# djeedai/bevy_hanabi

Hardware: AMD Instinct MI355X
Metric: particle-updates/sec (higher is better)
Workload: dtype f32

## Files before the change

### bevy_hanabi_amd/__init__.py

```python
from . import build

try:
    from ._hanabi_host import *
except ImportError:
    try:
        build.build_host(verbose=True)
        from ._hanabi_host import *
    except Exception as _e:
        raise ImportError("bevy_hanabi_amd._hanabi_host could not be built: run `python -m bevy_hanabi_amd.build`") from _e
from . import _hanabi_host as host

from .runtime import Comm, Context, Effect, EffectMetadata, HanabiError, Program, SimParams, jit_precompile, jit_precompile_set, jit_precompile_steps, validate_program
```

### bevy_hanabi_amd/build.py

```python
import os
import subprocess
import sys
import sysconfig

_DIR = os.path.dirname(os.path.abspath(__file__))
_CSRC = os.path.join(_DIR, "csrc")

HIP_FLAGS = ["--offload-arch=gfx950", "-O3", "-std=c++17", "-ffp-contract=off", "-fhip-fp32-correctly-rounded-divide-sqrt",
             "-fPIC", "-shared", "-Wno-unused-value"]
HOST_FLAGS = ["-std=c++17", "-O2", "-fPIC", "-shared", "-ffp-contract=off", "-fvisibility=hidden"]


def _newer(target, sources):
    if not os.path.exists(target):
        return True
    t = os.path.getmtime(target)
    return any(os.path.getmtime(s) > t for s in sources)


def runtime_lib_path():
    return os.path.join(_DIR, "libhanabi_amd.so")


def host_module_path():
# ... 74 lines not shown
    lines = [f"// generated by bevy_hanabi_amd/build.py from {unit}.hsaco -- do not edit",
             f"alignas(4096) static const unsigned char {array}[{len(code)}] = {{"]
    lines += ["    " + ",".join(str(b) for b in code[i:i + 64]) + "," for i in range(0, len(code), 64)]
    lines.append("};")
    new = "\n".join(lines) + "\n"
    if not os.path.exists(inc) or open(inc).read() != new:
        open(inc, "w").write(new)
    return out


def build_export_code(force=False, verbose=False):
    return _build_code_object("hnb_export", "kExportCode", [], force, verbose)


def build_export_sort_code(force=False, verbose=False):
    return _build_code_object("hnb_export_sort", "kExportSortCode", ["-ffp-contract=off"], force, verbose)


def build_export_filter_code(force=False, verbose=False):
    return _build_code_object("hnb_export_filter", "kExportFilterCode", ["-ffp-contract=off"], force, verbose)


def build_export_cull_code(force=False, verbose=False):
    return _build_code_object("hnb_export_cull", "kExportCullCode", ["-ffp-contract=off"], force, verbose)


def build_export_filter_prog_code(force=False, verbose=False):
    return _build_code_object("hnb_export_filter_prog", "kExportFilterProgCode", ["-ffp-contract=off"], force, verbose)


def build_export_cull_prog_code(force=False, verbose=False):
    return _build_code_object("hnb_export_cull_prog", "kExportCullProgCode", ["-ffp-contract=off"], force, verbose)


def build_export_bin_code(force=False, verbose=False):
    return _build_code_object("hnb_export_bin", "kExportBinCode", ["-ffp-contract=off"], force, verbose,
                              headers=("hnb_export_bin.h", "hnb_bin_cell.h", "hnb_export.h", "hnb_export_rows.hip.h", "hnb_sort_key.h", "hnb_export_sort.hip.h"))


EXPORT_CODE_OBJECTS = (build_export_code, build_export_sort_code, build_export_filter_code, build_export_cull_code, build_export_filter_prog_code,
                       build_export_cull_prog_code)
BINNED_CODE_OBJECTS = (build_export_bin_code,)


def build_bounds_code(force=False, verbose=False):
    return _build_code_object("hnb_bounds", "kBoundsCode", ["-ffp-contract=off"], force, verbose, headers=("hnb_bounds.h", "hnb_sort_key.h"))


QUERY_CODE_OBJECTS = (build_bounds_code,)


def build_runtime(force=False, verbose=False):
    srcs = [os.path.join(_CSRC, "hanabi_amd.hip")] + sorted(os.path.join(_CSRC, f) for f in os.listdir(_CSRC) if f.endswith(".h"))
    srcs += [os.path.join(_DIR, "..", "include", h) for h in ("hanabi_amd.h", "hanabi_amd_binned.h")]
    for build_code in EXPORT_CODE_OBJECTS + BINNED_CODE_OBJECTS + QUERY_CODE_OBJECTS:
        srcs.append(build_code(force, verbose))
    out = runtime_lib_path()
    if force or _newer(out, srcs):
        embed_headers()
        hipcc = os.environ.get("HIPCC", "/opt/rocm/bin/hipcc")
        cmd = [hipcc] + HIP_FLAGS + [srcs[0], "-o", out, "-lhiprtc", "-ldl"]
        if verbose:
            print(" ".join(cmd))
        subprocess.check_call(cmd, cwd=_CSRC)
    return out


def build_host(force=False, verbose=False):
    import pybind11

    hdir = os.path.join(_CSRC, "host")
    srcs = [os.path.join(hdir, f) for f in ("pybind.cpp", "hanabi.cpp", "lowering.cpp", "wgsl.cpp", "ron.cpp")]
    deps = srcs + [os.path.join(hdir, "hanabi.hpp"), os.path.join(_DIR, "..", "include", "hanabi_amd.h")]
    out = host_module_path()
    if force or _newer(out, deps):
        cmd = ["g++"] + HOST_FLAGS + ["-I" + pybind11.get_include(), "-I" + sysconfig.get_paths()["include"]] + srcs + ["-o", out]
        if verbose:
            print(" ".join(cmd))
        subprocess.check_call(cmd)
    return out


def host_lib_path():
    return os.path.join(_DIR, "libhanabi_host.so")


def build_host_lib(force=False, verbose=False):
    hdir = os.path.join(_CSRC, "host")
    srcs = [os.path.join(hdir, f) for f in ("capi.cpp", "hanabi.cpp", "lowering.cpp", "wgsl.cpp", "ron.cpp")]
    deps = srcs + [os.path.join(hdir, "hanabi.hpp"), os.path.join(_DIR, "..", "include", "hanabi_amd.h"), os.path.join(_DIR, "..", "include", "hanabi_amd_host.h")]
    out = host_lib_path()
    if force or _newer(out, deps):
        cmd = ["g++"] + [f for f in HOST_FLAGS if f != "-fvisibility=hidden"] + srcs + ["-o", out]
        if verbose:
            print(" ".join(cmd))
        subprocess.check_call(cmd)
    return out


def build_examples(force=False, verbose=False):
    root = os.path.join(_DIR, "..")
    src = os.path.join(root, "examples", "multi_gpu.c")
    out = os.path.join(root, "examples", "multi_gpu")
    if force or _newer(out, [src, os.path.join(root, "include", "hanabi_amd.h"), runtime_lib_path()]):
        cmd = ["gcc", "-std=c99", "-O2", "-Wall", "-pthread", "-I" + os.path.join(root, "include"), src, "-L" + _DIR, "-lhanabi_amd",
               "-Wl,-rpath," + os.path.abspath(_DIR), "-Wl,-rpath,$ORIGIN/../bevy_hanabi_amd", "-o", out]
        if verbose:
# ... 25 lines not shown
```

### bevy_hanabi_amd/csrc/hanabi_amd.hip

```cpp
#include <hip/hip_runtime.h>

#include <algorithm>
#include <atomic>
#include <chrono>
#include <cmath>
#include <condition_variable>
#include <cstdarg>
#include <cstdio>
#include <cstring>
#include <deque>
#include <memory>
#include <mutex>
#include <string>
#include <thread>
#include <vector>

#include "hnb_kernels.hip.h"
#include "hnb_jit.h"
#include "hnb_sort.hip.h"
#include "hnb_comm.h"
#include "hnb_plan.h"
#include "hnb_export.h"
#include "hnb_export_code.inc"
#include "hnb_export_sort_code.inc"
#include "hnb_filter_pred.h"
#include "hnb_export_filter_code.inc"
#include "hnb_export_cull_code.inc"
#include "hnb_export_filter_prog_code.inc"
#include "hnb_export_cull_prog_code.inc"
#include "hnb_export_bin.h"
#include "hnb_export_bin_code.inc"
#include "hnb_bounds.h"
#include "hnb_bounds_code.inc"

using namespace hnb;

namespace {

thread_local std::string g_last_error;

int fail(int code, const char* fmt, ...) {
    char buf[512];
    va_list ap;
    va_start(ap, fmt);
    vsnprintf(buf, sizeof buf, fmt, ap);
    va_end(ap);
    g_last_error = buf;
    return code;
}

#define HIP_TRY(expr)                                                                            \
    do {                                                                                         \
        hipError_t e_ = (expr);                                                                  \
        if (e_ != hipSuccess)                                                                    \
            return fail(e_ == hipErrorOutOfMemory ? HNB_ERR_OUT_OF_MEMORY : HNB_ERR_HIP, "%s failed: %s", #expr, \
                        hipGetErrorString(e_));                                                  \
    } while (0)

size_t align_up(size_t v, size_t a) { return (v + a - 1) / a * a; }


struct TimingPair { hipEvent_t a, b; const HnbProgram* prog; };
constexpr uint32_t kFrameRing = plan::kStageSlots;
constexpr uint32_t kSceneMaxChunks = 16;
constexpr uint32_t kSceneMaxInitBlocks = 64;
#ifndef HNB_GENERIC_SPLIT_MAX
#define HNB_GENERIC_SPLIT_MAX 128
#endif
constexpr uint32_t kGenericSplitMaxChunks = HNB_GENERIC_SPLIT_MAX;
#ifndef HNB_STREAM_QUARTERS
#define HNB_STREAM_QUARTERS 1
#endif
constexpr uint32_t kSceneMaxCodeLen = 64;

}

typedef void (*StreamLaunchFn)(uint32_t grid, hipStream_t stream, const SlotArgs& sa, const uint64_t* inst_base, const DevFrameInst* fi,
                               const uint32_t* ublocks, const CompactBufs& cb);
#ifndef HNB_STREAM_WAVES_COHORT
#define HNB_STREAM_WAVES_COHORT 4
#endif
template <class PROG, int WAVES>
void launch_stream(uint32_t grid, hipStream_t stream, const SlotArgs& sa, const uint64_t* inst_base, const DevFrameInst* fi,
                   const uint32_t* ublocks, const CompactBufs& cb) {
    if (sa.age_cohort) k_update_slots_stream<PROG, (WAVES > HNB_STREAM_WAVES_COHORT ? HNB_STREAM_WAVES_COHORT : WAVES), 0, true><<<grid, kBlock, 0, stream>>>(sa, inst_base, fi, ublocks, cb);
// ... 23 lines not shown
typedef ProgStatic<OP_(AGE_TICK), OP_(VEL_ADD), OP_(VEL_SCALE), OP_(EULER)> ProgAccelDrag;
typedef ProgStatic<OP_(AGE_TICK), OP_(VEL_ADD), OP_(KILL_AABB), OP_(EULER)> ProgAccelKillAabb;
typedef ProgStatic<OP_(AGE_TICK), OP_(RADIAL_ACCEL), OP_(EULER)> ProgRadial;
typedef ProgStatic<OP_(AGE_TICK), OP_(CONFORM_SPHERE), OP_(CONFORM_SPHERE), OP_(KILL_AABB), OP_(KILL_SPHERE), OP_(EULER)> ProgForceField;
#undef OP_
#ifndef HNB_STREAM_WAVES_INTERP
#define HNB_STREAM_WAVES_INTERP 5
#endif

void select_stream_kernel(const Ins* code, uint32_t n, StreamLaunchFn* fn, const char** name, StreamLaunchFn* fused) {
#define TRY_(PROG, WAVES) if (PROG::matches(code, n)) { *fn = &launch_stream<PROG, WAVES>; *fused = &launch_stream_fused<PROG, WAVES>; *name = #PROG; return; }
    *fused = nullptr;
    if (ProgNone::matches(code, n)) { *fn = &launch_stream<ProgNone, HNB_STREAM_WAVES>; *name = "ProgNone"; return; }
    if (ProgAge::matches(code, n)) { *fn = &launch_stream_age; *fused = &launch_stream_fused<ProgAge, 4>; *name = "ProgAge"; return; }
    TRY_(ProgAgeEuler, HNB_STREAM_WAVES)
    TRY_(ProgAccel, HNB_STREAM_WAVES)
    TRY_(ProgDrag, HNB_STREAM_WAVES)
    TRY_(ProgDragAccel, HNB_STREAM_WAVES)
    TRY_(ProgAccelDrag, HNB_STREAM_WAVES)
    TRY_(ProgAccelKillAabb, HNB_STREAM_WAVES)
    TRY_(ProgRadial, HNB_STREAM_WAVES)
    TRY_(ProgForceField, HNB_STREAM_WAVES_FULL)
#undef TRY_
    *fn = &launch_stream<ProgInterp, HNB_STREAM_WAVES_INTERP>;
    *name = "ProgInterp";
}

struct ProgramOptions {
    uint32_t age_cohort = HNB_AGE_COHORT_AUTO;
    bool cull_lifetime = true;
    bool horizon = true;
};

struct SetBuildJob {
    struct Member { std::vector<HnbAttrEntry> attrs; std::vector<Ins> init, update; bool streams = false, cohort = false; };
    std::vector<Member> members;
    jit::SetResult res;
    bool ok = false;
    std::atomic<bool> done{false};
    std::thread worker;
};

struct JitJob {
    uint64_t program_serial = 0;
    std::vector<uint8_t> blob;
    HnbProgramHeader hdr{};
    std::vector<HnbAttrEntry> attrs;
    bool streams = false, aot_static = false;
    ProgramOptions opt;
    bool steps = false;
    std::vector<Ins> steps_ops;
    int steps_waves = 0;
    bool steps_cohort = false;
    jit::Result res;
    bool ok = false;
};
struct JitWorker {
    std::thread thread;
    std::mutex mu;
    std::condition_variable cv, done_cv;
    std::deque<std::unique_ptr<JitJob>> queue, done;
    bool stop = false;
    uint32_t in_flight = 0;
};

struct HnbContext {
    int device = 0;
    hipStream_t stream = nullptr;
    hipStream_t own_stream = nullptr;
    hipStream_t upload_stream = nullptr;
    hipStream_t side_stream = nullptr;
    hipEvent_t ev_fork = nullptr, ev_join = nullptr;
    bool overlap_updates = true;
    bool stream_hints = true;
    bool break_proof = false;
    void* h_stage[kFrameRing] = {};
    void* d_stage[kFrameRing] = {};
    size_t stage_bytes = 0;
    bool large_bar = false;
    bool direct_upload = true;
    bool stage_direct = false;
    bool direct_failed = false;
    uint64_t direct_frames = 0, copied_frames = 0;
    uint64_t ring_waits = 0, ring_wait_ns = 0;
    hipEvent_t stage_done[plan::kStageGroups] = {};
    plan::StageRing stage_ring;
    uint32_t num_cus = 256;
    std::vector<HnbProgram*> programs;
    HnbSimParams sim{};
    uint32_t frame = 0;
    uint32_t list_order = HNB_LIST_ORDER_SPAWN;
    ProgramOptions popt;
    bool skip_lists = true;
    bool alternate = true;
    bool suffix_proof = true;
    uint32_t slot_init = 1;
    bool ring_lists = true;
    bool scene_merge = true;
    bool transpose = true;
    uint32_t timing = 0;
    uint32_t timing_tick = 0;
    std::vector<TimingPair> t_update, t_init, t_compact;
    std::vector<hipEvent_t> event_pool;
    uint32_t comm_refs = 0;
    uint32_t set_mode = HNB_SET_MODULE_CACHED;
    struct SetModule {
        hipModule_t module = nullptr;
        hipFunction_t init = nullptr, update = nullptr;
        jit::SetPlan plan;
        uint32_t gen = 0;
    } set;
    bool jit_async = false;
    std::unique_ptr<JitWorker> jit_worker;
    uint64_t next_program_serial = 1;
    std::shared_ptr<SetBuildJob> set_job;
    plan::SetLookupState set_lookup;
    uint32_t set_frames = 0;
    uint32_t set_failed_builds = 0;
    std::string set_log;
    bool fuse_steps = true;
    HnbStepStats step_stats{};
    hipModule_t export_module[kExportUnitCount] = {};
    hipFunction_t export_fn[kExpKernelCount] = {};
    hipModule_t export_bin_module = nullptr;
    hipFunction_t export_bin_fn[kExportBinKernelCount] = {};
    hipModule_t bounds_module = nullptr;
    hipFunction_t bounds_fn[kBoundsKernelCount] = {};
};

struct HnbProgram {
    HnbContext* ctx = nullptr;
    HnbProgramHeader hdr{};
    std::vector<HnbAttrEntry> attrs;
    std::vector<HnbPropEntry> props;
    DevProgram dev{};
    Ins* d_code = nullptr;
    size_t slab_bytes = 0;
    bool wide_file = false;
    uint32_t cull_dt_operand = 0;
    bool update_streams = false;
    uint32_t age_cohort_mode = HNB_AGE_COHORT_AUTO;
    bool auto_materialise = false;
    StreamLaunchFn stream_launch = nullptr;
    StreamLaunchFn stream_launch_fused = nullptr;
    uint32_t fuse_span = 1, fused_left = 0;
    uint32_t safe_launches = 0;
    std::vector<uint32_t> fuse_ublocks;
    uint32_t fused_frames = 0;
    const char* stream_kernel_name = "";
    hipModule_t jit_module = nullptr;
    hipFunction_t jit_init = nullptr, jit_update = nullptr, jit_init_slots = nullptr;
    bool slot_init_eligible = false;
    uint32_t slot_init_frames = 0;
    uint32_t sort_skipped_frames = 0;
    uint32_t sort_path_frames[3] = {0, 0, 0};
    bool tick_sign_seen = false;
    uint64_t serial = 0;
    bool jit_pending = false;
    std::string kernel_info, jit_log;
    enum class StepsState { NotRequested, Built, Pending, Failed };
    hipModule_t steps_module = nullptr;
    hipFunction_t steps_update = nullptr;
    StepsState steps_state = StepsState::NotRequested;
    bool steps_from_cache = false;
    std::string steps_why;
    std::vector<Ins> steps_ops;
    int steps_waves = 0;
    bool steps_cohort = false;
    std::vector<Ins> h_init, h_update;
    std::string set_sig;
    uint64_t set_sig_hash = 0;
    uint32_t set_gen = 0, set_case = kNoSetCase, set_frames = 0;
    std::vector<Ins> uniform_code;
    std::vector<HnbEffect*> effects;
    uint32_t table_cap = 0;
    uint64_t* d_inst_base = nullptr;
    DevMeta* d_meta[2] = {nullptr, nullptr};
    struct SlabBlock { char* base = nullptr; uint32_t n_slots = 0; };
    std::vector<SlabBlock> slab_blocks;
    std::vector<void*> free_slabs;
    size_t slab_stride = 0;
    bool slot_order = false;
    bool has_ribbons = false;
    SortArgs sort{};
    uint32_t* d_plane_by_attr = nullptr;
    std::vector<uint32_t> parent_attrs;
    uint32_t* d_ev_totals = nullptr;
    unsigned long long* h_ev_counts = nullptr;
    uint32_t level = 0;
    uint32_t* d_counts = nullptr;
    uint32_t* d_deaths = nullptr;
    plan::SkipFacts skip_facts;
    plan::SkipHistory skip_hist;
    plan::RibbonFacts ribbon_facts;
    plan::RibbonHistory ribbon_hist;
    plan::FramePlan plan;
    const char* d_frame_cur = nullptr;
    uint32_t ring = 0;
    size_t frame_bytes = 0;
    uint32_t parity = 0;
    uint32_t frames_run = 0;
    uint32_t merged_frames = 0;
    uint32_t unmerged_frames = 0;
    bool horizon_eligible = false;
    uint32_t hz_parity = 0;
    uint32_t hz_frames = 0;
    uint32_t* d_safe = nullptr;
    unsigned long long* h_safe = nullptr;
    uint32_t* d_fault = nullptr;
    uint32_t skipped_frames = 0;
    uint32_t sort_parity = 0;
    uint32_t suffix_frames = 0;
    uint32_t sort_rotated_frames = 0;
    bool ring_live = false;
    uint32_t ring_frames = 0;
    uint32_t* d_export = nullptr;
    uint32_t export_cap = 0;
    std::vector<uint32_t> export_slot_bases;
    void* d_export_sort = nullptr;
    uint32_t export_sort_inst = 0;
    void* d_export_filter = nullptr;
// ... 529 lines not shown

void install_program_jit(HnbProgram* p, const jit::Result& res) {
    const bool aot_static = p->update_streams && strcmp(p->stream_kernel_name, "ProgInterp") != 0;
    hipModule_t mod = nullptr;
    hipFunction_t fi = nullptr, fu = nullptr;
    hipError_t je = hipModuleLoadData(&mod, res.code.data());
    if (je == hipSuccess && !res.init_name.empty()) je = hipModuleGetFunction(&fi, mod, res.init_name.c_str());
    hipFunction_t fs = nullptr;
    if (je == hipSuccess && !res.init_slots_name.empty()) je = hipModuleGetFunction(&fs, mod, res.init_slots_name.c_str());
    if (je == hipSuccess && !res.update_name.empty()) je = hipModuleGetFunction(&fu, mod, res.update_name.c_str());
    if (je != hipSuccess) {
        p->jit_log = std::string("loading the specialised code object failed: ") + hipGetErrorString(je);
        if (mod) hipModuleUnload(mod);
        (void)hipGetLastError();
        return;
    }
    p->jit_module = mod; p->jit_init = fi; p->jit_update = fu; p->jit_init_slots = fs;
    p->kernel_info = std::string(p->wide_file ? "wide-file " : "") + "init=" + (p->jit_init ? "jit" : (p->hdr.init_len ? "interp" : "none")) + " update=" +
                     (p->jit_update ? (p->update_streams ? "jit-stream" : "jit-generic")
                                    : (p->update_streams ? (aot_static ? std::string("aot-stream:") + p->stream_kernel_name : std::string("interp-stream"))
                                                         : std::string("interp-generic")));
    if (res.from_cache) p->kernel_info += " (jit cache hit)";
}

jit::Request make_steps_request(const std::vector<Ins>& ops, int waves, bool cohort) {
    jit::Request rq;
    rq.update = ops.data(); rq.update_len = (uint32_t)ops.size();
    rq.want_update_stream = !ops.empty();
    rq.stream_waves = waves;
    rq.stream_cohort = cohort;
    return rq;
}
void steps_build_failed(HnbProgram* p, const std::string& log) {
    p->steps_state = HnbProgram::StepsState::Failed;
    p->steps_why = log.substr(0, log.find('\n'));
    if (p->steps_why.empty()) p->steps_why = "no log";
    p->jit_log = "steps kernel: " + log;
}
void install_program_steps(HnbProgram* p, const jit::Result& res) {
    hipModule_t mod = nullptr;
    hipFunction_t fu = nullptr;
    hipError_t je = hipModuleLoadData(&mod, res.code.data());
    if (je == hipSuccess) je = hipModuleGetFunction(&fu, mod, res.update_name.c_str());
    if (je != hipSuccess) {
        if (mod) hipModuleUnload(mod);
        (void)hipGetLastError();
        steps_build_failed(p, std::string("loading the code object failed: ") + hipGetErrorString(je));
        return;
    }
    p->steps_module = mod; p->steps_update = fu;
    p->steps_from_cache = res.from_cache;
    p->steps_state = HnbProgram::StepsState::Built;
}
const char* steps_never_reason(const HnbProgram* p) {
    if (!p->update_streams) return "never fuses: not a macro-op update";
    if (!p->skip_facts.eligible) return "never fuses: particles can die by more than their lifetime, or the program is linked to others";
    if (p->has_ribbons || p->hdr.n_event_channels != 0u) return "never fuses: ribbons or spawn events";
    if (p->stream_launch_fused) return "pre-built fused kernel";
    if (p->steps_ops.empty()) return "never fuses: the update is not specialised (HNB_JIT=0)";
    return nullptr;
}
void jit_worker_main(JitWorker* w);
void queue_jit_job(HnbContext* ctx, std::unique_ptr<JitJob> job) {
    if (!ctx->jit_worker) {
        ctx->jit_worker.reset(new JitWorker());
        ctx->jit_worker->thread = std::thread(jit_worker_main, ctx->jit_worker.get());
    }
    {
        std::lock_guard<std::mutex> lk(ctx->jit_worker->mu);
        ctx->jit_worker->queue.push_back(std::move(job));
        ctx->jit_worker->in_flight += 1;
    }
    ctx->jit_worker->cv.notify_one();
}
void request_steps_kernel(HnbContext* ctx, HnbProgram* p, bool wait) {
    if (p->steps_state != HnbProgram::StepsState::NotRequested || !p->jit_update || steps_never_reason(p)) return;
    const bool async = ctx->jit_async && !wait;
    jit::Result res;
    if (jit::build_steps(make_steps_request(p->steps_ops, p->steps_waves, p->steps_cohort), res, async)) {
        install_program_steps(p, res);
    } else if (async && res.log.empty()) {
        std::unique_ptr<JitJob> job(new JitJob());
        job->program_serial = p->serial;
        job->steps = true;
        job->steps_ops = p->steps_ops; job->steps_waves = p->steps_waves; job->steps_cohort = p->steps_cohort;
        queue_jit_job(ctx, std::move(job));
        p->steps_state = HnbProgram::StepsState::Pending;
    } else {
        steps_build_failed(p, res.log);
    }
}

void jit_worker_main(JitWorker* w) {
    for (;;) {
        std::unique_ptr<JitJob> job;
        {
            std::unique_lock<std::mutex> lk(w->mu);
            w->cv.wait(lk, [&] { return w->stop || !w->queue.empty(); });
            if (w->stop) return;
            job = std::move(w->queue.front());
            w->queue.pop_front();
        }
        if (job->steps) {
            job->ok = jit::build_steps(make_steps_request(job->steps_ops, job->steps_waves, job->steps_cohort), job->res);
        } else {
            const jit::Request rq = make_jit_request(job->blob.data(), job->hdr, job->attrs.data(), job->streams, job->aot_static, job->opt);
            job->ok = jit::build(rq, job->res);
        }
        {
            std::lock_guard<std::mutex> lk(w->mu);
            w->done.push_back(std::move(job));
        }
        w->done_cv.notify_all();
    }
}
void install_finished_jit(HnbContext* ctx) {
    if (!ctx->jit_worker) return;
    std::deque<std::unique_ptr<JitJob>> done;
    {
        std::lock_guard<std::mutex> lk(ctx->jit_worker->mu);
        done.swap(ctx->jit_worker->done);
        ctx->jit_worker->in_flight -= (uint32_t)done.size();
    }
    for (std::unique_ptr<JitJob>& j : done) {
        HnbProgram* p = nullptr;
        for (HnbProgram* q : ctx->programs)
            if (q->serial == j->program_serial) p = q;
        if (!p) continue;
        if (j->steps) {
            if (j->ok) install_program_steps(p, j->res);
            else steps_build_failed(p, j->res.log);
            continue;
        }
        p->jit_pending = false;
        if (j->ok) install_program_jit(p, j->res);
        else if (!j->res.log.empty()) p->jit_log = j->res.log;
    }
}

jit::Request make_set_request(const Ins* init, uint32_t init_len, const Ins* update, uint32_t update_len, const HnbAttrEntry* attrs, uint32_t n_attrs,
                              bool streams, bool cohort) {
    jit::Request rq;
    rq.attrs = attrs; rq.n_attrs = n_attrs;
    rq.init = init; rq.init_len = init_len; rq.update = update; rq.update_len = update_len;
    rq.want_init = true;
    rq.want_update_stream = streams;
    rq.want_update_generic = !streams;
    rq.stream_cohort = streams && cohort;
    rq.wide_file = false;
    return rq;
}

}

extern "C" {

const char* hnb_last_error(void) { return g_last_error.c_str(); }
const char* hnb_version(void) { return "bevy_hanabi_amd 0.2.0 (gfx950)"; }

int hnb_ctx_create(int device_id, HnbContext** out_ctx) {
    if (!out_ctx) return fail(HNB_ERR_INVALID_ARG, "out_ctx is NULL");
    int count = 0;
    if (hipGetDeviceCount(&count) != hipSuccess || count <= 0)
        return fail(HNB_ERR_NO_DEVICE, "no HIP device available (the hanabi hot path has no CPU fallback)");
    if (device_id < 0 || device_id >= count) return fail(HNB_ERR_INVALID_ARG, "device %d out of range [0,%d)", device_id, count);
    HIP_TRY(hipSetDevice(device_id));
    HnbContext* ctx = new HnbContext();
    ctx->device = device_id;
    hipError_t e = hipStreamCreateWithFlags(&ctx->stream, hipStreamNonBlocking);
    if (e != hipSuccess) { delete ctx; return fail(HNB_ERR_HIP, "hipStreamCreate failed: %s", hipGetErrorString(e)); }
    ctx->own_stream = ctx->stream;
    e = hipStreamCreateWithFlags(&ctx->upload_stream, hipStreamNonBlocking);
    if (e != hipSuccess) { hipStreamDestroy(ctx->stream); delete ctx; return fail(HNB_ERR_HIP, "hipStreamCreate failed: %s", hipGetErrorString(e)); }
    if (hipStreamCreateWithFlags(&ctx->side_stream, hipStreamNonBlocking) != hipSuccess || hipEventCreateWithFlags(&ctx->ev_fork, hipEventDisableTiming) != hipSuccess ||
        hipEventCreateWithFlags(&ctx->ev_join, hipEventDisableTiming) != hipSuccess) {
        (void)hipGetLastError();
        ctx->overlap_updates = false;
    }
    hipDeviceProp_t prop;
    if (hipGetDeviceProperties(&prop, device_id) == hipSuccess) {
        if (prop.multiProcessorCount > 0) ctx->num_cus = (uint32_t)prop.multiProcessorCount;
        ctx->large_bar = prop.isLargeBar != 0;
    }
    *out_ctx = ctx;
// ... 26 lines not shown
    if (ctx->ev_fork) hipEventDestroy(ctx->ev_fork);
    if (ctx->ev_join) hipEventDestroy(ctx->ev_join);
    for (uint32_t i = 0; i < kFrameRing; ++i) {
        hipFree(ctx->d_stage[i]);
        if (ctx->h_stage[i]) hipHostFree(ctx->h_stage[i]);
    }
    for (hipEvent_t e : ctx->stage_done)
        if (e) hipEventDestroy(e);
    delete ctx;
    return HNB_OK;
}

int hnb_ctx_set_stream(HnbContext* ctx, void* hip_stream) {
    if (!ctx) return fail(HNB_ERR_INVALID_ARG, "ctx is NULL");
    HIP_TRY(hipStreamSynchronize(ctx->stream));
    plan::stage_ring_drained(ctx->stage_ring);
    ctx->stream = hip_stream ? static_cast<hipStream_t>(hip_stream) : ctx->own_stream;
    return HNB_OK;
}

int hnb_ctx_set_option(HnbContext* ctx, uint32_t option, uint32_t value) {
    if (!ctx) return fail(HNB_ERR_INVALID_ARG, "ctx is NULL");
    switch (option) {
        case HNB_OPT_LIST_ORDER:
            if (value != HNB_LIST_ORDER_SPAWN && value != HNB_LIST_ORDER_SLOT) return fail(HNB_ERR_INVALID_ARG, "unknown list order %u", value);
            ctx->list_order = value;
            return HNB_OK;
        case HNB_OPT_ALTERNATE: ctx->alternate = value != 0u; return HNB_OK;
        case HNB_OPT_SKIP_LISTS: ctx->skip_lists = value != 0u; return HNB_OK;
        case HNB_OPT_AGE_COHORT:
            if (value > HNB_AGE_COHORT_AUTO) return fail(HNB_ERR_INVALID_ARG, "unknown age-cohort mode %u", value);
            ctx->popt.age_cohort = value;
            return HNB_OK;
        case HNB_OPT_CULL_LIFETIME: ctx->popt.cull_lifetime = value != 0u; return HNB_OK;
        case HNB_OPT_HORIZON: ctx->popt.horizon = value != 0u; return HNB_OK;
        case HNB_OPT_TEST_BREAK_PROOF: {
            const char* e = getenv("HNB_ENABLE_TEST_HOOKS");
            if (value != 0u && !(e && e[0] == '1')) return fail(HNB_ERR_INVALID_ARG, "HNB_OPT_TEST_BREAK_PROOF is a test hook: refused unless HNB_ENABLE_TEST_HOOKS=1 is set in the environment");
            ctx->break_proof = value != 0u;
            return HNB_OK;
        }
        case HNB_OPT_TRANSPOSE: ctx->transpose = value != 0u; return HNB_OK;
        case HNB_OPT_SCENE_MERGE: ctx->scene_merge = value != 0u; return HNB_OK;
        case HNB_OPT_SUFFIX_PROOF: ctx->suffix_proof = value != 0u; return HNB_OK;
        case HNB_OPT_RING_LISTS: ctx->ring_lists = value != 0u; return HNB_OK;
        case HNB_OPT_SLOT_INIT:
            if (value > 2u) return fail(HNB_ERR_INVALID_ARG, "unknown slot-init mode %u", value);
            ctx->slot_init = value;
            return HNB_OK;
        case HNB_OPT_STREAM_HINTS: ctx->stream_hints = value != 0u; return HNB_OK;
        case HNB_OPT_DIRECT_UPLOAD: ctx->direct_upload = value != 0u; return HNB_OK;
        case HNB_OPT_JIT_ASYNC: ctx->jit_async = value != 0u; return HNB_OK;
        case HNB_OPT_FUSE_STEPS: ctx->fuse_steps = value != 0u; return HNB_OK;
        case HNB_OPT_SET_MODULE:
            if (value > HNB_SET_MODULE_BACKGROUND) return fail(HNB_ERR_INVALID_ARG, "unknown set-module mode %u", value);
            ctx->set_mode = value;
            ctx->set_lookup = plan::SetLookupState();
            return HNB_OK;
        case HNB_OPT_OVERLAP_UPDATES: ctx->overlap_updates = value != 0u && ctx->side_stream && ctx->ev_fork && ctx->ev_join; return HNB_OK;
        default: return fail(HNB_ERR_INVALID_ARG, "unknown option %u", option);
    }
}

int hnb_ctx_synchronize(HnbContext* ctx) {
    if (!ctx) return fail(HNB_ERR_INVALID_ARG, "ctx is NULL");
    HIP_TRY(hipStreamSynchronize(ctx->stream));
    return HNB_OK;
}

int hnb_program_validate(const void* blob, size_t blob_size) { return validate_blob(blob, blob_size, nullptr); }

int hnb_program_create(HnbContext* ctx, const void* blob, size_t blob_size, HnbProgram** out_prog) {
    if (!ctx || !out_prog) return fail(HNB_ERR_INVALID_ARG, "NULL argument");
    HnbProgramHeader h;
    int rc = validate_blob(blob, blob_size, &h);
    if (rc != HNB_OK) return rc;
    HIP_TRY(hipSetDevice(ctx->device));
    const uint8_t* b = static_cast<const uint8_t*>(blob);
    HnbProgram* p = new HnbProgram();
    p->ctx = ctx;
    p->hdr = h;
    p->attrs.resize(h.n_attrs);
    memcpy(p->attrs.data(), b + h.attrs_off, h.n_attrs * sizeof(HnbAttrEntry));
    p->props.resize(h.n_props);
    if (h.n_props) memcpy(p->props.data(), b + h.props_off, h.n_props * sizeof(HnbPropEntry));

    DevProgram& d = p->dev;
    size_t slab_bytes = 0;
    p->update_streams = update_is_streamable(b, h, p->attrs.data());
    if (!layout_slab(h, p->attrs.data(), d, p->sort, &slab_bytes)) { delete p; return fail(HNB_ERR_BAD_PROGRAM, "effect slab exceeds 1 TiB (capacity %u)", h.capacity); }
    p->slot_order = ctx->list_order == HNB_LIST_ORDER_SLOT && !(h.flags & HNB_PROG_HAS_RIBBONS);
    p->has_ribbons = (h.flags & HNB_PROG_HAS_RIBBONS) != 0;
    p->slab_bytes = slab_bytes;
    p->parent_attrs.resize(h.parent_n_attrs);
    if (h.parent_n_attrs) memcpy(p->parent_attrs.data(), b + h.parent_attrs_off, (size_t)h.parent_n_attrs * 4);
    {
        uint32_t planes[HNB_ATTR_COUNT];
        for (uint32_t i = 0; i < HNB_ATTR_COUNT; ++i) planes[i] = kNoPlane;
        for (uint32_t i = 0; i < h.n_attrs; ++i) planes[p->attrs[i].attr] = d.attrs[i].plane_off.v;
        hipError_t pe = hipMalloc(&p->d_plane_by_attr, sizeof planes);
        if (pe != hipSuccess) { delete p; return fail(HNB_ERR_OUT_OF_MEMORY, "hipMalloc failed: %s", hipGetErrorString(pe)); }
        hipMemcpy(p->d_plane_by_attr, planes, sizeof planes, hipMemcpyHostToDevice);
    }
    p->uniform_code.resize(h.uniform_len);
    if (h.uniform_len) memcpy(p->uniform_code.data(), b + h.uniform_off, (size_t)h.uniform_len * 8);
    p->wide_file = std::max(h.init_regs, h.update_regs) > HNB_VM_MAX_REGS;
    p->slot_init_eligible = slot_init_eligible(b, h);
    if (cull_eligible(b, h, p->attrs.data(), p->update_streams, ctx->popt, &p->cull_dt_operand)) {
        d.cull_lifetime = 1u;
        d.age_cohort = age_cohort_eligible(b, h, p->attrs.data(), p->update_streams, ctx->popt) ? 1u : 0u;
    }
    p->age_cohort_mode = ctx->popt.age_cohort;
    p->auto_materialise = ctx->popt.age_cohort == HNB_AGE_COHORT_AUTO && d.age_cohort != 0u && (h.render_reads_lo >> HNB_ATTR_AGE & 1u) != 0u;
    if (p->update_streams) select_stream_kernel(reinterpret_cast<const Ins*>(b + h.update_off), h.update_len, &p->stream_launch, &p->stream_kernel_name, &p->stream_launch_fused);
    if (!p->wide_file && jit::enabled()) {
        p->h_init.assign(reinterpret_cast<const Ins*>(b + h.init_off), reinterpret_cast<const Ins*>(b + h.init_off) + h.init_len);
        p->h_update.assign(reinterpret_cast<const Ins*>(b + h.update_off), reinterpret_cast<const Ins*>(b + h.update_off) + h.update_len);
        p->set_sig = jit::set_signature(make_set_request(p->h_init.data(), h.init_len, p->h_update.data(), h.update_len, p->attrs.data(), h.n_attrs, p->update_streams, d.age_cohort != 0u));
        p->set_sig_hash = jit::fnv1a(p->set_sig);
    }
    const bool aot_static = p->update_streams && strcmp(p->stream_kernel_name, "ProgInterp") != 0;
    p->kernel_info = std::string(p->wide_file ? "wide-file " : "") + "init=" + (h.init_len ? "interp" : "none") + " update=" +
                     (p->update_streams ? (aot_static ? std::string("aot-stream:") + p->stream_kernel_name : std::string("interp-stream")) : std::string("interp-generic"));
    p->serial = ctx->next_program_serial++;
    if (jit::enabled()) {
        const jit::Request rq = make_jit_request(b, h, p->attrs.data(), p->update_streams, aot_static, ctx->popt);
        if (rq.want_update_stream) {
            p->steps_ops.assign(rq.update, rq.update + rq.update_len);
            p->steps_waves = rq.stream_waves; p->steps_cohort = rq.stream_cohort;
        }
        jit::Result res;
        if (jit::build(rq, res, ctx->jit_async)) {
            install_program_jit(p, res);
        } else if (ctx->jit_async && res.log.empty() && (rq.want_init || rq.want_update_generic || rq.want_update_stream)) {
            std::unique_ptr<JitJob> job(new JitJob());
            job->program_serial = p->serial;
            job->blob.assign(b, b + blob_size);
            job->hdr = h; job->attrs = p->attrs; job->streams = p->update_streams; job->aot_static = aot_static; job->opt = ctx->popt;
            queue_jit_job(ctx, std::move(job));
            p->jit_pending = true;
        } else if (!res.log.empty()) {
            p->jit_log = res.log;
        }
    }
    if (p->has_ribbons && p->update_streams) {
        bool ok = true;
        uint32_t ticks = 0;
        const Ins* uc = reinterpret_cast<const Ins*>(b + h.update_off);
        for (uint32_t i = 0; i < h.update_len && ok; ++i) {
            const uint32_t op = uc[i].x & 0xffu, dst = (uc[i].x >> 8) & 0xffu;
            if (op == HNB_OP_M_AGE_TICK) { ticks += 1; p->ribbon_facts.tick_operand = HNB_OPERAND_DECODE((uc[i].x >> 16) & 0xffu, uc[i].y >> 13); ok = (p->ribbon_facts.tick_operand & HNB_OPERAND_DECODED_U) != 0; }
            if (op == HNB_OP_M_PIN_SET && dst == HNB_REG_AGE) ok = false;
        }
        ok = ok && ticks == 1;
        for (uint32_t a = 0; a < h.n_attrs; ++a)
            if (p->attrs[a].attr == HNB_ATTR_RIBBON_ID && (p->attrs[a].update_flags & HNB_ATTR_UPD_STORE)) ok = false;
        const Ins* ic = reinterpret_cast<const Ins*>(b + h.init_off);
        for (uint32_t i = 0; i < h.init_len && ok; ++i) {
            const uint32_t op = ic[i].x & 0xffu, dst = (ic[i].x >> 8) & 0xffu, wd = ((ic[i].y >> 8) & 3u) + 1u;
            if (op == HNB_OP_M_PIN_SET && dst == HNB_REG_AGE) {
                p->ribbon_facts.age_init_operand = HNB_OPERAND_DECODE((ic[i].x >> 16) & 0xffu, ic[i].y >> 13);
                p->ribbon_facts.age_init_set = true;
                ok = (p->ribbon_facts.age_init_operand & HNB_OPERAND_DECODED_U) != 0;
            } else if (op != HNB_OP_STA && op != HNB_OP_ALIVE_SET && op != HNB_OP_ALIVE_AND && op != HNB_OP_KILL_IF && !(op >= HNB_OP_M_AGE_TICK) &&
                       dst <= HNB_REG_AGE && dst + wd > HNB_REG_AGE) {
                ok = false;
            }
        }
        p->ribbon_facts.provable = ok;
        int rid_index = -1;
        for (uint32_t a = 0; a < h.n_attrs; ++a) if (p->attrs[a].attr == HNB_ATTR_RIBBON_ID) rid_index = (int)a;
        uint32_t rid_stores = 0;
        bool front = ok && rid_index >= 0;
        for (uint32_t i = 0; i < h.init_len && front; ++i) {
            const uint32_t op = ic[i].x & 0xffu;
            if (op == HNB_OP_STA && (ic[i].y >> 16) == (uint32_t)rid_index) {
                rid_stores += 1;
                p->ribbon_facts.rid_operand = HNB_OPERAND_DECODE((ic[i].x >> 16) & 0xffu, ic[i].y >> 13);
                front = (p->ribbon_facts.rid_operand & HNB_OPERAND_DECODED_U) != 0;
            }
        }
        p->ribbon_facts.rid_set = rid_stores == 1;
        uint32_t life_sets = 0;
        for (uint32_t i = 0; i < h.init_len && front; ++i) {
            const uint32_t op = ic[i].x & 0xffu, dst = (ic[i].x >> 8) & 0xffu, wd = ((ic[i].y >> 8) & 3u) + 1u;
            if (op == HNB_OP_M_PIN_SET && dst == HNB_REG_LIFETIME) {
                life_sets += 1;
                p->ribbon_facts.life_operand = HNB_OPERAND_DECODE((ic[i].x >> 16) & 0xffu, ic[i].y >> 13);
                front = (p->ribbon_facts.life_operand & HNB_OPERAND_DECODED_U) != 0;
            } else if (op != HNB_OP_STA && op != HNB_OP_ALIVE_SET && op != HNB_OP_ALIVE_AND && op != HNB_OP_KILL_IF && !(op >= HNB_OP_M_AGE_TICK) &&
                       dst <= HNB_REG_LIFETIME && dst + wd > HNB_REG_LIFETIME) {
                front = false;
            }
        }
        for (uint32_t i = 0; i < h.update_len && front; ++i) {
            const uint32_t op = uc[i].x & 0xffu, dst = (uc[i].x >> 8) & 0xffu;
            if (op == HNB_OP_M_KILL_SPHERE || op == HNB_OP_M_KILL_AABB || op == HNB_OP_KILL_IF || op == HNB_OP_ALIVE_SET || op == HNB_OP_ALIVE_AND) front = false;
            if (op == HNB_OP_M_PIN_SET && dst == HNB_REG_LIFETIME) front = false;
        }
        p->ribbon_facts.front_static = front && rid_stores <= 1 && life_sets == 1;
    }
    {
        bool kills = false;
        const Ins* uc = reinterpret_cast<const Ins*>(b + h.update_off);
        for (uint32_t i = 0; i < h.update_len; ++i) {
            const uint32_t op = uc[i].x & 0xffu;
            kills = kills || op == HNB_OP_M_KILL_SPHERE || op == HNB_OP_M_KILL_AABB;
        }
        p->skip_facts.eligible = p->update_streams && d.cull_lifetime && !kills && h.n_event_channels == 0 && !(h.flags & HNB_PROG_READS_PARENT);
        p->skip_facts.dt_operand = p->cull_dt_operand;
        p->horizon_eligible = p->update_streams && d.cull_lifetime && !kills && !p->has_ribbons && !p->slot_order && ctx->popt.horizon;
        if (hipMalloc(&p->d_fault, 4) != hipSuccess ||
            hipHostMalloc(reinterpret_cast<void**>(&p->h_safe), 8, hipHostMallocDefault) != hipSuccess) {
            if (p->jit_module) hipModuleUnload(p->jit_module);
            hipFree(p->d_fault); hipFree(p->d_plane_by_attr);
            delete p;
            return fail(HNB_ERR_OUT_OF_MEMORY, "allocating the program's bookkeeping words failed");
        }
        hipMemset(p->d_fault, 0, 4);
        *p->h_safe = 0xffffffffull;
        p->dev.horizon = p->horizon_eligible ? 1u : 0u;
    }
    const size_t code_bytes = ((size_t)h.init_len + h.update_len) * 8;
    hipError_t e = hipMalloc(&p->d_code, std::max<size_t>(code_bytes, 8));
    if (e != hipSuccess) {
        if (p->jit_module) hipModuleUnload(p->jit_module);
        hipFree(p->d_plane_by_attr); hipFree(p->d_fault); hipHostFree(p->h_safe);
        delete p;
        return fail(HNB_ERR_OUT_OF_MEMORY, "hipMalloc(code) failed: %s", hipGetErrorString(e));
    }
    if (h.init_len) hipMemcpy(p->d_code, b + h.init_off, (size_t)h.init_len * 8, hipMemcpyHostToDevice);
    if (h.update_len) hipMemcpy(p->d_code + h.init_len, b + h.update_off, (size_t)h.update_len * 8, hipMemcpyHostToDevice);
    d.init_code = p->d_code;
    d.update_code = p->d_code + h.init_len;
    ctx->programs.push_back(p);
    *out_prog = p;
    return HNB_OK;
}

int hnb_program_destroy(HnbProgram* p) {
    if (!p) return HNB_OK;
    HnbContext* ctx = p->ctx;
    hipSetDevice(ctx->device);
    hipStreamSynchronize(ctx->stream);
    while (!p->effects.empty()) hnb_effect_destroy(p->effects.back());
    free_tables(p);
    if (p->jit_module) hipModuleUnload(p->jit_module);
    if (p->steps_module) hipModuleUnload(p->steps_module);
    for (auto& blk : p->slab_blocks) hipFree(blk.base);
    hipFree(p->d_plane_by_attr);
    hipFree(p->d_code);
    hipFree(p->d_fault);
    hipFree(p->d_export);
    hipFree(p->d_export_sort);
    hipFree(p->d_export_filter);
    hipFree(p->d_bounds);
    hipFree(p->d_export_cull);
    if (p->h_export_filter_rows) hipHostFree(p->h_export_filter_rows);
    if (p->export_filter_staged) hipEventDestroy(p->export_filter_staged);
    if (p->h_safe) hipHostFree(p->h_safe);
    ctx->programs.erase(std::remove(ctx->programs.begin(), ctx->programs.end(), p), ctx->programs.end());
    delete p;
    return HNB_OK;
}

constexpr size_t kPlacementMinBytes = (size_t)256 << 20;
constexpr size_t kPlacementMaxTransient = (size_t)32 << 30;
hipError_t alloc_slab_block(HnbProgram* p, size_t bytes, char** out) {
    int want = 24;
    if (const char* e = getenv("HNB_SLAB_CANDIDATES")) want = std::max(1, std::min(32, atoi(e)));
    want = (int)std::min<size_t>((size_t)want, std::max<size_t>(1, kPlacementMaxTransient / std::max<size_t>(bytes, 1)));
    if (bytes < kPlacementMinBytes || bytes != p->slab_stride) want = 1;
    const bool debug = getenv("HNB_DEBUG_ALLOC") != nullptr;
    if (want == 1) return hipMalloc(reinterpret_cast<void**>(out), bytes);
    ProbeArgs pa{};
    pa.n_quads = (p->dev.capacity + 3u) / 4u;
    for (uint32_t a = 0; a < p->dev.n_attrs && pa.n_planes < 8; ++a) {
        const DevAttr& at = p->dev.attrs[a];
        if (at.reg == HNB_REG_NONE) continue;
        pa.off[pa.n_planes] = at.plane_off;
        pa.stride16[pa.n_planes] = at.ncomp;
        if (at.reg != HNB_REG_LIFETIME) pa.write_mask |= 1u << pa.n_planes;
        pa.n_planes += 1;
    }
    hipStream_t st = p->ctx->stream;
    hipEvent_t ev0 = nullptr, ev1 = nullptr;
    if (hipEventCreate(&ev0) != hipSuccess || hipEventCreate(&ev1) != hipSuccess) {
        if (ev0) hipEventDestroy(ev0);
        (void)hipGetLastError();
        return hipMalloc(reinterpret_cast<void**>(out), bytes);
    }
    char* best = nullptr;
    float best_ms = 0.0f;
    std::vector<float> times;
    std::vector<char*> rejected;
    hipError_t first_error = hipSuccess;
    for (int c = 0; c < want; ++c) {
        char* cand = nullptr;
        const hipError_t e = hipMalloc(reinterpret_cast<void**>(&cand), bytes);
        if (e != hipSuccess) { if (!best) first_error = e; (void)hipGetLastError(); break; }
        hipMemsetAsync(cand, 0, bytes, st);
// ... 743 lines not shown
    } else {
        p->sort_path_frames[2] += 1;
        for (uint32_t pass = 0; pass < 8; ++pass) {
            k_sort_hist<<<tiles, kBlock, 0, st>>>(so, p->d_inst_base, mo, pass);
            k_sort_scatter<<<tiles, kBlock, 0, st>>>(so, p->d_inst_base, mo, pass);
        }
    }
    k_sort_merge<<<tiles, kBlock, 0, st>>>(so, p->d_inst_base, mo);
    p->ribbon_hist.dirty = false;
}

static bool reads_particles_of(const HnbProgram* child, const HnbProgram* parent) {
    for (const HnbEffect* fx : child->effects)
        if (fx->parent && fx->parent->prog == parent) return true;
    return false;
}
static int enqueue_init_passes(HnbContext* ctx, const std::vector<HnbProgram*>& order, FrameJobs& fj, bool timed) {
    const uint32_t np = (uint32_t)order.size();
    std::vector<uint8_t> on_side(np, 0);
    if (fj.heavy) {
        std::vector<uint8_t> reads((size_t)np * np, 0);
        int heavy = -1;
        for (uint32_t c = 0; c < np; ++c) {
            if (order[c] == fj.heavy) heavy = (int)c;
            for (uint32_t p = 0; p < np; ++p) reads[(size_t)c * np + p] = reads_particles_of(order[c], order[p]) ? 1u : 0u;
        }
        plan::partition_init_passes(reads.data(), np, heavy, on_side.data());
    }
    for (int pass = 0; pass < (fj.heavy ? 2 : 1); ++pass) {
    hipStream_t st = ctx->stream;
    if (pass == 1) {
        st = ctx->side_stream;
        HIP_TRY(hipEventRecord(ctx->ev_fork, ctx->stream));
        HIP_TRY(hipStreamWaitEvent(st, ctx->ev_fork, 0));
        fj.forked = true;
    }
    for (size_t pi = 0; pi < order.size(); ++pi) {
        HnbProgram* p = order[pi];
        if ((int)on_side[pi] != pass) continue;
        const uint32_t n = (uint32_t)p->effects.size();
        const uint32_t par = p->parity;
        const uint32_t blocks = p->plan.init_blocks;
        const char* d = p->d_frame_cur;
        const DevFrameInst* dfi = reinterpret_cast<const DevFrameInst*>(d);
        const uint32_t* dub = reinterpret_cast<const uint32_t*>(d + (size_t)n * sizeof(DevFrameInst));
        if (blocks && p->plan.merge.init_family < 0) {
            TimingPair ti{};
            ti.prog = p;
            if (timed) { ti.a = take_event(ctx); ti.b = take_event(ctx); hipEventRecord(ti.a, st); }
            if (p->plan.slot_init.use) {
                const uint32_t grid = n * p->dev.chunks_per_inst * (kChunk / kSlotInitWg);
                const DevMeta* mi = p->d_meta[par];
                if (p->plan.slot_init.marks) k_spawn_mark<<<grid, kBlock, 0, st>>>(p->dev, p->d_inst_base, mi, dfi);
                if (p->jit_init_slots) {
                    void* ka[] = {&p->dev, &p->d_inst_base, &mi, &dfi, &dub};
                    HIP_TRY(hipModuleLaunchKernel(p->jit_init_slots, grid, 1, 1, kBlock, 1, 1, 0, st, ka, nullptr));
                } else if (p->wide_file) k_init_slots<InterpCodeWide><<<grid, kBlock, 0, st>>>(p->dev, p->d_inst_base, mi, dfi, dub);
                else k_init_slots<InterpCode><<<grid, kBlock, 0, st>>>(p->dev, p->d_inst_base, mi, dfi, dub);
                p->slot_init_frames += 1;
            } else if (p->jit_init) {
                const DevMeta* mi = p->d_meta[par];
                void* ka[] = {&p->dev, &p->d_inst_base, &mi, &dfi, &dub};
                HIP_TRY(hipModuleLaunchKernel(p->jit_init, blocks, 1, 1, kInitBlock, 1, 1, 0, st, ka, nullptr));
            } else {
                if (p->wide_file) k_init<InterpCodeWide><<<blocks, kInitBlock, 0, st>>>(p->dev, p->d_inst_base, p->d_meta[par], dfi, dub);
                else k_init<InterpCode><<<blocks, kInitBlock, 0, st>>>(p->dev, p->d_inst_base, p->d_meta[par], dfi, dub);
            }
            if (timed) { hipEventRecord(ti.b, st); ctx->t_init.push_back(ti); }
        }
    }
    }

    hipStream_t ms = fj.forked ? ctx->side_stream : ctx->stream;
    if (fj.init_set) {
        const void* jobs = fj.init[0].d_jobs;
        uint32_t n_jobs = fj.init[0].n;
        void* ka[] = {&jobs, &n_jobs};
        HIP_TRY(hipModuleLaunchKernel(ctx->set.init, fj.init[0].wgs, 1, 1, kInitBlock, 1, 1, 0, ms, ka, nullptr));
    } else if (fj.init[0].n) k_init_jobs<InterpCode><<<fj.init[0].wgs, kInitBlock, 0, ms>>>(static_cast<const ProgJob*>(fj.init[0].d_jobs), fj.init[0].n);
    if (fj.init[1].n) k_init_jobs<InterpCodeWide><<<fj.init[1].wgs, kInitBlock, 0, ms>>>(static_cast<const ProgJob*>(fj.init[1].d_jobs), fj.init[1].n);
    return HNB_OK;
}

static int enqueue_program_update(HnbContext* ctx, HnbProgram* p, hipStream_t st, bool timed) {
    const uint32_t n = (uint32_t)p->effects.size();
    const uint32_t par = p->parity;
    const char* d = p->d_frame_cur;
    const DevFrameInst* dfi = reinterpret_cast<const DevFrameInst*>(d);
    const uint32_t* dub = reinterpret_cast<const uint32_t*>(d + (size_t)n * sizeof(DevFrameInst));
    const uint32_t total_chunks = n * p->dev.chunks_per_inst;
    CompactBufs cb = compact_bufs_of(ctx, p, n);
    TimingPair tu{}, tc{};
    tu.prog = tc.prog = p;
    if (timed) { tu.a = take_event(ctx); tu.b = take_event(ctx); tc.b = take_event(ctx); hipEventRecord(tu.a, st); }
    const uint32_t write_died = (p->plan.lists && !p->slot_order) ? 1u : 0u;
    if (p->plan.merge.update_family >= 0) {
    } else if (p->update_streams) {
        SlotArgs sa = slot_args_of(ctx, p, n, write_died);
        ctx->step_stats.update_launches += 1;
        if (p->fuse_span >= 2u) {
            sa.fuse_steps = p->fuse_span;
            if (p->steps_update) {
                void* ka[] = {&sa, &p->d_inst_base, &dfi, &dub, &cb};
                HIP_TRY(hipModuleLaunchKernel(p->steps_update, total_chunks, 1, 1, kBlock, 1, 1, 0, st, ka, nullptr));
            } else p->stream_launch_fused(total_chunks, st, sa, p->d_inst_base, dfi, dub, cb);
            ctx->step_stats.fused_launches += 1;
            ctx->step_stats.fused_frames += p->fuse_span;
            p->fused_frames += p->fuse_span;
        } else if (p->jit_update) {
            void* ka[] = {&sa, &p->d_inst_base, &dfi, &dub, &cb};
            HIP_TRY(hipModuleLaunchKernel(p->jit_update, total_chunks, 1, 1, kBlock, 1, 1, 0, st, ka, nullptr));
        } else {
            p->stream_launch(total_chunks, st, sa, p->d_inst_base, dfi, dub, cb);
        }
    } else {
        uint32_t split = total_chunks <= kGenericSplitMaxChunks ? 1u : 0u;
        const uint32_t grid = split ? total_chunks * (kChunk / kBlock) : total_chunks;
        ctx->step_stats.update_launches += 1;
        if (p->jit_update) {
            uint32_t dm = write_died;
            void* ka[] = {&p->dev, &p->d_inst_base, &dfi, &dub, &cb, &dm, &split};
            HIP_TRY(hipModuleLaunchKernel(p->jit_update, grid, 1, 1, kBlock, 1, 1, 0, st, ka, nullptr));
        } else if (p->wide_file) k_update_slots_generic<InterpCodeWide><<<grid, kBlock, 0, st>>>(p->dev, p->d_inst_base, dfi, dub, cb, write_died, split);
        else k_update_slots_generic<InterpCode><<<grid, kBlock, 0, st>>>(p->dev, p->d_inst_base, dfi, dub, cb, write_died, split);
    }
    if (timed) { hipEventRecord(tu.b, st); ctx->t_update.push_back(tu); }
    const CompactArgs ca = compact_args_of(p);
    const bool lists = p->plan.lists;
    if (!lists) p->skipped_frames += p->fuse_span;
    else if (ca.suffix_dead) p->suffix_frames += 1;
    if (lists && p->dev.n_event_channels) {
        k_emit_count<<<total_chunks, kBlock, 0, st>>>(p->dev, p->d_inst_base, p->d_meta[par], dfi, cb);
        uint32_t max_ev = 0;
        for (const HnbEffect* fx : p->effects)
            for (const EventChannel& ch : fx->channels) max_ev = std::max(max_ev, ch.capacity);
        const uint32_t splits = plan::size_event_grid(max_ev, total_chunks);
        k_emit_events<<<dim3(total_chunks, splits), kBlock, 0, st>>>(p->dev, p->d_inst_base, p->d_meta[par], dfi, cb, p->h_ev_counts, ctx->frame);
    }
    if (!p->plan.lists_merged) {
        if (lists) ctx->step_stats.list_launches += ((!p->slot_order && !ca.suffix_dead) ? 2u : 1u) + (p->slot_order ? 2u : 0u);
        if (lists && !p->slot_order && !ca.suffix_dead) k_count_rows<<<total_chunks, kBlock, 0, st>>>(ca, p->d_inst_base, p->d_meta[par], dfi, cb);
        if (lists) k_compact<<<total_chunks, kBlock, 0, st>>>(ca, p->d_inst_base, p->d_meta[par], p->d_meta[par ^ 1], dfi, cb);
        if (lists && p->slot_order) {
            k_order_count<<<total_chunks, kBlock, 0, st>>>(ca, p->d_inst_base, p->d_meta[par], dfi, cb);
            k_order_write<<<total_chunks, kBlock, 0, st>>>(ca, p->d_inst_base, p->d_meta[par], p->d_meta[par ^ 1], dfi, cb);
        }
        if (timed) { tc.a = tu.b; hipEventRecord(tc.b, st); ctx->t_compact.push_back(tc); }
        if (p->has_ribbons) enqueue_ribbon_sort(ctx, p, st);
    }
    HIP_TRY(hipGetLastError());
    return HNB_OK;
}

static int enqueue_update_passes(HnbContext* ctx, const std::vector<HnbProgram*>& order, const FrameJobs& fj, bool timed) {
    hipStream_t light = ctx->stream;
    if (fj.heavy) {
        light = ctx->side_stream;
        if (!fj.forked) {
            HIP_TRY(hipEventRecord(ctx->ev_fork, ctx->stream));
            HIP_TRY(hipStreamWaitEvent(light, ctx->ev_fork, 0));
        }
// ... 5 lines not shown
        const void *sj0 = fj.stream[0].d_jobs, *sj1 = fj.stream[1].d_jobs, *pj = fj.generic[0].d_jobs;
        uint32_t n0 = fj.stream[0].n, n1 = fj.stream[1].n, np = fj.generic[0].n, b0 = fj.stream[0].wgs, b1 = fj.stream[0].wgs + fj.stream[1].wgs;
        void* ka[] = {&sj0, &n0, &sj1, &n1, &pj, &np, &b0, &b1};
        HIP_TRY(hipModuleLaunchKernel(ctx->set.update, fj.stream[0].wgs + fj.stream[1].wgs + fj.generic[0].wgs, 1, 1, kBlock, 1, 1, 0, light, ka, nullptr));
    } else if (fj.stream[0].wgs + fj.stream[1].wgs + fj.generic[0].wgs)
        k_update_jobs<<<fj.stream[0].wgs + fj.stream[1].wgs + fj.generic[0].wgs, kBlock, 0, light>>>(
            static_cast<const StreamJob*>(fj.stream[0].d_jobs), fj.stream[0].n, static_cast<const StreamJob*>(fj.stream[1].d_jobs), fj.stream[1].n,
            static_cast<const ProgJob*>(fj.generic[0].d_jobs), fj.generic[0].n, fj.stream[0].wgs, fj.stream[0].wgs + fj.stream[1].wgs);
    if (fj.generic[1].wgs) k_update_generic_wide_jobs<<<fj.generic[1].wgs, kBlock, 0, light>>>(static_cast<const ProgJob*>(fj.generic[1].d_jobs), fj.generic[1].n);
    for (HnbProgram* p : order) {
        if (p == fj.heavy) continue;
        const int rc = enqueue_program_update(ctx, p, light, timed);
        if (rc != HNB_OK) return rc;
    }
    if (fj.n_lists) {
        k_count_rows_multi<<<fj.lists_wgs, kBlock, 0, light>>>(fj.d_lists, fj.n_lists);
        k_compact_multi<<<fj.lists_wgs, kBlock, 0, light>>>(fj.d_lists, fj.n_lists);
        for (HnbProgram* p : order)
            if (p->plan.lists_merged && p->has_ribbons) enqueue_ribbon_sort(ctx, p, light);
        HIP_TRY(hipGetLastError());
    }
    if (fj.heavy) {
        const int rc = enqueue_program_update(ctx, const_cast<HnbProgram*>(fj.heavy), ctx->stream, timed);
        if (rc != HNB_OK) return rc;
        HIP_TRY(hipEventRecord(ctx->ev_join, light));
        HIP_TRY(hipStreamWaitEvent(ctx->stream, ctx->ev_join, 0));
    }
    return HNB_OK;
}

static int simulate_frame(HnbContext* ctx) {
    HIP_TRY(hipSetDevice(ctx->device));
    install_finished_jit(ctx);
    std::vector<HnbProgram*> order, covered;
    for (HnbProgram* p : ctx->programs)
        if (!p->effects.empty()) (p->fused_left ? covered : order).push_back(p);
    std::stable_sort(order.begin(), order.end(), [](const HnbProgram* x, const HnbProgram* y) { return x->level < y->level; });
    const bool timed = ctx->timing && (ctx->timing_tick % ctx->timing) == 0;
    for (HnbProgram* p : order)
        if (!p->parent_attrs.empty())
            for (size_t i = 0; i < p->effects.size(); ++i)
                if (!p->effects[i]->parent)
                    return fail(HNB_ERR_INVALID_ARG, "effect #%zu reads its parent particle (InheritAttributeModifier / parent_attr) but has no parent: call hnb_effect_set_parent", i);
    uint32_t slot = 0;
    int rc = ensure_stage(ctx, order, &slot);
    if (rc != HNB_OK) return rc;
    size_t stage_off = 0;
    std::vector<plan::InstanceFrame> inst_frames;
    for (HnbProgram* p : order) stage_program_frame(ctx, p, slot, stage_off, inst_frames);
    FrameJobs fj;
    fj.heavy = pick_heavy_program(ctx, order, timed);
    fill_lists_jobs(ctx, order, slot, stage_off, timed, fj);
    fill_merge_jobs(ctx, order, slot, stage_off, timed, fj);
    if (stage_off) {
        if (ctx->stage_direct) {
            direct_write(ctx->d_stage[slot], ctx->h_stage[slot], stage_off);
            ctx->direct_frames += 1;
        } else {
            hipError_t ce = hipMemcpyAsync(ctx->d_stage[slot], ctx->h_stage[slot], stage_off, hipMemcpyHostToDevice, ctx->upload_stream);
            if (ce == hipSuccess) ce = hipStreamSynchronize(ctx->upload_stream);
            if (ce != hipSuccess) {
                plan::stage_ring_end(ctx->stage_ring, !order.empty(), true, false);
                HIP_TRY(ce);
            }
            ctx->copied_frames += 1;
        }
    }
    rc = enqueue_init_passes(ctx, order, fj, timed);
    if (rc == HNB_OK) rc = enqueue_update_passes(ctx, order, fj, timed);
    if (rc != HNB_OK) {
        if (ctx->side_stream && (fj.forked || fj.heavy)) hipStreamSynchronize(ctx->side_stream);
        plan::stage_ring_end(ctx->stage_ring, !order.empty(), true, false);
        return rc;
    }
    for (HnbProgram* p : covered) p->fused_left -= 1;
    for (HnbProgram* p : order) {
        const uint32_t span = p->fuse_span;
        p->fused_left = span - 1u;
        p->fuse_span = 1u;
        p->safe_launches += 1;
        p->ring += span;
        p->parity ^= span & 1u;
        p->frames_run += span;
        if (p->horizon_eligible && p->plan.lists) p->hz_parity ^= 1u;
        if (p->plan.ribbon.ring) { p->ring_live = true; p->ring_frames += 1; }
        else if (p->plan.lists) p->ring_live = false;
    }
    const int stage_event = plan::stage_ring_end(ctx->stage_ring, !order.empty(), true, true);
    if (stage_event != plan::kStageWaitNone) {
        const hipError_t re = hipEventRecord(ctx->stage_done[stage_event], ctx->stream);
        if (re != hipSuccess) ctx->stage_ring.torn = true;
        HIP_TRY(re);
    }
    for (HnbProgram* p : ctx->programs)
        for (HnbEffect* fx : p->effects) fx->spawn_count = 0;
    ctx->frame += 1;
    ctx->step_stats.frames += 1;
    if (ctx->timing) ctx->timing_tick += 1;
    return HNB_OK;
}

static void drop_ahead_inputs(HnbContext* ctx) {
    for (HnbProgram* p : ctx->programs)
        for (HnbEffect* fx : p->effects) { fx->ahead_n = 0; fx->ahead_spawn.clear(); fx->ahead_seed.clear(); fx->ahead_xf.clear(); }
}

// ... 53 lines not shown
        p->fuse_ublocks.resize((size_t)n * span * nu);
        for (uint32_t i = 0; i < n; ++i)
            for (uint32_t t = 0; t < span; ++t)
                if (nu) memcpy(p->fuse_ublocks.data() + ((size_t)i * span + t) * nu, blocks.data() + ((size_t)t * n + i) * nu, (size_t)nu * 4);
    }
}

int hnb_simulate_steps(HnbContext* ctx, uint32_t n_steps, const HnbSimParams* params) {
    if (!ctx) return fail(HNB_ERR_INVALID_ARG, "ctx is NULL");
    if (n_steps == 0u) return HNB_OK;
    if (!params) return fail(HNB_ERR_INVALID_ARG, "params is NULL");
    for (HnbProgram* p : ctx->programs)
        if (!p->parent_attrs.empty())
            for (size_t i = 0; i < p->effects.size(); ++i)
                if (!p->effects[i]->parent)
                    return fail(HNB_ERR_INVALID_ARG, "effect #%zu reads its parent particle (InheritAttributeModifier / parent_attr) but has no parent: call hnb_effect_set_parent", i);
    if (n_steps >= 2u) {
        HIP_TRY(hipSetDevice(ctx->device));
        install_finished_jit(ctx);
        for (HnbProgram* p : ctx->programs) {
            if (p->steps_state != HnbProgram::StepsState::NotRequested || !p->jit_update || !ctx->fuse_steps) continue;
            bool parent = false;
            for (const HnbEffect* fx : p->effects) parent = parent || fx->parent != nullptr;
            if (!parent && (uint64_t)p->effects.size() * p->dev.chunks_per_inst > kSceneMaxChunks) request_steps_kernel(ctx, p, false);
        }
    }
    int rc = HNB_OK;
    for (uint32_t s = 0; s < n_steps && rc == HNB_OK; ++s) {
        ctx->sim = params[s];
        for (HnbProgram* p : ctx->programs)
            for (HnbEffect* fx : p->effects) {
                if (s >= fx->ahead_n) continue;
                fx->spawn_count = fx->ahead_spawn[s];
                fx->seed = fx->ahead_seed[s];
                if (!fx->ahead_xf.empty()) memcpy(fx->xf, &fx->ahead_xf[(size_t)s * 12], sizeof fx->xf);
            }
        if (n_steps - s >= 2u) plan_fused_spans(ctx, params + s, n_steps - s, s);
        rc = simulate_frame(ctx);
    }
    for (HnbProgram* p : ctx->programs) {
        if (rc != HNB_OK) {
            if (p->fuse_span >= 2u) p->skip_hist.dirty = true;
            p->fused_left = 0u;
        }
        p->fuse_span = 1u;
    }
    drop_ahead_inputs(ctx);
    return rc;
}

int hnb_ctx_step_stats(HnbContext* ctx, HnbStepStats* out) {
    if (!ctx || !out) return fail(HNB_ERR_INVALID_ARG, "NULL argument");
    *out = ctx->step_stats;
    return HNB_OK;
}

int hnb_effect_metadata(HnbEffect* fx, HnbEffectMetadata* out) {
    if (!fx || !out) return fail(HNB_ERR_INVALID_ARG, "NULL argument");
    DevMeta m;
    int rc = read_meta(fx, &m);
    if (rc != HNB_OK) return rc;
    const uint32_t cap = fx->prog->dev.capacity;
    out->capacity = cap;
    out->alive_count = m.alive_count;
    out->max_update = m.max_update;
    out->max_spawn = cap - m.alive_count;
    out->indirect_write_index = m.ref_write_index;
    out->particle_counter = m.particle_counter;
    out->instance_count = m.instance_count;
    out->dispatch_x = (m.alive_count + 63u) >> 6;
    out->dead_count = m.dead_count;
    out->spawned = m.spawned;
    out->fault = 0;
    if (fx->prog->d_fault) HIP_TRY(hipMemcpy(&out->fault, fx->prog->d_fault, 4, hipMemcpyDeviceToHost));
    out->reserved = 0;
    return HNB_OK;
}

int hnb_effect_alive_count(HnbEffect* fx, uint32_t* out) {
    if (!fx || !out) return fail(HNB_ERR_INVALID_ARG, "NULL argument");
    DevMeta m;
    int rc = read_meta(fx, &m);
    if (rc != HNB_OK) return rc;
    *out = m.alive_count;
    return HNB_OK;
}

int hnb_effect_read_attr(HnbEffect* fx, uint32_t attr, void* dst, size_t dst_size) {
    if (!fx || !dst) return fail(HNB_ERR_INVALID_ARG, "NULL argument");
    HnbProgram* p = fx->prog;
    const int ai = find_attr(p, attr);
    if (ai < 0) return fail(HNB_ERR_NOT_FOUND, "attribute %u is not part of the particle layout", attr);
    const size_t bytes = (size_t)p->dev.capacity * p->attrs[ai].ncomp * 4;
    if (dst_size < bytes) return fail(HNB_ERR_INVALID_ARG, "destination too small (%zu < %zu)", dst_size, bytes);
    HIP_TRY(hipSetDevice(p->ctx->device));
    if (p->dev.age_cohort && attr == HNB_ATTR_AGE)
        k_materialise_age<<<p->dev.chunks_per_inst, kBlock, 0, p->ctx->stream>>>(p->d_inst_base + fx->index, p->dev.capacity, p->dev.chunks_per_inst, p->dev.lmin_off,
                                                                                  p->dev.attrs[ai].plane_off, p->dev.alive_flag_off);
    HIP_TRY(hipStreamSynchronize(p->ctx->stream));
    HIP_TRY(hipMemcpy(dst, static_cast<char*>(fx->slab) + p->dev.attrs[ai].plane_off, bytes, hipMemcpyDeviceToHost));
    return HNB_OK;
}

int hnb_effect_write_attr(HnbEffect* fx, uint32_t attr, const void* src, size_t src_size) {
    if (!fx || !src) return fail(HNB_ERR_INVALID_ARG, "NULL argument");
    HnbProgram* p = fx->prog;
// ... 808 lines not shown
        cmp(0, sa + pa->dev.alive_off[list_column(ma.write_index)], sb + pb->dev.alive_off[list_column(mb.write_index)], ma.alive_count, list_head(ma.write_index), list_head(mb.write_index), cap);
        cmp(1, sa + pa->dev.dead_off + (size_t)ma.alive_count * 4, sb + pb->dev.dead_off + (size_t)mb.alive_count * 4, cap - ma.alive_count);
    }
    for (size_t i = 0; i < pa->attrs.size(); ++i) cmp(2 + i, sa + pa->dev.attrs[i].plane_off, sb + pb->dev.attrs[i].plane_off, (uint64_t)cap * pa->attrs[i].ncomp);
    std::vector<unsigned long long> res(n_sections * 2);
    e = hipGetLastError();
    if (e == hipSuccess) e = hipDeviceSynchronize();
    if (e == hipSuccess) e = hipMemcpy(res.data(), d_out, n_sections * 16, hipMemcpyDeviceToHost);
    hipFree(d_out);
    if (e != hipSuccess) return fail(HNB_ERR_HIP, "hnb_effect_compare: %s", hipGetErrorString(e));
    out->alive_list_diffs = res[0]; out->dead_list_diffs = res[2];
    for (size_t i = 0; i < pa->attrs.size(); ++i) out->attr_diffs += res[2 * (2 + i)];
    for (size_t i = 0; i < n_sections && out->first_section < 0; ++i)
        if (res[2 * i]) { out->first_section = i < 2 ? (int32_t)i : (int32_t)(2 + pa->attrs[i - 2].attr); out->first_index = res[2 * i + 1]; }
    out->equal = out->counter_diffs == 0u && out->alive_list_diffs == 0ull && out->dead_list_diffs == 0ull && out->attr_diffs == 0ull;
    return HNB_OK;
}

int hnb_effect_sort_ribbons(HnbEffect* fx) {
    if (!fx) return fail(HNB_ERR_INVALID_ARG, "fx is NULL");
    if (!fx->prog->has_ribbons) return fail(HNB_ERR_INVALID_ARG, "the particle layout has no RIBBON_ID attribute: nothing to sort");
    return HNB_OK;
}

int hnb_program_kernel_info(HnbProgram* prog, char* buf, size_t buf_size) {
    if (!prog || !buf || !buf_size) return fail(HNB_ERR_INVALID_ARG, "NULL argument");
    std::string s = prog->kernel_info;
    if (prog->jit_pending) s += " (specialisation pending: HNB_OPT_JIT_ASYNC)";
    if (!prog->jit_log.empty()) s += "\njit log: " + prog->jit_log;
    {
        const char* never = steps_never_reason(prog);
        s += "\nsteps kernel: ";
        switch (prog->steps_state) {
        case HnbProgram::StepsState::NotRequested: s += std::string("not requested") + (never ? std::string(" (") + never + ")" : std::string()); break;
        case HnbProgram::StepsState::Built: s += std::string("built") + (prog->steps_from_cache ? " (jit cache hit)" : ""); break;
        case HnbProgram::StepsState::Pending: s += "pending (HNB_OPT_JIT_ASYNC)"; break;
        case HnbProgram::StepsState::Failed: s += "failed: " + prog->steps_why; break;
        }
    }
    if (!prog->dev.age_cohort && prog->dev.cull_lifetime && prog->age_cohort_mode == HNB_AGE_COHORT_AUTO && (prog->hdr.render_reads_lo >> HNB_ATTR_AGE & 1u))
        s += "\nage cohorts: off (HNB_AGE_COHORT_AUTO: the asset's render modifiers read AGE after every frame)";
    if (prog->dev.age_cohort) {
        hipStreamSynchronize(prog->ctx->stream);
        std::vector<uint32_t> st(prog->dev.chunks_per_inst);
        size_t in_cohort = 0;
        for (const HnbEffect* fx : prog->effects) {
            if (hipMemcpy(st.data(), static_cast<const char*>(fx->slab) + prog->dev.lmin_off + (size_t)prog->dev.chunks_per_inst * 8, st.size() * 4, hipMemcpyDeviceToHost) != hipSuccess) break;
            for (uint32_t v : st) in_cohort += v == 1u ? 1u : 0u;
        }
        s += "\nage cohorts: " + std::to_string(in_cohort) + " of " + std::to_string(prog->effects.size() * (size_t)prog->dev.chunks_per_inst) + " chunks";
        if (prog->auto_materialise) s += " (HNB_AGE_COHORT_AUTO: the asset's render modifiers read AGE, the update keeps the plane current)";
    }
    if (prog->slot_init_frames) s += "\nslot-major init (large spawns): " + std::to_string(prog->slot_init_frames) + " frames";
    if (prog->has_ribbons && prog->suffix_frames) s += "\ncasualties proven to be the list's last rows (no k_count_rows): " + std::to_string(prog->suffix_frames) + " frames";
    if (prog->has_ribbons && prog->ring_frames) s += "\nlist kept as a ring (no row rewritten): " + std::to_string(prog->ring_frames) + " frames";
    if (prog->has_ribbons && prog->sort_skipped_frames) s += "\nribbon sorts skipped in list-free frames: " + std::to_string(prog->sort_skipped_frames) + " frames";
    if (prog->has_ribbons) s += "\nribbon sorts by rotation: " + std::to_string(prog->sort_rotated_frames) + " of " + std::to_string(prog->frames_run) + " frames" + (prog->ribbon_facts.front_static ? "" : " (not eligible)");
    if (prog->has_ribbons) s += "\nribbon sorts by path: one-tile " + std::to_string(prog->sort_path_frames[0]) + ", one-workgroup " + std::to_string(prog->sort_path_frames[1]) +
                                ", multi-launch " + std::to_string(prog->sort_path_frames[2]) + " frames";
    if (prog->merged_frames) s += "\nupdate served by a merged launch (small programs of the context share one): " + std::to_string(prog->merged_frames) + " frames";
    if (prog->unmerged_frames) s += "\nkept out of the shared launches (the loaded set module does not know this program; its own specialised kernels): " + std::to_string(prog->unmerged_frames) + " frames";
    if (prog->set_frames) s += "\n... by the context's set module (the program's specialised code behind the shared launch): " + std::to_string(prog->set_frames) + " frames";
    if (!prog->ctx->set_log.empty() && !prog->set_sig.empty()) s += "\nset module: " + prog->ctx->set_log;
    if (prog->ctx->set_failed_builds && !prog->set_sig.empty()) s += "\nset module builds that failed: " + std::to_string(prog->ctx->set_failed_builds);
    if (prog->horizon_eligible) s += "\ndeath horizons in use: " + std::to_string(prog->hz_frames) + " frames";
    s += "\nlists skipped: " + std::to_string(prog->skipped_frames) + " of " + std::to_string(prog->frames_run) + " frames" + (prog->skip_facts.eligible ? "" : " (not eligible)");
    s += "\nframe parameters (context): written by the host into device memory in " + std::to_string(prog->ctx->direct_frames) + " frames, copied in " + std::to_string(prog->ctx->copied_frames) +
         (prog->ctx->large_bar ? "" : " (the device memory is not host-visible: no large BAR)") + (prog->ctx->direct_failed ? " (host-visible slots failed their check)" : "");
    s += "\nhnb_simulate waited for the device (the frame " + std::to_string(kFrameRing - plan::kStageGroup + 1u) + " before still running) in " + std::to_string(prog->ctx->ring_waits) + " of " + std::to_string(prog->ctx->frame) +
         " frames, " + std::to_string(prog->ctx->ring_wait_ns / 1000) + " us in all";
    snprintf(buf, buf_size, "%s", s.c_str());
    return HNB_OK;
}

int hnb_jit_precompile(const void* blob, size_t blob_size) {
    HnbProgramHeader h;
    int rc = validate_blob(blob, blob_size, &h);
    if (rc != HNB_OK) return rc;
    const uint8_t* b = static_cast<const uint8_t*>(blob);
    std::vector<HnbAttrEntry> attrs(h.n_attrs);
    memcpy(attrs.data(), b + h.attrs_off, h.n_attrs * sizeof(HnbAttrEntry));
    const bool streams = update_is_streamable(b, h, attrs.data());
    bool aot_static = false;
    if (streams) {
        StreamLaunchFn fn = nullptr;
        const char* name = "";
        StreamLaunchFn fused = nullptr;
        select_stream_kernel(reinterpret_cast<const Ins*>(b + h.update_off), h.update_len, &fn, &name, &fused);
        aot_static = strcmp(name, "ProgInterp") != 0;
    }
    const jit::Request rq = make_jit_request(b, h, attrs.data(), streams, aot_static, ProgramOptions());
    if (!rq.want_init && !rq.want_update_generic && !rq.want_update_stream) return HNB_OK;
    jit::Result res;
    if (!jit::build(rq, res)) return fail(HNB_ERR_BAD_PROGRAM, "kernel specialisation failed: %s", res.log.c_str());
    return HNB_OK;
}

int hnb_jit_precompile_steps(const void* blob, size_t blob_size) {
    HnbProgramHeader h;
    int rc = validate_blob(blob, blob_size, &h);
    if (rc != HNB_OK) return rc;
    const uint8_t* b = static_cast<const uint8_t*>(blob);
    std::vector<HnbAttrEntry> attrs(h.n_attrs);
    memcpy(attrs.data(), b + h.attrs_off, h.n_attrs * sizeof(HnbAttrEntry));
    if (!update_is_streamable(b, h, attrs.data())) return HNB_OK;
    StreamLaunchFn fn = nullptr, fused = nullptr;
    const char* name = "";
    select_stream_kernel(reinterpret_cast<const Ins*>(b + h.update_off), h.update_len, &fn, &name, &fused);
    const jit::Request rq = make_jit_request(b, h, attrs.data(), true, strcmp(name, "ProgInterp") != 0, ProgramOptions());
    if (!rq.want_update_stream) return HNB_OK;
    jit::Result res;
    if (!jit::build_steps(rq, res)) return fail(HNB_ERR_BAD_PROGRAM, "steps kernel: specialisation failed: %s", res.log.c_str());
    return HNB_OK;
}

int hnb_program_prepare_steps(HnbProgram* prog) {
    if (!prog) return fail(HNB_ERR_INVALID_ARG, "prog is NULL");
    HnbContext* ctx = prog->ctx;
    if (steps_never_reason(prog)) return HNB_OK;
    HIP_TRY(hipSetDevice(ctx->device));
    for (;;) {
        install_finished_jit(ctx);
        if (!prog->jit_pending && prog->steps_state != HnbProgram::StepsState::Pending) break;
        std::unique_lock<std::mutex> lk(ctx->jit_worker->mu);
        ctx->jit_worker->done_cv.wait(lk, [&] { return !ctx->jit_worker->done.empty(); });
    }
    request_steps_kernel(ctx, prog, true);
    if (prog->steps_state == HnbProgram::StepsState::Failed) return fail(HNB_ERR_BAD_PROGRAM, "steps kernel: %s", prog->steps_why.c_str());
    return HNB_OK;
}

int hnb_jit_precompile_set(const void* const* blobs, const size_t* blob_sizes, uint32_t n_blobs) {
    if (!blobs || !blob_sizes || n_blobs == 0u) return fail(HNB_ERR_INVALID_ARG, "NULL argument");
    struct Member { std::vector<HnbAttrEntry> attrs; std::vector<Ins> init, update; bool streams = false, cohort = false; };
    std::vector<Member> mem;
    mem.reserve(n_blobs);
    for (uint32_t i = 0; i < n_blobs; ++i) {
        HnbProgramHeader h;
        const int rc = validate_blob(blobs[i], blob_sizes[i], &h);
        if (rc != HNB_OK) return rc;
        if (std::max(h.init_regs, h.update_regs) > HNB_VM_MAX_REGS) continue;
        if ((uint64_t)h.capacity > (uint64_t)kSceneMaxChunks * kChunk || h.n_event_channels != 0u || (h.flags & HNB_PROG_READS_PARENT)) continue;
        const uint8_t* b = static_cast<const uint8_t*>(blobs[i]);
        Member m;
        m.attrs.resize(h.n_attrs);
        memcpy(m.attrs.data(), b + h.attrs_off, h.n_attrs * sizeof(HnbAttrEntry));
        m.init.assign(reinterpret_cast<const Ins*>(b + h.init_off), reinterpret_cast<const Ins*>(b + h.init_off) + h.init_len);
        m.update.assign(reinterpret_cast<const Ins*>(b + h.update_off), reinterpret_cast<const Ins*>(b + h.update_off) + h.update_len);
        m.streams = update_is_streamable(b, h, m.attrs.data());
        uint32_t dt_operand = 0;
        const ProgramOptions opt;
        m.cohort = cull_eligible(b, h, m.attrs.data(), m.streams, opt, &dt_operand) && age_cohort_eligible(b, h, m.attrs.data(), m.streams, opt);
        mem.push_back(std::move(m));
    }
    std::vector<jit::Request> members;
    for (const Member& m : mem)
        members.push_back(make_set_request(m.init.data(), (uint32_t)m.init.size(), m.update.data(), (uint32_t)m.update.size(), m.attrs.data(), (uint32_t)m.attrs.size(), m.streams, m.cohort));
    if (members.size() < 2u) return HNB_OK;
    jit::SetResult res;
    if (!jit::build_set(members, res, false)) return fail(HNB_ERR_BAD_PROGRAM, "set module: kernel specialisation failed: %s", res.log.c_str());
    return HNB_OK;
}

int hnb_comm_unique_id(void* out_id) {
    if (!out_id) return fail(HNB_ERR_INVALID_ARG, "out_id is NULL");
// ... 191 lines not shown
```

### bevy_hanabi_amd/csrc/hnb_jit.h

```cpp
#pragma once
#include <dlfcn.h>
#include <hip/hip_runtime.h>
#include <hip/hiprtc.h>
#include <sys/stat.h>
#include <unistd.h>
#include <cstdio>
#include <cstdlib>
#include <cstring>
#include <fstream>
#include <algorithm>
#include <atomic>
#include <sstream>
#include <string>
#include <vector>
#include "hnb_dev.h"
#include "hnb_embedded_headers.inc"

namespace hnb {
namespace jit {

inline bool enabled() {
    const char* e = getenv("HNB_JIT");
    return !(e && e[0] == '0');
}

inline uint64_t fnv1a(const std::string& s, uint64_t h = 1469598103934665603ull) {
    for (unsigned char c : s) { h ^= c; h *= 1099511628211ull; }
    return h;
}

inline std::string cache_dir() {
    if (const char* e = getenv("HNB_JIT_CACHE")) return e;
    Dl_info info;
    if (dladdr(reinterpret_cast<const void*>(&fnv1a), &info) && info.dli_fname) {
        std::string p = info.dli_fname;
        const size_t k = p.rfind('/');
        if (k != std::string::npos) return p.substr(0, k) + "/jit_cache";
    }
    return "/tmp/hanabi_amd_jit_cache";
}

struct Request {
    const HnbAttrEntry* attrs = nullptr;
    uint32_t n_attrs = 0;
    const Ins* init = nullptr;
    uint32_t init_len = 0;
    const Ins* update = nullptr;
    uint32_t update_len = 0;
    bool want_init = false;
    bool want_init_slots = false;
    bool want_update_generic = false;
    bool want_update_stream = false;
    int stream_waves = 6;
    bool stream_cohort = false;
    bool wide_file = false;
};

struct Result {
    std::vector<char> code;
    std::string init_name, init_slots_name, update_name;
    std::string log;
    bool from_cache = false;
};

inline void emit_ins(std::ostringstream& o, const Ins* code, uint32_t n) {
    char buf[160];
    for (uint32_t i = 0; i < n; ++i) {
        snprintf(buf, sizeof buf, "        vm_exec<true, false>(Ins{0x%08xu, 0x%08xu}, S, U, nullptr, nullptr, io);\n", code[i].x, code[i].y);
        o << buf;
    }
}

inline void emit_code_struct(std::ostringstream& o, const Request& rq, const std::string& name) {
    o << "struct " << name << " {\n";
    o << "    using file_t = " << (rq.wide_file ? "vreg_file_wide_t" : "vreg_file_t") << ";\n";
    o << "    template <class ST> static __device__ __forceinline__ void run_init(const DevProgram& p, ST& S, const VmUniforms& U, const VmAttrIO& io) {\n";
    if (rq.want_init) emit_ins(o, rq.init, rq.init_len);
    o << "    }\n";
    o << "    template <class ST> static __device__ __forceinline__ void run_update(const DevProgram& p, ST& S, const VmUniforms& U, const VmAttrIO& io) {\n";
    if (rq.want_update_generic) emit_ins(o, rq.update, rq.update_len);
    o << "    }\n";
    o << "    static __device__ __forceinline__ void zero_unassigned(const DevProgram& p, const VmAttrIO& io) {\n";
    for (uint32_t a = 0; a < rq.n_attrs; ++a) {
        if (rq.attrs[a].reg != HNB_REG_NONE) continue;
        o << "        { uint32_t* q = vm_attr_ptr(io, " << a << "u);";
        for (uint32_t c = 0; c < rq.attrs[a].ncomp; ++c) o << " q[" << c << "] = 0u;";
        o << " }\n";
    }
    o << "    }\n";
    o << "    template <class ST> static __device__ __forceinline__ void store_init(const DevProgram& p, const ST& S, char* base, uint32_t slot) {\n";
    for (uint32_t a = 0; a < rq.n_attrs; ++a)
        if (rq.attrs[a].reg != HNB_REG_NONE)
            o << "        vfile_store_attr(S.r, " << (unsigned)rq.attrs[a].ncomp << "u, " << (unsigned)rq.attrs[a].reg << "u, base + p.attrs[" << a
              << "].plane_off, slot);\n";
    o << "    }\n";
    o << "    template <class ST> static __device__ __forceinline__ void load_update(const DevProgram& p, ST& S, const char* base, uint32_t slot, bool valid) {\n";
    for (uint32_t a = 0; a < rq.n_attrs; ++a) {
        const HnbAttrEntry& at = rq.attrs[a];
        if (!(at.update_flags & HNB_ATTR_UPD_LOAD) || at.reg == HNB_REG_NONE) continue;
        o << "        { Out4 o = Out4{0u, 0u, 0u, 0u}; if (valid) o = vfile_load_attr(" << (unsigned)at.ncomp << "u, base + p.attrs[" << a << "].plane_off, slot);";
        for (uint32_t c = 0; c < at.ncomp; ++c) o << " S.r[" << (unsigned)(at.reg + c) << "] = o.v" << c << ";";
        o << " }\n";
    }
    o << "    }\n";
    o << "    template <class ST> static __device__ __forceinline__ void store_update(const DevProgram& p, const ST& S, char* base, uint32_t slot) {\n";
    for (uint32_t a = 0; a < rq.n_attrs; ++a) {
        const HnbAttrEntry& at = rq.attrs[a];
        if ((at.update_flags & HNB_ATTR_UPD_STORE) && at.reg != HNB_REG_NONE)
            o << "        vfile_store_attr(S.r, " << (unsigned)at.ncomp << "u, " << (unsigned)at.reg << "u, base + p.attrs[" << a << "].plane_off, slot);\n";
    }
    o << "    }\n};\n";
}
inline std::string stream_prog_type(const Request& rq) {
    std::ostringstream e;
    e << "hnb::ProgStatic<";
    for (uint32_t i = 0; i < rq.update_len; ++i) e << (i ? ", " : "") << (rq.update[i].x & 0xffu) << "u";
    e << ">";
    return e.str();
}

inline std::string make_source(const Request& rq, std::vector<std::string>& name_exprs) {
    std::ostringstream o;
    o << "#define HNB_JIT_TU 1\n#include \"hnb_kernels.hip.h\"\nnamespace hnb {\n";
    if (rq.want_init || rq.want_update_generic) emit_code_struct(o, rq, "JitCode");
    o << "}  // namespace hnb\n";
    name_exprs.clear();
    if (rq.want_init) name_exprs.push_back("hnb::k_init<hnb::JitCode>");
    if (rq.want_init && rq.want_init_slots) name_exprs.push_back("hnb::k_init_slots<hnb::JitCode>");
    if (rq.want_update_generic) name_exprs.push_back("hnb::k_update_slots_generic<hnb::JitCode>");
    if (rq.want_update_stream) {
        std::ostringstream e;
        e << "hnb::k_update_slots_stream<" << stream_prog_type(rq) << ", " << rq.stream_waves << ", 0, " << (rq.stream_cohort ? "true" : "false") << ">";
        name_exprs.push_back(e.str());
    }
    return o.str();
}

inline std::string make_steps_source(const Request& rq, std::vector<std::string>& name_exprs) {
    name_exprs.clear();
    if (!rq.want_update_stream) return std::string();
    std::ostringstream e;
    e << "hnb::k_update_slots_stream<" << stream_prog_type(rq) << ", " << rq.stream_waves << ", 0, " << (rq.stream_cohort ? "true" : "false") << ", true>";
    name_exprs.push_back(e.str());
    return "#define HNB_JIT_TU 1\n#include \"hnb_kernels.hip.h\"\n// steps module\n";
}

inline std::string set_signature(const Request& rq) {
    std::ostringstream o;
    if (rq.want_init || rq.want_update_generic) emit_code_struct(o, rq, "C");
    if (rq.want_update_stream) o << "//stream " << stream_prog_type(rq) << (rq.stream_cohort ? " cohort" : " plain") << "\n";
    return o.str();
}
struct SetPlan {
    std::vector<std::string> signatures;
    uint32_t case_of(const std::string& sig) const {
        const auto it = std::lower_bound(signatures.begin(), signatures.end(), sig);
        return (it != signatures.end() && *it == sig) ? (uint32_t)(it - signatures.begin()) : 0xffffffffu;
    }
};
inline std::string make_set_source(const std::vector<Request>& members, SetPlan& plan) {
    std::vector<std::pair<std::string, const Request*>> sorted;
    for (const Request& rq : members) sorted.emplace_back(set_signature(rq), &rq);
    std::sort(sorted.begin(), sorted.end(), [](const auto& a, const auto& b) { return a.first < b.first; });
    sorted.erase(std::unique(sorted.begin(), sorted.end(), [](const auto& a, const auto& b) { return a.first == b.first; }), sorted.end());
    plan.signatures.clear();
    std::ostringstream o, ki, ks0, ks1, kg;
    o << "#define HNB_JIT_TU 1\n#include \"hnb_kernels.hip.h\"\nnamespace hnb {\n";
    for (size_t i = 0; i < sorted.size(); ++i) {
        const Request& rq = *sorted[i].second;
        plan.signatures.push_back(sorted[i].first);
        const std::string name = "SetCode" + std::to_string(i);
        if (rq.want_init || rq.want_update_generic) emit_code_struct(o, rq, name);
        if (rq.want_init)
            ki << "    case " << i << "u: init_workgroup<" << name << ">(jb.prog, jb.inst_base, jb.meta_in, jb.fi, jb.ublocks, blockIdx.x - jb.first_wg, jb.n_wg); break;\n";
        if (rq.want_update_stream)
            (rq.stream_cohort ? ks1 : ks0) << "        case " << i << "u: update_stream_chunk<" << stream_prog_type(rq) << ", 0, " << (rq.stream_cohort ? "true" : "false")
                                           << ">(jb.args, jb.inst_base, jb.fi, jb.ublocks, jb.cb, blockIdx.x - jb.first_wg, jb.n_wg); break;\n";
        if (rq.want_update_generic)
            kg << "        case " << i << "u: update_generic_chunk<" << name
               << ">(jb.prog, jb.inst_base, jb.fi, jb.ublocks, jb.cb, jb.write_died, w / kGenericSubs, jb.n_wg / kGenericSubs, sub, sub + 1u); break;\n";
    }
    o << "extern \"C\" __global__ void __launch_bounds__(kInitBlock) hnb_set_init(const ProgJob* __restrict__ jobs, uint32_t n_jobs) {\n"
         "    const ProgJob& jb = job_of_workgroup_t(jobs, n_jobs);\n    switch (jb.set_case) {\n" << ki.str() << "    default: break;\n    }\n}\n";
    o << "extern \"C\" __global__ void __launch_bounds__(kBlock) hnb_set_update(const StreamJob* __restrict__ sj0, uint32_t n0, const StreamJob* __restrict__ sj1, uint32_t n1,\n"
         "                                                                    const ProgJob* __restrict__ pj, uint32_t np, uint32_t b0, uint32_t b1) {\n"
         "    if (blockIdx.x < b0) {\n        const StreamJob& jb = job_of_workgroup_t(sj0, n0);\n        switch (jb.set_case) {\n" << ks0.str() << "        default: break;\n        }\n"
         "    } else if (blockIdx.x < b1) {\n        const StreamJob& jb = job_of_workgroup_t(sj1, n1);\n        switch (jb.set_case) {\n" << ks1.str() << "        default: break;\n        }\n"
         "    } else {\n        const ProgJob& jb = job_of_workgroup_t(pj, np);\n        const uint32_t w = blockIdx.x - jb.first_wg, sub = w % kGenericSubs;\n        switch (jb.set_case) {\n"
      << kg.str() << "        default: break;\n        }\n    }\n}\n";
    o << "}  // namespace hnb\n";
    return o.str();
}

inline bool read_file(const std::string& p, std::vector<char>& out) {
    std::ifstream f(p, std::ios::binary);
    if (!f) return false;
    out.assign(std::istreambuf_iterator<char>(f), std::istreambuf_iterator<char>());
// ... 86 lines not shown
    }
    for (const std::string& e : exprs) {
        const char* ln = nullptr;
        if (hiprtcGetLoweredName(prog, e.c_str(), &ln) != HIPRTC_SUCCESS || !ln) { log = "no lowered name for " + e; hiprtcDestroyProgram(&prog); return false; }
        lowered.push_back(ln);
    }
    size_t cs = 0;
    hiprtcGetCodeSize(prog, &cs);
    code_out.resize(cs);
    hiprtcGetCode(prog, code_out.data());
    hiprtcDestroyProgram(&prog);
    mkdir(dir.c_str(), 0700);
    std::string names;
    for (const std::string& l : lowered) names += l + "\n";
    CacheHeader h = want;
    h.code_size = code_out.size(); h.code_hash = hash_bytes(code_out.data(), code_out.size());
    h.n_names = (uint32_t)lowered.size(); h.names_bytes = (uint32_t)names.size();
    static std::atomic<unsigned> tmp_serial{0};
    const std::string tmp = entry_path + ".tmp" + std::to_string((long)getpid()) + "." + std::to_string(tmp_serial.fetch_add(1u));
    bool ok = false;
    {
        std::ofstream f(tmp, std::ios::binary);
        f.write(reinterpret_cast<const char*>(&h), sizeof h);
        f.write(names.data(), (std::streamsize)names.size());
        f.write(code_out.data(), (std::streamsize)code_out.size());
        f.flush();
        ok = f.good();
    }
    if (!ok || rename(tmp.c_str(), entry_path.c_str()) != 0) unlink(tmp.c_str());
    return true;
}

inline bool build(const Request& rq, Result& out, bool cache_only = false) {
    std::vector<std::string> exprs, lowered;
    const std::string src = make_source(rq, exprs);
    if (exprs.empty()) return false;
    if (!compile_cached(src, exprs, out.code, lowered, out.log, out.from_cache, cache_only)) return false;
    size_t k = 0;
    if (rq.want_init) out.init_name = lowered[k++];
    if (rq.want_init && rq.want_init_slots) out.init_slots_name = lowered[k++];
    if (rq.want_update_generic || rq.want_update_stream) out.update_name = lowered[k++];
    return true;
}

inline bool build_steps(const Request& rq, Result& out, bool cache_only = false) {
    std::vector<std::string> exprs, lowered;
    const std::string src = make_steps_source(rq, exprs);
    if (exprs.empty()) return false;
    if (!compile_cached(src, exprs, out.code, lowered, out.log, out.from_cache, cache_only)) return false;
    out.update_name = lowered[0];
    return true;
}

struct SetResult {
    std::vector<char> code;
    SetPlan plan;
    std::string log;
    bool from_cache = false;
};
inline bool build_set(const std::vector<Request>& members, SetResult& out, bool cache_only) {
    if (members.empty()) return false;
    const std::string src = make_set_source(members, out.plan);
    std::vector<std::string> lowered;
    return compile_cached(src, {}, out.code, lowered, out.log, out.from_cache, cache_only);
}

}
}
```

### bevy_hanabi_amd/csrc/hnb_kernels.hip.h

```cpp
#pragma once
#ifndef __HIPCC_RTC__
#include <hip/hip_runtime.h>
#endif
#include "hnb_dev.h"

namespace hnb {

template <class T>
__device__ __forceinline__ T* global_ptr(uint64_t addr) {
    typedef __attribute__((address_space(1))) T global_t;
    return (T*)(global_t*)addr;
}

struct u2_t { uint32_t x, y; };
struct u3_t { uint32_t x, y, z; };
typedef uint32_t u4v __attribute__((ext_vector_type(4)));
#if defined(HNB_NONTEMPORAL) || defined(HNB_NONTEMPORAL_LOADS)
#define HNB_NT_LOAD(p) __builtin_nontemporal_load(p)
#else
#define HNB_NT_LOAD(p) (*(p))
#endif
#if defined(HNB_NONTEMPORAL) || defined(HNB_NONTEMPORAL_STORES)
#define HNB_NT_STORE(v, p) __builtin_nontemporal_store(v, p)
#else
// ... 261 lines not shown
                atomicMin(&hz.D(prog.hz_parity)[rc], d2u(clock_now + (double)u2f(m)));
                atomicMin(&hz.BF(prog.hz_parity)[rc], prog.frame_no);
            }
        }
        pass_no += 1u;
    }
    }
}
template <class CODE>
__global__ void __launch_bounds__(kInitBlock)
k_init(const DevProgram prog, const uint64_t* __restrict__ inst_base, const DevMeta* __restrict__ meta_in,
       const DevFrameInst* __restrict__ fi, const uint32_t* __restrict__ ublocks) {
    init_workgroup<CODE>(prog, inst_base, meta_in, fi, ublocks, blockIdx.x, gridDim.x);
}
constexpr uint32_t kSlotInitWg = 1024u;
struct SlotInitCtx {
    uint32_t k, w;
    uint32_t alive0, n_spawn;
    bool full;
    char* base;
};
__device__ __forceinline__ void slot_init_setup(SlotInitCtx& c, const DevProgram& prog, const uint64_t* __restrict__ inst_base, const DevMeta* __restrict__ meta_in,
                                                const DevFrameInst* __restrict__ fi, const uint32_t wg) {
    const uint32_t per_inst = prog.chunks_per_inst * (kChunk / kSlotInitWg);
    c.k = wg / per_inst;
    c.w = wg - c.k * per_inst;
    const uint64_t slab = inst_base[c.k];
    c.alive0 = meta_in[c.k].alive_count;
    const uint32_t max_spawn = prog.capacity - c.alive0;
    const uint32_t spawn = requested_spawn(fi[c.k]);
    c.n_spawn = spawn < max_spawn ? spawn : max_spawn;
    c.full = c.n_spawn == max_spawn;
    c.base = global_ptr<char>(slab);
}
#ifndef HNB_JIT_TU
__global__ void __launch_bounds__(kBlock)
k_spawn_mark(const DevProgram prog, const uint64_t* __restrict__ inst_base, const DevMeta* __restrict__ meta_in, const DevFrameInst* __restrict__ fi) {
    SlotInitCtx c;
    slot_init_setup(c, prog, inst_base, meta_in, fi, blockIdx.x);
    if (c.full || c.w * kSlotInitWg >= c.n_spawn) return;
    const uint32_t* dead = reinterpret_cast<const uint32_t*>(c.base + prog.dead_off);
    uint8_t* flags = reinterpret_cast<uint8_t*>(c.base + prog.alive_flag_off);
    uint32_t slot[kSlotInitWg / kBlock];
#pragma unroll
    for (uint32_t q = 0; q < kSlotInitWg / kBlock; ++q) {
        const uint32_t r = c.w * kSlotInitWg + q * kBlock + threadIdx.x;
        slot[q] = r < c.n_spawn ? dead[c.alive0 + r] : 0xffffffffu;
    }
#pragma unroll
    for (uint32_t q = 0; q < kSlotInitWg / kBlock; ++q)
        if (slot[q] != 0xffffffffu) flags[slot[q]] = 2u;
}
#endif
template <class CODE>
__device__ __forceinline__ void init_slots_workgroup(const DevProgram& prog, const uint64_t* __restrict__ inst_base, const DevMeta* __restrict__ meta_in,
                                                     const DevFrameInst* __restrict__ fi, const uint32_t* __restrict__ ublocks, const uint32_t wg) {
    SlotInitCtx c;
    slot_init_setup(c, prog, inst_base, meta_in, fi, wg);
    if (c.n_spawn == 0u) return;
    const uint32_t tid = threadIdx.x, k = c.k;
    char* base = c.base;
    constexpr uint32_t kSubs = kSlotInitWg / kBlock;
    const uint32_t* dead = reinterpret_cast<const uint32_t*>(base + prog.dead_off);
    uint32_t* alive = reinterpret_cast<uint32_t*>(base + prog.alive_off[list_column(meta_in[k].write_index)]);
    const uint32_t list_first = ring_row(list_head(meta_in[k].write_index), c.alive0, prog.capacity);
    const bool nt = prog.stream_hint != 0u;
    uint32_t row_slot[kSubs];
#pragma unroll
    for (uint32_t q = 0; q < kSubs; ++q) {
        const uint32_t r = c.w * kSlotInitWg + q * kBlock + tid;
        row_slot[q] = r < c.n_spawn ? ld_hint(dead + (c.alive0 + r), nt) : 0xffffffffu;
    }
    uint8_t* flags = reinterpret_cast<uint8_t*>(base + prog.alive_flag_off);
    const uint32_t slot0 = c.w * kSlotInitWg, j = slot0 / kChunk;
    uint32_t byte[kSubs];
#pragma unroll
    for (uint32_t q = 0; q < kSubs; ++q) {
        const uint32_t slot = slot0 + q * kBlock + tid;
        byte[q] = slot < prog.capacity ? (uint32_t)flags[slot] : 1u;
    }
    uint8_t alive_byte = 1u;
    uint32_t* astate = reinterpret_cast<uint32_t*>(base + prog.lmin_off) + 2u * prog.chunks_per_inst;
    uint32_t st = 0u;
    if (prog.age_cohort) {
        st = slot0 < prog.capacity ? astate[j] : 0u;
        if (st == 1u || st == 2u) alive_byte = 3u;
    }
    VmUniforms U;
    U.u = ublocks + (size_t)k * prog.n_uregs;
    U.xf = fi[k].xf;
    const uint32_t want = c.full ? 0u : 2u;
    bool any_spawn = false;
#pragma unroll 1
    for (uint32_t q = 0; q < kSubs; ++q) {
        const uint32_t b = q == 0u ? byte[0] : q == 1u ? byte[1] : q == 2u ? byte[2] : byte[3];
        const bool here = b == want;
        if (!__any(here)) continue;
        any_spawn = true;
        if (here) {
            const uint32_t slot = slot0 + q * kBlock + tid;
            VmState<typename CODE::file_t> S;
            S.r = typename CODE::file_t{};
            S.pindex = slot + fi[k].slot_base;
            S.seed = pcg_hash(S.pindex ^ fi[k].seed);
            S.pcounter = 0u;
            S.alive = true;
            VmAttrIO io;
            io.slab = base; io.attrs = prog.attrs; io.slot = slot;
            CODE::zero_unassigned(prog, io);
            CODE::run_init(prog, S, U, io);
            flags[slot] = alive_byte;
            CODE::store_init(prog, S, base, slot);
        }
    }
    static_assert(kSubs == 4u, "the byte select above is written for four steps");
    if (any_spawn && (tid & 63u) == 0u) {
        if (prog.cull_lifetime) reinterpret_cast<float*>(base + prog.lmin_off)[j] = 0.0f;
        if (alive_byte == 3u && st != 2u) astate[j] = 2u;
    }
#pragma unroll
    for (uint32_t q = 0; q < kSubs; ++q) {
        const uint32_t r = c.w * kSlotInitWg + q * kBlock + tid;
        if (row_slot[q] != 0xffffffffu) st_hint(row_slot[q], alive + ring_row(list_first, r, prog.capacity), nt);
    }
    if (prog.horizon && tid < 2u && c.w * kSlotInitWg < c.n_spawn) {
        const HorizonView hz = horizon_view(base, prog.horizon_off, prog.chunks_per_inst);
        const uint32_t r_first = c.alive0 + c.w * kSlotInitWg;
        const uint32_t r_last = c.alive0 + ((c.w + 1u) * kSlotInitWg < c.n_spawn ? (c.w + 1u) * kSlotInitWg : c.n_spawn) - 1u;
        const uint32_t rc = tid == 0u ? r_first / kChunk : r_last / kChunk;
        if ((tid == 0u || rc != r_first / kChunk) && rc < prog.chunks_per_inst) {
            atomicMin(&hz.D(prog.hz_parity)[rc], d2u(*hz.clock));
            atomicMin(&hz.BF(prog.hz_parity)[rc], prog.frame_no);
        }
    }
}
template <class CODE>
__global__ void __launch_bounds__(kBlock)
k_init_slots(const DevProgram prog, const uint64_t* __restrict__ inst_base, const DevMeta* __restrict__ meta_in,
             const DevFrameInst* __restrict__ fi, const uint32_t* __restrict__ ublocks) {
    init_slots_workgroup<CODE>(prog, inst_base, meta_in, fi, ublocks, blockIdx.x);
}

template <int P>
__device__ __forceinline__ void pin_load3(V3 (&dst)[P], const char* plane, const uint32_t (&slot)[P], const bool (&valid)[P], bool dense) {
    if constexpr (P == 4) {
        if (dense) {
            const u4v* src = reinterpret_cast<const u4v*>(plane) + (size_t)(slot[0] >> 2) * 3;
            const u4v q0 = HNB_NT_LOAD(src), q1 = HNB_NT_LOAD(src + 1), q2 = HNB_NT_LOAD(src + 2);
            dst[0] = V3{u2f(q0.x), u2f(q0.y), u2f(q0.z)};
            dst[1] = V3{u2f(q0.w), u2f(q1.x), u2f(q1.y)};
            dst[2] = V3{u2f(q1.z), u2f(q1.w), u2f(q2.x)};
            dst[3] = V3{u2f(q2.y), u2f(q2.z), u2f(q2.w)};
            return;
        }
    }
#pragma unroll
    for (int p = 0; p < P; ++p) {
        dst[p] = V3{0.0f, 0.0f, 0.0f};
        if (valid[p]) {
            const u3_t t = reinterpret_cast<const u3_t*>(plane)[slot[p]];
            dst[p] = V3{u2f(t.x), u2f(t.y), u2f(t.z)};
        }
    }
}
template <int P>
__device__ __forceinline__ void pin_store3(const V3 (&src)[P], char* plane, const uint32_t (&slot)[P], const bool (&valid)[P], bool dense) {
    if constexpr (P == 4) {
        if (dense) {
            u4v* dst = reinterpret_cast<u4v*>(plane) + (size_t)(slot[0] >> 2) * 3;
            HNB_NT_STORE((u4v{f2u(src[0].x), f2u(src[0].y), f2u(src[0].z), f2u(src[1].x)}), dst);
            HNB_NT_STORE((u4v{f2u(src[1].y), f2u(src[1].z), f2u(src[2].x), f2u(src[2].y)}), dst + 1);
            HNB_NT_STORE((u4v{f2u(src[2].z), f2u(src[3].x), f2u(src[3].y), f2u(src[3].z)}), dst + 2);
            return;
        }
    }
    if constexpr (P == 4) {
        u4v* dst = reinterpret_cast<u4v*>(plane) + (size_t)(slot[0] >> 2) * 3;
        u4v q0 = dst[0], q1 = dst[1], q2 = dst[2];
        if (valid[0]) { q0.x = f2u(src[0].x); q0.y = f2u(src[0].y); q0.z = f2u(src[0].z); }
        if (valid[1]) { q0.w = f2u(src[1].x); q1.x = f2u(src[1].y); q1.y = f2u(src[1].z); }
        if (valid[2]) { q1.z = f2u(src[2].x); q1.w = f2u(src[2].y); q2.x = f2u(src[2].z); }
        if (valid[3]) { q2.y = f2u(src[3].x); q2.z = f2u(src[3].y); q2.w = f2u(src[3].z); }
        dst[0] = q0; dst[1] = q1; dst[2] = q2;
        return;
    }
#pragma unroll
    for (int p = 0; p < P; ++p)
        if (valid[p]) reinterpret_cast<u3_t*>(plane)[slot[p]] = u3_t{f2u(src[p].x), f2u(src[p].y), f2u(src[p].z)};
}
template <int P>
__device__ __forceinline__ void pin_load1(float (&dst)[P], const char* plane, const uint32_t (&slot)[P], const bool (&valid)[P], bool dense) {
    if constexpr (P == 4) {
        if (dense) {
// ... 525 lines not shown
    soff_t alive_flag_off;
    uint32_t update_len;
    soff_t plane_off[4];
    uint32_t flags;
    soff_t died_bits_off;
    uint32_t write_died;
    uint32_t cull_lifetime;
    soff_t lmin_off;
    uint32_t dt_operand;
    uint32_t age_cohort;
    soff_t horizon_off;
    uint32_t horizon;
    uint32_t frame_phase;
    const Ins* update_code;
    uint32_t* safe_words;
    unsigned long long* safe_host;
    uint32_t safe_parity, publish_tag, safe_stride;
    uint32_t skip_lists;
    const DevMeta* meta_in;
    DevMeta* meta_out;
    uint32_t* fault;
    uint32_t transpose;
    uint32_t stream_hint;
    uint32_t store_hint;
    uint32_t quarters;
    uint32_t age_current;
    uint32_t fuse_steps;
};




__device__ __forceinline__ void store_died_bits(uint32_t* __restrict__ bits, uint32_t step_first, uint32_t nib, uint32_t lane) {
    int v = (int)(nib << (4u * (lane & 7u)));
    v |= __builtin_amdgcn_update_dpp(0, v, 0xB1, 0xf, 0xf, true);
    v |= __builtin_amdgcn_update_dpp(0, v, 0x4E, 0xf, 0xf, true);
    v |= __builtin_amdgcn_update_dpp(0, v, 0x141, 0xf, 0xf, true);
    if ((lane & 7u) == 0u) bits[(step_first >> 5) + (lane >> 3)] = (uint32_t)v;
}

struct StreamLds {
    uint32_t died[kBlock / 64];
    float lmin[kBlock / 64];
    uint32_t alive[kBlock / 64];
    float rem[kBlock / 64];
    uint32_t amin[kBlock / 64], amax[kBlock / 64];
    u4v xp[2][kBlock / 64][kStepRows * 3u / 4u];
};
__device__ __forceinline__ StreamLds& stream_lds() {
    __shared__ StreamLds s;
    return s;
}

template <class PROG, int PROBE, bool COHORT, bool FUSED = false>
__device__ __forceinline__ void update_stream_chunk(const SlotArgs& args, const uint64_t* __restrict__ inst_base, const DevFrameInst* __restrict__ fi,
                                                    const uint32_t* __restrict__ ublocks, const CompactBufs& cb,
                                                    const uint32_t wg, const uint32_t wg_total) {
    StreamLds& lds = stream_lds();
    uint32_t (&s_died)[kBlock / 64] = lds.died;
    float (&s_lmin)[kBlock / 64] = lds.lmin;
    uint32_t (&s_alive)[kBlock / 64] = lds.alive;
    float (&s_rem)[kBlock / 64] = lds.rem;
    uint32_t (&s_amin)[kBlock / 64] = lds.amin;
    uint32_t (&s_amax)[kBlock / 64] = lds.amax;
    u4v (&s_xp)[2][kBlock / 64][kStepRows * 3u / 4u] = lds.xp;
    const uint32_t tid = threadIdx.x, lane = tid & 63u, wave = tid >> 6;
    const bool split = !FUSED && !COHORT && args.quarters == 4u;
    const uint32_t S = FUSED ? args.fuse_steps : 1u;
    const uint32_t chunk = split ? chunk_of_workgroup(cb.xcd_remap, wg >> 2, wg_total >> 2) : chunk_of_workgroup(cb.xcd_remap, wg, wg_total);
    const uint32_t quarter = split ? (wg & 3u) : 0u;
    const uint32_t k = chunk / args.chunks_per_inst, j = chunk - k * args.chunks_per_inst;
    const uint32_t wave0 = j * kChunk + (split ? (quarter * (kBlock / 64u) + wave) * kStepRows : wave * kWaveRows);
    const uint32_t n_steps = split ? 1u : kWaveRows / kStepRows;
    const uint32_t n_words = split ? wg_total >> 2 : wg_total;
    const uint32_t frozen = fi[k].skip;
    const uint64_t slab = inst_base[k];
    const bool store_nt = args.store_hint != 0u;
#ifndef HNB_PUBLISH_FIRST_WG
#define HNB_PUBLISH_FIRST_WG 1
#endif
    if (args.safe_words && (HNB_PUBLISH_FIRST_WG ? wg == 0u : chunk == 0u)) {
        uint32_t* prev = args.safe_words + (size_t)(args.safe_parity ^ 1u) * args.safe_stride;
        uint32_t m = 0x7f800000u;
        for (uint32_t i = tid; i < n_words; i += kBlock) { const uint32_t v = prev[i]; prev[i] = 0x7f800000u; m = v < m ? v : m; }
        m = wave_min_u32(m);
        if (lane == 0) s_alive[wave] = m;
        __syncthreads();
        if (tid == 0u) {
            for (uint32_t w = 1; w < kBlock / 64; ++w) m = s_alive[w] < m ? s_alive[w] : m;
            *reinterpret_cast<volatile unsigned long long*>(args.safe_host) = ((unsigned long long)m << 32) | (unsigned long long)args.publish_tag;
        }
        __syncthreads();
    }
    if (args.skip_lists && j == 0u && quarter == 0u && tid == 0u) {
        DevMeta o = args.meta_in[k];
        if constexpr (FUSED) {
            DevMeta before = o;
            if (!frozen) {
                o.max_update = o.alive_count; o.dead_count = 0u; o.spawned = 0u; o.instance_count = o.alive_count;
                before = o;
                o.ref_write_index ^= S & 1u;
                before.ref_write_index ^= (S - 1u) & 1u;
            }
            DevMeta* row_in = const_cast<DevMeta*>(args.meta_in);
            ((S & 1u) ? args.meta_out : row_in)[k] = o;
            ((S & 1u) ? row_in : args.meta_out)[k] = before;
            cb.deaths[(size_t)(cb.parity ^ 1u) * cb.table_cap + k] = 0u;
        } else {
        if (!frozen) {
            o.ref_write_index ^= 1u;
            o.max_update = o.alive_count; o.dead_count = 0u; o.spawned = 0u; o.instance_count = o.alive_count;
        }
        args.meta_out[k] = o;
        cb.deaths[(size_t)(cb.parity ^ 1u) * cb.table_cap + k] = 0u;
        }
    }
    if (frozen) return;
    char* base = global_ptr<char>(slab);
    VmUniforms U;
    U.u = ublocks + (size_t)k * args.n_uregs * S;
    auto uniforms_of = [&](const uint32_t s) { VmUniforms Us = U; Us.u = U.u + (size_t)s * args.n_uregs; return Us; };
    U.xf = fi[k].xf;
    float rem_min = __builtin_inff();
    char* p_pos = base + args.plane_off[0];
    char* p_vel = base + args.plane_off[1];
    char* p_age = base + args.plane_off[2];
    char* p_life = base + args.plane_off[3];
    uint32_t* flags4 = reinterpret_cast<uint32_t*>(base + args.alive_flag_off);
    const uint32_t fl = args.flags;
    uint32_t died_total = 0;
    uint32_t* cfull = reinterpret_cast<uint32_t*>(base + args.lmin_off) + args.chunks_per_inst;
    const bool chunk_full = cfull[j] == 1u;
    uint32_t* astate = cfull + args.chunks_per_inst;
    uint32_t* aval = astate + args.chunks_per_inst;
    const uint32_t ast_raw = COHORT ? astate[j] : 0u;
    bool check_due = ((args.frame_phase + j) & 15u) == 0u;
    if constexpr (FUSED) {
        for (uint32_t s = 1; s < S; ++s) check_due = check_due || ((args.frame_phase + s + j) & 15u) == 0u;
    }
    const bool mixed = COHORT && ast_raw == 4u && !check_due;
    const uint32_t ast = ast_raw == 4u ? 0u : ast_raw;
    const float A = COHORT ? u2f(aval[j]) : 0.0f;
    uint32_t amin = 0xffffffffu, amax = 0u;
    uint32_t lane_alive = 0;
    const bool cull = args.cull_lifetime != 0u;
    float* lmin = reinterpret_cast<float*>(base + args.lmin_off);
    const float Lm = cull ? lmin[j] : 0.0f;
    const float dt_tick = cull ? uf(U, args.dt_operand) : 0.0f;
    auto age_after = [&](float a) {
        if constexpr (FUSED) {
            for (uint32_t s = 0; s < S; ++s) a = a + uf(uniforms_of(s), args.dt_operand);
            return a;
        } else return a + dt_tick;
    };
    if (args.horizon && j == 0u && quarter == 0u && tid == 0u) {
        double* clk = horizon_view(base, args.horizon_off, args.chunks_per_inst).clock;
        if constexpr (FUSED) {
            double c = *clk;
            for (uint32_t s = 0; s < S; ++s) { const float t = cull ? uf(uniforms_of(s), args.dt_operand) : 0.0f; c = c + (double)(t > 0.0f ? t : 0.0f) * (1.0 + 0x1p-16); }
            *clk = c;
        } else
        *clk = *clk + (double)(dt_tick > 0.0f ? dt_tick : 0.0f) * (1.0 + 0x1p-16);
    }
    float wave_min = __builtin_inff();
    bool loaded_all = true;
    bool flat = false;
    if constexpr (PROG::kFlat && COHORT && PROBE == 0) {
        flat = chunk_full && ast == 1u && cull && Lm > 0.0f && (age_after(A) < Lm) && (fl & 3u) == 3u && !(fl & 128u);
    }
    if (flat) {
        if constexpr (PROG::kFlat && COHORT && PROBE == 0) {
            const float A2 = age_after(A);
            u4v* pw = reinterpret_cast<u4v*>(p_pos + (size_t)j * (kChunk * 12u)) + wave * (kWaveRows * 3u / 4u);
            u4v* vw = reinterpret_cast<u4v*>(p_vel + (size_t)j * (kChunk * 12u)) + wave * (kWaveRows * 3u / 4u);
            const uint32_t rot = lane % 3u;
            if (args.age_current && (fl & 64u)) {
                u4v* aw = reinterpret_cast<u4v*>(p_age + (size_t)j * (kChunk * 4u)) + wave * (kWaveRows / 4u);
                const uint32_t a2 = f2u(A2);
#pragma unroll
                for (uint32_t step = 0; step < kWaveRows / kStepRows; ++step) aw[step * 64u + lane] = u4v{a2, a2, a2, a2};
            }
#pragma unroll 2
            for (uint32_t step = 0; step < kWaveRows / kStepRows; ++step) {
                float P[3][4], V[3][4];
#pragma unroll
                for (uint32_t w = 0; w < 3; ++w) {
                    const u4v a = pw[(step * 3u + w) * 64u + lane], b = vw[(step * 3u + w) * 64u + lane];
                    P[w][0] = u2f(a.x); P[w][1] = u2f(a.y); P[w][2] = u2f(a.z); P[w][3] = u2f(a.w);
                    V[w][0] = u2f(b.x); V[w][1] = u2f(b.y); V[w][2] = u2f(b.z); V[w][3] = u2f(b.w);
                }
                if constexpr (FUSED) {
                    for (uint32_t s = 0; s < S; ++s) PROG::run_flat(args.update_code, P, V, rot, uniforms_of(s));
                } else
                PROG::run_flat(args.update_code, P, V, rot, U);
#pragma unroll
                for (uint32_t w = 0; w < 3; ++w) {
                    if (fl & 16u) pw[(step * 3u + w) * 64u + lane] = u4v{f2u(P[w][0]), f2u(P[w][1]), f2u(P[w][2]), f2u(P[w][3])};
                    if (fl & 32u) vw[(step * 3u + w) * 64u + lane] = u4v{f2u(V[w][0]), f2u(V[w][1]), f2u(V[w][2]), f2u(V[w][3])};
                }
            }
            if (args.write_died && lane < kWaveRows / 32u)
                reinterpret_cast<uint32_t*>(base + args.died_bits_off)[((j * kChunk + wave * kWaveRows) >> 5) + lane] = 0u;
            amin = amax = f2u(A2);
            loaded_all = false;
            if (args.safe_words) rem_min = (f2u(A2) >> 31) ? 0.0f : (Lm - A2) - 1.0e-5f * Lm;
        }
    }
    auto step_body = [&](auto coh_tag, const uint32_t step, const uint32_t f4, const u4v* pre_age = nullptr) {
        constexpr bool COH = decltype(coh_tag)::value;
        const uint32_t s0 = wave0 + step * kStepRows + lane * 4u;
        bool was[4], fresh[4];
#pragma unroll
        for (int p = 0; p < 4; ++p) {
            const uint32_t byte = (f4 >> (8 * p)) & 0xffu;
            fresh[p] = COH && byte == 3u;
            was[p] = byte == 1u || fresh[p];
            lane_alive += was[p] ? 1u : 0u;
        }
        const bool any = was[0] || was[1] || was[2] || was[3];
        if (!__any(any)) {
            if (args.write_died) store_died_bits(reinterpret_cast<uint32_t*>(base + args.died_bits_off), s0 - lane * 4u, 0u, lane);
            return;
        }
        const bool full = was[0] && was[1] && was[2] && was[3];
        uint32_t slot[4];
#pragma unroll
        for (int p = 0; p < 4; ++p) slot[p] = s0 + p;
        bool lanes_on[4] = {any, any, any, any};
        Pinned<4> X;
#pragma unroll
        for (int p = 0; p < 4; ++p) { X.pos[p] = V3{0, 0, 0}; X.vel[p] = V3{0, 0, 0}; X.age[p] = 0.0f; X.lifetime[p] = 0.0f; X.alive[p] = true; }
        bool need_life = true;
        float age_was[4] = {0.0f, 0.0f, 0.0f, 0.0f};
        const uint32_t step_first = s0 - lane * 4u;
        const bool xp = args.transpose != 0u && PROBE == 0 && step_first + kStepRows <= args.capacity && __popcll(__ballot(any)) >= 32;
        if (xp) {
            if (fl & 1u) xpose_load3(X.pos, p_pos, step_first, s_xp[0][wave], lane);
            if (fl & 2u) xpose_load3(X.vel, p_vel, step_first, s_xp[1][wave], lane);
        }
        if (any) {
            if (!xp) {
                if (fl & 1u) pin_load3<4>(X.pos, p_pos, slot, lanes_on, true);
                if (fl & 2u) pin_load3<4>(X.vel, p_vel, slot, lanes_on, true);
            }
            if (fl & 4u) {
                if (!COH || ast != 1u) {
                    if (pre_age) { X.age[0] = u2f(pre_age->x); X.age[1] = u2f(pre_age->y); X.age[2] = u2f(pre_age->z); X.age[3] = u2f(pre_age->w); }
                    else pin_load1<4>(X.age, p_age, slot, lanes_on, true);
                    for (int p = 0; p < 4; ++p) age_was[p] = X.age[p];
                }
                if (COH && ast != 0u) {
#pragma unroll
                    for (int p = 0; p < 4; ++p) X.age[p] = fresh[p] ? X.age[p] : A;
                }
            }
        }
        if (cull && Lm > 0.0f && (COH || !mixed)) {
            bool may_die = false;
#pragma unroll
            for (int p = 0; p < 4; ++p) may_die = may_die || (was[p] && !(age_after(X.age[p]) < Lm));
            need_life = __any(may_die);
        }
        if (any && (fl & 8u)) {
            if (need_life) {
                if (args.stream_hint) {
                    const u4v ql = __builtin_nontemporal_load(reinterpret_cast<const u4v*>(p_life) + (slot[0] >> 2));
                    X.lifetime[0] = u2f(ql.x); X.lifetime[1] = u2f(ql.y); X.lifetime[2] = u2f(ql.z); X.lifetime[3] = u2f(ql.w);
                } else pin_load1<4>(X.lifetime, p_life, slot, lanes_on, true);
            }
            else {
#pragma unroll
                for (int p = 0; p < 4; ++p) X.lifetime[p] = Lm;
            }
        }
        if (!need_life) loaded_all = false;
        if constexpr (FUSED) {
            bool gone[4] = {false, false, false, false};
            for (uint32_t s = 0; s < S; ++s) {
                PROG::template run<4>(args.update_code, args.update_len, X, uniforms_of(s));
#pragma unroll
                for (int p = 0; p < 4; ++p) gone[p] = gone[p] || !X.alive[p];
            }
#pragma unroll
            for (int p = 0; p < 4; ++p) X.alive[p] = !gone[p];
        } else
        if constexpr (!(PROBE & 8)) PROG::template run<4>(args.update_code, args.update_len, X, U);
        if constexpr (!(PROBE & 4)) {
            const bool xp_pos = xp && (fl & 17u) == 17u, xp_vel = xp && (fl & 34u) == 34u;
            if (xp_pos) xpose_store3(X.pos, p_pos, step_first, s_xp[0][wave], lane, was, full, store_nt);
            if (xp_vel) xpose_store3(X.vel, p_vel, step_first, s_xp[1][wave], lane, was, full, store_nt);
            if (any) {
                if ((fl & 16u) && !xp_pos) pin_store3<4>(X.pos, p_pos, slot, was, full);
                if ((fl & 32u) && !xp_vel) pin_store3<4>(X.vel, p_vel, slot, was, full);
                if (fl & 64u) {
                    const bool plane_loaded = !COH || ast != 1u;
                    if (plane_loaded || args.age_current) {
                        if (plane_loaded && (fl & 4u) && !full) {
                            float q[4];
#pragma unroll
                            for (int p = 0; p < 4; ++p) q[p] = was[p] ? X.age[p] : age_was[p];
                            pin_store1<4>(q, p_age, slot, was, true, store_nt);
                        } else pin_store1<4>(X.age, p_age, slot, was, full, store_nt);
                    }
                }
                if (fl & 128u) pin_store1<4>(X.lifetime, p_life, slot, was, full);
            }
        } else {
            float acc = 0.0f;
#pragma unroll
            for (int p = 0; p < 4; ++p) acc += X.pos[p].x + X.pos[p].y + X.pos[p].z + X.vel[p].x + X.vel[p].y + X.vel[p].z + X.age[p] + X.lifetime[p];
            if (acc == 123.456f) X.alive[0] = false;
        }
        if (cull && need_life) {
#pragma unroll
            for (int p = 0; p < 4; ++p)
                if (was[p] && X.alive[p]) wave_min = fminf(wave_min, X.lifetime[p]);
        }
        if (args.safe_words) {
#pragma unroll
            for (int p = 0; p < 4; ++p)
                if (was[p] && X.alive[p]) rem_min = fminf(rem_min, (f2u(X.age[p]) >> 31) ? 0.0f : (X.lifetime[p] - X.age[p]) - 1.0e-5f * X.lifetime[p]);
        }
        if constexpr (COH) {
#pragma unroll
            for (int p = 0; p < 4; ++p) {
                const bool stays = was[p] && X.alive[p];
                const uint32_t b = f2u(X.age[p]);
                amin = (stays && b < amin) ? b : amin;
                amax = (stays && b > amax) ? b : amax;
            }
            if constexpr (!(PROBE & 4)) {
                const bool dies = (was[0] && !X.alive[0]) || (was[1] && !X.alive[1]) || (was[2] && !X.alive[2]) || (was[3] && !X.alive[3]);
                if (ast == 1u && (fl & 64u) && !args.age_current && __any(dies)) {
#pragma unroll
                    for (int p = 0; p < 4; ++p)
                        if (was[p] && !X.alive[p]) reinterpret_cast<float*>(p_age)[slot[p]] = X.age[p];
                }
            }
        }
        uint32_t nf = f4, nib = 0u;
        uint32_t died_here = 0;
#pragma unroll
        for (int p = 0; p < 4; ++p) {
            const bool died = was[p] && !X.alive[p];
            if (died) { nf &= ~(0xffu << (8 * p)); nib |= 1u << p; }
            else if (COH && fresh[p]) nf = (nf & ~(0xffu << (8 * p))) | (1u << (8 * p));
            died_here += (uint32_t)__popcll(__ballot(died));
        }
        if (nf != f4) flags4[s0 >> 2] = nf;
        if (args.write_died) store_died_bits(reinterpret_cast<uint32_t*>(base + args.died_bits_off), step_first, nib, lane);
        died_total += died_here;
    };
    if (!flat) {
        auto f4_of = [&](const uint32_t step) {
            const uint32_t s0 = wave0 + step * kStepRows + lane * 4u;
            return chunk_full ? 0x01010101u : (s0 < args.capacity ? ld_hint(flags4 + (s0 >> 2), args.stream_hint != 0u) : 0u);
        };
        if constexpr (COHORT || PROG::kFlat) {
            uint32_t f4s[kWaveRows / kStepRows];
#pragma unroll
            for (uint32_t step = 0; step < kWaveRows / kStepRows; ++step) f4s[step] = step < n_steps ? f4_of(step) : 0u;
            if constexpr (PROG::kAgeOnly && !COHORT) {
                if ((fl & 4u) && !(fl & 3u)) {
                    u4v ages[kWaveRows / kStepRows];
#pragma unroll
                    for (uint32_t step = 0; step < kWaveRows / kStepRows; ++step) {
                        const uint32_t s0 = wave0 + step * kStepRows + lane * 4u;
                        ages[step] = (step < n_steps && s0 < args.capacity) ? reinterpret_cast<const u4v*>(p_age)[s0 >> 2] : u4v{0u, 0u, 0u, 0u};
                    }
#pragma unroll
                    for (uint32_t step = 0; step < kWaveRows / kStepRows; ++step) if (step < n_steps) step_body(BoolTag<false>{}, step, f4s[step], &ages[step]);
                    goto steps_done;
                }
            }
            if (mixed) {
#pragma unroll
                for (uint32_t step = 0; step < kWaveRows / kStepRows; ++step) if (step < n_steps) step_body(BoolTag<false>{}, step, f4s[step]);
            } else {
#pragma unroll
                for (uint32_t step = 0; step < kWaveRows / kStepRows; ++step) if (step < n_steps) step_body(BoolTag<COHORT>{}, step, f4s[step]);
            }
        } else {
#pragma unroll
            for (uint32_t step = 0; step < kWaveRows / kStepRows; ++step) if (step < n_steps) step_body(BoolTag<false>{}, step, f4_of(step));
        }
    }
steps_done:
    if (cull) wave_min = wave_min_f32(wave_min);
    if (!chunk_full) lane_alive = wave_sum_u32(lane_alive);
    if (lane == 0) s_alive[wave] = lane_alive;
    if (args.safe_words) {
        rem_min = wave_min_f32(rem_min);
        if (lane == 0) s_rem[wave] = rem_min;
    }
    if constexpr (COHORT) {
        amin = wave_min_u32(amin); amax = wave_max_u32(amax);
        if (lane == 0) { s_amin[wave] = amin; s_amax[wave] = amax; }
    }
    if (lane == 0) { s_died[wave] = died_total; s_lmin[wave] = loaded_all ? wave_min : -1.0f; }
    lds_barrier();
    if (tid == 0) {
        if (COHORT && !mixed) {
            uint32_t lo = 0xffffffffu, hi = 0u;
#pragma unroll
            for (uint32_t w = 0; w < kBlock / 64; ++w) { lo = s_amin[w] < lo ? s_amin[w] : lo; hi = s_amax[w] > hi ? s_amax[w] : hi; }
            const uint32_t next = (lo == hi) ? 1u : (lo > hi ? 0u : 4u);
            if (next == 1u) aval[j] = lo;
            if (next != ast_raw) astate[j] = next;
        }
        uint32_t d = 0;
#pragma unroll
        for (uint32_t w = 0; w < kBlock / 64; ++w) d += s_died[w];
        if (d) atomicAdd(&cb.deaths[(size_t)cb.parity * cb.table_cap + k], d);
        if (d && args.skip_lists) *args.fault = 1u;
        if (args.safe_words) {
            float r = fminf(fminf(s_rem[0], s_rem[1]), fminf(s_rem[2], s_rem[3]));
            r = r > 0.0f ? r : 0.0f;
            uint32_t* word = args.safe_words + (size_t)args.safe_parity * args.safe_stride + chunk;
            if (split) atomicMin(word, f2u(r));
            else *word = f2u(r);
        }
        if (chunk_full) { if (d) cfull[j] = 0u; }
        else if (!split && d == 0u && s_alive[0] + s_alive[1] + s_alive[2] + s_alive[3] == kChunk) cfull[j] = 1u;
        if (cull && !split) {
            float m = __builtin_inff();
            bool all = true;
#pragma unroll
            for (uint32_t w = 0; w < kBlock / 64; ++w) { all = all && !(s_lmin[w] < 0.0f); m = fminf(m, s_lmin[w]); }
            if (all) lmin[j] = m < 3.0e38f ? m : 3.0e38f;
        }
    }
}

template <class PROG, int WAVES, int PROBE = 0, bool COHORT = false, bool FUSED = false>
__global__ void __launch_bounds__(kBlock, WAVES)
k_update_slots_stream(const SlotArgs args, const uint64_t* __restrict__ inst_base, const DevFrameInst* __restrict__ fi,
                      const uint32_t* __restrict__ ublocks, const CompactBufs cb) {
    update_stream_chunk<PROG, PROBE, COHORT, FUSED>(args, inst_base, fi, ublocks, cb, blockIdx.x, gridDim.x);
}
#ifndef HNB_JIT_TU
#ifndef HNB_AGEK_CUT
#define HNB_AGEK_CUT 0
#endif
__global__ void __launch_bounds__(kBlock)
k_update_slots_stream_age(const SlotArgs args, const uint64_t* __restrict__ inst_base, const DevFrameInst* __restrict__ fi,
                          const uint32_t* __restrict__ ublocks, const CompactBufs cb) {
    __shared__ uint32_t s_died[kBlock / 64], s_alive[kBlock / 64];
    __shared__ float s_lmin[kBlock / 64], s_rem[kBlock / 64];
    constexpr uint32_t kSteps = kWaveRows / kStepRows;
    const uint32_t tid = threadIdx.x, lane = tid & 63u, wave = tid >> 6;
    const uint32_t wg = blockIdx.x, wg_total = gridDim.x;
    const uint32_t chunk = chunk_of_workgroup(cb.xcd_remap, wg, wg_total);
    const uint32_t k = chunk / args.chunks_per_inst, j = chunk - k * args.chunks_per_inst;
    const uint32_t frozen = fi[k].skip;
    char* base = global_ptr<char>(inst_base[k]);
    const float dt_tick = u2f(ublocks[(size_t)k * args.n_uregs + (args.dt_operand & 0xffu)]);
    char* p_age = base + args.plane_off[2];
    const char* p_life = base + args.plane_off[3];
    uint32_t* flags4 = reinterpret_cast<uint32_t*>(base + args.alive_flag_off);
    float* lmin = reinterpret_cast<float*>(base + args.lmin_off);
    uint32_t* cfull = reinterpret_cast<uint32_t*>(lmin) + args.chunks_per_inst;
    const uint32_t wave0 = j * kChunk + wave * kWaveRows;
    uint32_t f4s[kSteps];
    u4v ages[kSteps];
#pragma unroll
    for (uint32_t step = 0; step < kSteps; ++step) {
        const uint32_t s0 = wave0 + step * kStepRows + lane * 4u;
        const bool in = s0 < args.capacity;
        f4s[step] = in ? ld_hint(flags4 + (s0 >> 2), args.stream_hint != 0u) : 0u;
        ages[step] = in ? reinterpret_cast<const u4v*>(p_age)[s0 >> 2] : u4v{0u, 0u, 0u, 0u};
    }
    const uint32_t cf = cfull[j];
    const float Lm = lmin[j];
    if (!(HNB_AGEK_CUT & 1) && args.safe_words && wg == 0u) {
        uint32_t* prev = args.safe_words + (size_t)(args.safe_parity ^ 1u) * args.safe_stride;
        uint32_t m = 0x7f800000u;
        for (uint32_t i = tid; i < wg_total; i += kBlock) { const uint32_t v = prev[i]; prev[i] = 0x7f800000u; m = v < m ? v : m; }
        m = wave_min_u32(m);
        if (lane == 0) s_alive[wave] = m;
        __syncthreads();
        if (tid == 0u) {
            for (uint32_t w = 1; w < kBlock / 64; ++w) m = s_alive[w] < m ? s_alive[w] : m;
            *reinterpret_cast<volatile unsigned long long*>(args.safe_host) = ((unsigned long long)m << 32) | (unsigned long long)args.publish_tag;
        }
        __syncthreads();
    }
    if (args.skip_lists && j == 0u && tid == 0u) {
        DevMeta o = args.meta_in[k];
        if (!frozen) {
            o.ref_write_index ^= 1u;
            o.max_update = o.alive_count; o.dead_count = 0u; o.spawned = 0u; o.instance_count = o.alive_count;
// ... 402 lines not shown
```

### bevy_hanabi_amd/csrc/hnb_plan.h

```cpp
#pragma once
#include <cstdint>
#include <cstring>

namespace hnb {
namespace plan {

struct InstanceFrame {
    bool simulated = true;
    bool has_parent = false;
    uint32_t spawn_count = 0;
    uint32_t event_capacity = 0;
    const uint32_t* ublock = nullptr;
};
inline uint32_t uword(const InstanceFrame& f, uint32_t decoded_operand) { return f.ublock[decoded_operand & 0xffu]; }
inline float as_float(uint32_t bits) { float f; std::memcpy(&f, &bits, 4); return f; }
inline bool nonneg_not_nan(uint32_t float_bits) { return float_bits <= 0x7f800000u; }

struct SkipFacts {
    bool eligible = false;
    uint32_t dt_operand = 0;
};
struct SkipHistory {
    double cum_tick[128] = {};
    uint32_t last_dirty = 0;
// ... 124 lines not shown
    d.ring = option_ring && d.suffix && (d.rotate || d.max_spawn == 0u);
    return d;
}

inline bool horizon_usable(bool eligible, uint32_t dt_operand, const InstanceFrame* inst, uint32_t n) {
    if (!eligible) return false;
    for (uint32_t i = 0; i < n; ++i)
        if (inst[i].simulated && (uword(inst[i], dt_operand) & 0x7f800000u) == 0x7f800000u) return false;
    return true;
}

struct InitGridInputs {
    bool simulated = true, has_parent = false;
    uint32_t spawn_count = 0, event_capacity = 0;
    bool events_known = false;
    uint32_t known_events = 0;
};
inline uint32_t size_init_grid(const InitGridInputs& in, uint32_t capacity, uint32_t init_block, uint32_t rounds_if_big, bool big_burst, uint32_t num_cus) {
    uint32_t request = in.simulated ? in.spawn_count : 0u;
    if (in.has_parent && in.simulated) {
        request = in.event_capacity;
        if (in.events_known) request = in.known_events < in.event_capacity ? in.known_events : in.event_capacity;
    }
    const uint32_t capped = request < capacity ? request : capacity;
    uint32_t blocks = (uint32_t)(((uint64_t)capped + init_block - 1u) / init_block);
    if (big_burst) blocks = (blocks + rounds_if_big - 1u) / rounds_if_big;
    if (in.has_parent) blocks = blocks < num_cus * 8u ? blocks : num_cus * 8u;
    return blocks;
}
inline uint32_t size_event_grid(uint32_t max_event_capacity, uint32_t total_chunks) {
    const uint32_t per_chunk = max_event_capacity / (total_chunks ? total_chunks : 1u);
    const uint32_t splits = (per_chunk + 16383u) / 16384u;
    return splits < 1u ? 1u : (splits > 64u ? 64u : splits);
}

struct SlotInitDecision { bool use = false, marks = false; };
constexpr uint32_t kSlotInitMinChunks = 17;
inline SlotInitDecision plan_slot_init(bool eligible, uint32_t option, uint32_t capacity, uint32_t chunks_per_inst, const InstanceFrame* inst, uint32_t n) {
    SlotInitDecision d;
    if (!eligible || option == 0u || n == 0u || (option == 1u && (uint64_t)n * chunks_per_inst < kSlotInitMinChunks)) return d;
    uint64_t spawns = 0;
    bool partial = false;
    for (uint32_t i = 0; i < n; ++i) {
        if (inst[i].has_parent) return d;
        if (!inst[i].simulated || inst[i].spawn_count == 0u) continue;
        spawns += inst[i].spawn_count < capacity ? inst[i].spawn_count : capacity;
        partial = partial || inst[i].spawn_count < capacity;
    }
    d.use = spawns != 0u && (option >= 2u || spawns * 8u >= (uint64_t)n * capacity);
    d.marks = d.use && partial;
    return d;
}

struct MergeFacts {
    bool independent = false;
    uint32_t total_chunks = 0;
    uint32_t init_blocks = 0;
    uint32_t init_len = 0, update_len = 0;
    bool wide_file = false, update_streams = false, age_cohort = false;
};
enum UpdateFamily : int8_t { kNotMerged = -1, kStream = 0, kStreamCohort = 1, kGeneric = 2, kGenericWide = 3 };
struct MergeDecision { int8_t init_family = -1;  int8_t update_family = kNotMerged; };
struct MergeLimits { uint32_t max_chunks = 16, max_init_blocks = 64, max_code_len = 64; };

inline void plan_merged_launches(const MergeFacts* progs, MergeDecision* out, uint32_t n, bool option_enabled, bool timed_frame, MergeLimits lim = MergeLimits()) {
    for (uint32_t i = 0; i < n; ++i) out[i] = MergeDecision();
    if (!option_enabled || timed_frame || n < 2u) return;
    auto small = [&](const MergeFacts& p) { return p.independent && p.total_chunks <= lim.max_chunks; };
    auto init_family = [&](const MergeFacts& p) -> int { return small(p) && p.init_blocks != 0u && p.init_blocks <= lim.max_init_blocks && p.init_len <= lim.max_code_len ? (p.wide_file ? 1 : 0) : -1; };
    auto update_family = [&](const MergeFacts& p) -> int {
        if (!small(p) || p.update_len > lim.max_code_len) return kNotMerged;
        if (p.update_streams) return p.age_cohort ? kStreamCohort : kStream;
        return p.wide_file ? kGenericWide : kGeneric;
    };
    uint32_t n_init[2] = {0, 0}, n_upd[4] = {0, 0, 0, 0};
    for (uint32_t i = 0; i < n; ++i) {
        const int fi = init_family(progs[i]), fu = update_family(progs[i]);
        if (fi >= 0) n_init[fi] += 1;
        if (fu >= 0) n_upd[fu] += 1;
    }
    const bool shared_update = n_upd[kStream] + n_upd[kStreamCohort] + n_upd[kGeneric] >= 2u;
    for (uint32_t i = 0; i < n; ++i) {
        const int fi = init_family(progs[i]), fu = update_family(progs[i]);
        if (fi >= 0 && n_init[fi] >= 2u) out[i].init_family = (int8_t)fi;
        if (fu == kGenericWide ? n_upd[kGenericWide] >= 2u : (fu >= 0 && shared_update)) out[i].update_family = (int8_t)fu;
    }
}

inline void split_uncovered(const MergeDecision* dec, const uint8_t* has_case, const uint8_t* has_own_kernels, uint32_t n, bool module_loaded, uint8_t* out) {
    for (uint32_t i = 0; i < n; ++i) out[i] = 0u;
    if (!module_loaded) return;
    auto in_set_launch = [&](uint32_t i) { return dec[i].init_family == 0 || (dec[i].update_family >= 0 && dec[i].update_family != kGenericWide); };
    uint32_t covered = 0, uncovered = 0;
    for (uint32_t i = 0; i < n; ++i) {
        if (!in_set_launch(i)) continue;
        if (has_case[i]) covered += 1; else uncovered += 1;
    }
    if (uncovered == 0u || covered < 2u || covered < 4u * uncovered) return;
    for (uint32_t i = 0; i < n; ++i)
        if (in_set_launch(i) && !has_case[i] && has_own_kernels[i]) out[i] = 1u;
}

inline void partition_init_passes(const uint8_t* reads, uint32_t n, int heavy, uint8_t* side) {
    for (uint32_t i = 0; i < n; ++i) side[i] = heavy >= 0 ? 1u : 0u;
    if (heavy < 0) return;
    side[heavy] = 0u;
// ... 15 lines not shown
    if (population != st.seen) { st.seen = population; return false; }
    st.tried = population;
    return true;
}

constexpr uint64_t kStreamHintBytes = 256ull << 20;
inline bool use_streaming_hints(uint64_t total_slots, uint32_t update_bytes_per_slot) {
    return total_slots * (uint64_t)(update_bytes_per_slot + 8u) > kStreamHintBytes;
}

constexpr uint64_t kStoreHintBytes = 384ull << 20;
inline bool use_store_hints(uint64_t total_slots, uint32_t stored_bytes_per_slot) { return total_slots * (uint64_t)stored_bytes_per_slot > kStoreHintBytes; }

constexpr uint32_t kStageSlots = 16, kStageGroup = 4, kStageGroups = kStageSlots / kStageGroup;
constexpr int kStageWaitNone = -1, kStageWaitStream = -2;
struct StageRing {
    uint32_t staged = 0;
    uint32_t recorded = 0;
    bool torn = false;
};
struct StageStep { uint32_t slot = 0; int wait = kStageWaitNone; };
inline StageStep stage_ring_begin(const StageRing& r, bool stages) {
    StageStep st;
    if (!stages) return st;
    st.slot = r.staged % kStageSlots;
    const uint32_t g = st.slot / kStageGroup;
    if (r.torn) st.wait = kStageWaitStream;
    else if (st.slot % kStageGroup == 0u && (r.recorded >> g & 1u)) st.wait = (int)g;
    return st;
}
inline void stage_ring_drained(StageRing& r) { r.recorded = 0u; r.torn = false; }
inline int stage_ring_end(StageRing& r, bool stages, bool written, bool ok) {
    if (!stages) return kStageWaitNone;
    if (!ok) { r.torn = r.torn || written; return kStageWaitNone; }
    const uint32_t slot = r.staged % kStageSlots, g = slot / kStageGroup;
    r.staged += 1u;
    if (slot % kStageGroup != kStageGroup - 1u) return kStageWaitNone;
    r.recorded |= 1u << g;
    return (int)g;
}

struct FramePlan {
    bool skip_lists = false;
    bool lists = true;
    bool lists_merged = false;
    bool hz_use = false;
    bool stream_hint = false;
    bool store_hint = false;
    RibbonDecision ribbon;
    bool independent = false;
    MergeDecision merge;
    uint32_t init_blocks = 0;
    SlotInitDecision slot_init;
};

}
}
```

### bevy_hanabi_amd/runtime.py

```python
import ctypes as C
import os

import numpy as np

from . import build as _build

HNB_OK = 0
HNB_ERR_NO_DEVICE = -4
HNB_ERR_NOT_FOUND = -6

ATTR_COMPONENTS = [1, 1, 3, 3, 1, 1, 1, 4, 1, 1, 2, 3, 1, 1, 3, 3, 3, 1, 1, 1, 1, 1, 2, 2, 2, 2, 3, 3, 3, 3, 4, 4, 4, 4, 1, 1, 1, 1, 1]
ATTR_IS_FLOAT = [0, 0, 1, 1, 1, 1, 0, 1, 1, 1, 1, 1, 0, 0, 1, 1, 1, 0] + [1] * 16 + [0] * 5

ABI_SYMBOLS = [
    "hnb_last_error", "hnb_version", "hnb_ctx_create", "hnb_ctx_destroy", "hnb_ctx_set_stream", "hnb_ctx_synchronize",
    "hnb_program_create", "hnb_program_destroy", "hnb_program_validate", "hnb_effect_create", "hnb_effect_destroy",
    "hnb_effect_set_parent", "hnb_frame_begin", "hnb_effect_set_frame", "hnb_effect_set_property", "hnb_simulate",
    "hnb_effect_metadata", "hnb_effect_alive_count", "hnb_effect_read_attr", "hnb_effect_read_alive_list",
    "hnb_effect_read_dead_list", "hnb_effect_write_attr", "hnb_effect_sort_ribbons", "hnb_ctx_enable_kernel_timing",
    "hnb_ctx_kernel_timing", "hnb_program_kernel_info", "hnb_jit_precompile", "hnb_effect_set_simulated", "hnb_ctx_set_option", "hnb_program_set_frames", "hnb_effect_index",
    "hnb_ctx_profile_marker", "hnb_program_kernel_timing",
    "hnb_comm_create_local", "hnb_comm_unique_id", "hnb_comm_create_rank", "hnb_comm_allreduce_alive", "hnb_comm_destroy", "hnb_comm_set_library",
    "hnb_effect_device_view", "hnb_effect_materialise", "hnb_jit_precompile_set", "hnb_effect_check", "hnb_effect_compare", "hnb_comm_describe", "hnb_program_device_view",
    "hnb_simulate_steps", "hnb_effect_set_frames_ahead", "hnb_program_set_frames_ahead", "hnb_ctx_step_stats",
    "hnb_program_prepare_steps", "hnb_jit_precompile_steps",
    "hnb_effect_export", "hnb_program_export", "hnb_effect_export_sorted", "hnb_program_export_sorted",
    "hnb_effect_export_filtered", "hnb_effect_export_filtered_sorted", "hnb_program_export_filtered",
    "hnb_effect_bounds", "hnb_program_bounds",
]
ABI_BINNED_SYMBOLS = ["hnb_effect_export_binned"]

OPTIONS = {"list_order": 1, "alternate": 2, "skip_lists": 3, "age_cohort": 4, "cull_lifetime": 5, "horizon": 6, "transpose": 7, "scene_merge": 8,
           "suffix_proof": 9, "overlap_updates": 10, "stream_hints": 11, "set_module": 12, "jit_async": 13, "test_break_proof": 15, "ring_lists": 16, "slot_init": 17, "direct_upload": 18, "fuse_steps": 19}
MAX_FUSED_STEPS = 8
SET_MODULE_OFF, SET_MODULE_CACHED, SET_MODULE_COMPILE, SET_MODULE_BACKGROUND = 0, 1, 2, 3


class HanabiError(RuntimeError):
    def __init__(self, code, message):
        super().__init__(f"[{code}] {message}")
        self.code = code


class SimParams(C.Structure):
    _fields_ = [("delta_time", C.c_float), ("time", C.c_float), ("virtual_delta_time", C.c_float), ("virtual_time", C.c_float),
                ("real_delta_time", C.c_float), ("real_time", C.c_float)]


class EffectMetadata(C.Structure):
    _fields_ = [(n, C.c_uint32) for n in ("capacity", "alive_count", "max_update", "max_spawn", "indirect_write_index",
                                          "particle_counter", "instance_count", "dispatch_x", "dead_count", "spawned", "fault",
                                          "reserved")]

    def as_dict(self):
        return {n: int(getattr(self, n)) for n, _ in self._fields_ if n != "reserved"}


class StepStats(C.Structure):
    _fields_ = [(n, C.c_uint64) for n in ("frames", "fused_frames", "fused_launches", "update_launches", "list_launches")]

    def as_dict(self):
        return {n: int(getattr(self, n)) for n, _ in self._fields_}


class DeviceMeta(C.Structure):
    _fields_ = [(n, C.c_uint32) for n in ("alive_count", "particle_counter", "list_column", "max_update", "dead_count", "spawned",
                                          "indirect_write_index", "instance_count")]


class EffectCheck(C.Structure):
    _fields_ = [(n, C.c_uint32) for n in ("ok", "capacity", "alive_count", "bad_slots", "duplicate_slots", "alive_byte_mismatches", "alive_past_lifetime", "fault")]

    def as_dict(self):
        return {n: int(getattr(self, n)) for n, _ in self._fields_}


class EffectDiff(C.Structure):
    _fields_ = [("equal", C.c_uint32), ("counter_diffs", C.c_uint32), ("alive_list_diffs", C.c_uint64), ("dead_list_diffs", C.c_uint64), ("attr_diffs", C.c_uint64),
                ("first_section", C.c_int32), ("reserved", C.c_uint32), ("first_index", C.c_uint64)]

    def as_dict(self):
        return {n: int(getattr(self, n)) for n, _ in self._fields_ if n != "reserved"}


class DeviceAttr(C.Structure):
    _fields_ = [("attr", C.c_uint16), ("ncomp", C.c_uint8), ("scalar_type", C.c_uint8), ("stride_bytes", C.c_uint16), ("reserved", C.c_uint16),
                ("plane", C.c_void_p)]


class DeviceView(C.Structure):
    _fields_ = [("struct_size", C.c_uint32), ("device", C.c_int32), ("stream", C.c_void_p),
                ("capacity", C.c_uint32), ("slot_base", C.c_uint32), ("n_attrs", C.c_uint32), ("reserved", C.c_uint32),
                ("stale_attr_mask", C.c_uint64), ("alive_list", C.c_void_p * 2), ("dead_list", C.c_void_p),
                ("meta", C.c_void_p), ("meta_next", C.c_void_p), ("attrs", DeviceAttr * 40)]

    def plane(self, attr_id):
        for i in range(self.n_attrs):
            if self.attrs[i].attr == int(attr_id):
                return self.attrs[i]
        raise KeyError(attr_id)


class ProgramAttr(C.Structure):
    _fields_ = [("attr", C.c_uint16), ("ncomp", C.c_uint8), ("scalar_type", C.c_uint8), ("stride_bytes", C.c_uint16), ("reserved", C.c_uint16),
                ("plane_off", C.c_uint64)]


class ProgramView(C.Structure):
    _fields_ = [("struct_size", C.c_uint32), ("device", C.c_int32), ("stream", C.c_void_p),
                ("capacity", C.c_uint32), ("n_instances", C.c_uint32), ("n_attrs", C.c_uint32), ("reserved", C.c_uint32),
                ("stale_attr_mask", C.c_uint64), ("slabs", C.c_void_p), ("meta", C.c_void_p), ("meta_next", C.c_void_p),
                ("alive_list_off", C.c_uint64 * 2), ("dead_list_off", C.c_uint64), ("attrs", ProgramAttr * 40)]
# ... 138 lines not shown
        if not os.path.exists(path):
            raise HanabiError(-1, f"{path} not found: run `python -m bevy_hanabi_amd.build` (needs hipcc)")
        lib = C.CDLL(path)
        lib.hnb_last_error.restype = C.c_char_p
        lib.hnb_version.restype = C.c_char_p
        lib.hnb_ctx_create.argtypes = [C.c_int, C.POINTER(C.c_void_p)]
        lib.hnb_ctx_destroy.argtypes = [C.c_void_p]
        lib.hnb_ctx_set_stream.argtypes = [C.c_void_p, C.c_void_p]
        lib.hnb_ctx_synchronize.argtypes = [C.c_void_p]
        lib.hnb_program_create.argtypes = [C.c_void_p, C.c_char_p, C.c_size_t, C.POINTER(C.c_void_p)]
        lib.hnb_program_destroy.argtypes = [C.c_void_p]
        lib.hnb_program_validate.argtypes = [C.c_char_p, C.c_size_t]
        lib.hnb_effect_create.argtypes = [C.c_void_p, C.c_uint32, C.POINTER(C.c_void_p)]
        lib.hnb_effect_destroy.argtypes = [C.c_void_p]
        lib.hnb_effect_set_parent.argtypes = [C.c_void_p, C.c_void_p, C.c_uint32, C.c_uint32]
        lib.hnb_frame_begin.argtypes = [C.c_void_p, C.POINTER(SimParams)]
        lib.hnb_effect_set_frame.argtypes = [C.c_void_p, C.c_uint32, C.c_uint32, C.c_void_p]
        lib.hnb_effect_set_property.argtypes = [C.c_void_p, C.c_char_p, C.c_void_p, C.c_uint32]
        lib.hnb_simulate.argtypes = [C.c_void_p]
        lib.hnb_effect_metadata.argtypes = [C.c_void_p, C.POINTER(EffectMetadata)]
        lib.hnb_effect_alive_count.argtypes = [C.c_void_p, C.POINTER(C.c_uint32)]
        lib.hnb_effect_read_attr.argtypes = [C.c_void_p, C.c_uint32, C.c_void_p, C.c_size_t]
        lib.hnb_effect_write_attr.argtypes = [C.c_void_p, C.c_uint32, C.c_void_p, C.c_size_t]
        lib.hnb_effect_read_alive_list.argtypes = [C.c_void_p, C.c_void_p, C.c_size_t]
        lib.hnb_effect_read_dead_list.argtypes = [C.c_void_p, C.c_void_p, C.c_size_t]
        lib.hnb_effect_sort_ribbons.argtypes = [C.c_void_p]
        lib.hnb_ctx_enable_kernel_timing.argtypes = [C.c_void_p, C.c_int]
        lib.hnb_ctx_kernel_timing.argtypes = [C.c_void_p, C.POINTER(C.c_double), C.POINTER(C.c_double), C.POINTER(C.c_double), C.POINTER(C.c_uint32)]
        lib.hnb_effect_set_simulated.argtypes = [C.c_void_p, C.c_int]
        lib.hnb_ctx_set_option.argtypes = [C.c_void_p, C.c_uint32, C.c_uint32]
        lib.hnb_program_set_frames.argtypes = [C.c_void_p, C.c_uint32, C.c_uint32, C.c_void_p, C.c_void_p, C.c_void_p]
        lib.hnb_effect_index.argtypes = [C.c_void_p, C.POINTER(C.c_uint32)]
        lib.hnb_ctx_profile_marker.argtypes = [C.c_void_p, C.c_uint32]
        lib.hnb_program_kernel_timing.argtypes = [C.c_void_p, C.POINTER(C.c_double), C.POINTER(C.c_double), C.POINTER(C.c_double), C.POINTER(C.c_uint32)]
        lib.hnb_comm_create_local.argtypes = [C.POINTER(C.c_void_p), C.c_uint32, C.POINTER(C.c_void_p)]
        lib.hnb_comm_unique_id.argtypes = [C.c_void_p]
        lib.hnb_comm_create_rank.argtypes = [C.c_void_p, C.c_void_p, C.c_uint32, C.c_uint32, C.POINTER(C.c_void_p)]
        lib.hnb_comm_allreduce_alive.argtypes = [C.c_void_p, C.POINTER(C.c_void_p), C.c_uint32, C.POINTER(C.c_uint64)]
        lib.hnb_comm_destroy.argtypes = [C.c_void_p]
        lib.hnb_comm_set_library.argtypes = [C.c_char_p, C.c_uint32]
        lib.hnb_program_device_view.argtypes = [C.c_void_p, C.POINTER(ProgramView)]
        lib.hnb_comm_describe.argtypes = [C.c_void_p, C.c_char_p, C.c_size_t]
        lib.hnb_effect_check.argtypes = [C.c_void_p, C.POINTER(EffectCheck)]
        lib.hnb_effect_compare.argtypes = [C.c_void_p, C.c_void_p, C.POINTER(EffectDiff)]
        lib.hnb_effect_device_view.argtypes = [C.c_void_p, C.POINTER(DeviceView)]
        lib.hnb_effect_materialise.argtypes = [C.c_void_p, C.c_uint64]
        lib.hnb_program_kernel_info.argtypes = [C.c_void_p, C.c_char_p, C.c_size_t]
        lib.hnb_jit_precompile.argtypes = [C.c_char_p, C.c_size_t]
        lib.hnb_jit_precompile_set.argtypes = [C.POINTER(C.c_char_p), C.POINTER(C.c_size_t), C.c_uint32]
        lib.hnb_simulate_steps.argtypes = [C.c_void_p, C.c_uint32, C.POINTER(SimParams)]
        lib.hnb_effect_set_frames_ahead.argtypes = [C.c_void_p, C.c_uint32, C.c_void_p, C.c_void_p, C.c_void_p]
        lib.hnb_program_set_frames_ahead.argtypes = [C.c_void_p, C.c_uint32, C.c_uint32, C.c_uint32, C.c_void_p, C.c_void_p, C.c_void_p]
        lib.hnb_ctx_step_stats.argtypes = [C.c_void_p, C.POINTER(StepStats)]
        lib.hnb_program_prepare_steps.argtypes = [C.c_void_p]
        lib.hnb_jit_precompile_steps.argtypes = [C.c_char_p, C.c_size_t]
        lib.hnb_effect_export.argtypes = [C.c_void_p, C.POINTER(ExportDesc)]
        lib.hnb_program_export.argtypes = [C.c_void_p, C.POINTER(ExportDesc), C.c_void_p]
        lib.hnb_effect_export_sorted.argtypes = [C.c_void_p, C.POINTER(ExportDesc), C.POINTER(ExportSort)]
        lib.hnb_program_export_sorted.argtypes = [C.c_void_p, C.POINTER(ExportDesc), C.POINTER(ExportSort), C.c_uint32, C.c_void_p]
        lib.hnb_effect_export_filtered.argtypes = [C.c_void_p, C.POINTER(ExportDesc), C.POINTER(ExportFilter)]
        lib.hnb_effect_export_filtered_sorted.argtypes = [C.c_void_p, C.POINTER(ExportDesc), C.POINTER(ExportFilter), C.POINTER(ExportSort)]
        lib.hnb_program_export_filtered.argtypes = [C.c_void_p, C.POINTER(ExportDesc), C.POINTER(ExportFilter), C.c_uint32, C.c_void_p]
        lib.hnb_effect_bounds.argtypes = [C.c_void_p, C.POINTER(BoundsDesc)]
        lib.hnb_program_bounds.argtypes = [C.c_void_p, C.POINTER(BoundsDesc)]
        lib.hnb_effect_export_binned.argtypes = [C.c_void_p, C.POINTER(ExportDesc), C.POINTER(ExportBins)]
        _lib = lib
    return _lib


def _check(rc):
    if rc != HNB_OK:
        raise HanabiError(rc, load_library().hnb_last_error().decode())


def validate_program(blob: bytes):
    _check(load_library().hnb_program_validate(blob, len(blob)))


def jit_precompile(blob: bytes):
    _check(load_library().hnb_jit_precompile(blob, len(blob)))


def jit_precompile_steps(blob: bytes):
    _check(load_library().hnb_jit_precompile_steps(blob, len(blob)))


def jit_precompile_set(blobs):
    blobs = list(blobs)
    arr = (C.c_char_p * len(blobs))(*blobs)
    sizes = (C.c_size_t * len(blobs))(*[len(b) for b in blobs])
    _check(load_library().hnb_jit_precompile_set(arr, sizes, len(blobs)))


class Context:

    def __init__(self, device_id=0):
        self._lib = load_library()
        self._h = C.c_void_p()
        _check(self._lib.hnb_ctx_create(device_id, C.byref(self._h)))
        self._programs = []
        for kv in filter(None, os.environ.get("HNB_CTX_OPTIONS", "").split(",")):
            k, v = kv.split("=")
            self.set_option(k.strip(), int(v))

    def close(self):
        if self._h:
            for p in list(self._programs):
                p._h = None
                for e in p._effects:
                    e._h = None
            self._lib.hnb_ctx_destroy(self._h)
            self._h = None

    def __del__(self):
        try:
            self.close()
        except Exception:
            pass

    def set_stream(self, hip_stream):
        _check(self._lib.hnb_ctx_set_stream(self._h, C.c_void_p(hip_stream)))

    def synchronize(self):
        _check(self._lib.hnb_ctx_synchronize(self._h))

    def set_list_order(self, order):
        _check(self._lib.hnb_ctx_set_option(self._h, 1, {"spawn": 0, "slot": 1}[order]))

    def set_option(self, option, value):
        _check(self._lib.hnb_ctx_set_option(self._h, OPTIONS[option] if isinstance(option, str) else int(option), int(value)))

    def create_program(self, blob: bytes):
        return Program(self, blob)

    def frame_begin(self, dt, time=0.0, virtual_dt=None, virtual_time=None, real_dt=None, real_time=None):
        sp = SimParams(dt, time, dt if virtual_dt is None else virtual_dt, time if virtual_time is None else virtual_time,
                       dt if real_dt is None else real_dt, time if real_time is None else real_time)
        _check(self._lib.hnb_frame_begin(self._h, C.byref(sp)))

    def simulate(self):
        _check(self._lib.hnb_simulate(self._h))

    def simulate_steps(self, params_list):
        steps = []
        for e in params_list:
            if isinstance(e, SimParams):
                steps.append(e)
                continue
            a = tuple(e) if isinstance(e, (tuple, list)) else (e,)
            dt, time = a[0], (a[1] if len(a) > 1 else 0.0)
            rest = list(a[2:]) + [None] * (6 - len(a))
            steps.append(SimParams(dt, time, dt if rest[0] is None else rest[0], time if rest[1] is None else rest[1],
                                   dt if rest[2] is None else rest[2], time if rest[3] is None else rest[3]))
        arr = (SimParams * max(len(steps), 1))(*steps)
        _check(self._lib.hnb_simulate_steps(self._h, len(steps), arr))

    def step_stats(self):
        s = StepStats()
        _check(self._lib.hnb_ctx_step_stats(self._h, C.byref(s)))
        return s.as_dict()

    def enable_kernel_timing(self, every_n_frames=1):
        _check(self._lib.hnb_ctx_enable_kernel_timing(self._h, int(every_n_frames)))

    def profile_marker(self, tag):
        _check(self._lib.hnb_ctx_profile_marker(self._h, int(tag)))

    def kernel_timing(self):
        u, c, i, n = C.c_double(), C.c_double(), C.c_double(), C.c_uint32()
        _check(self._lib.hnb_ctx_kernel_timing(self._h, C.byref(u), C.byref(c), C.byref(i), C.byref(n)))
        return {"update_ms_avg": u.value, "compact_ms_avg": c.value, "init_ms_avg": i.value, "frames": n.value}


def comm_set_library(path, duplicate_devices=False, single_rank=False):
    _check(load_library().hnb_comm_set_library(None if path is None else os.fsencode(path), (1 if duplicate_devices else 0) | (2 if single_rank else 0)))


class Comm:

    def __init__(self, handle, contexts):
        self._lib = load_library()
        self._h = handle
        self._contexts = list(contexts)

    @classmethod
    def local(cls, contexts):
        lib = load_library()
        arr = (C.c_void_p * len(contexts))(*[c._h for c in contexts])
        h = C.c_void_p()
        _check(lib.hnb_comm_create_local(arr, len(contexts), C.byref(h)))
        return cls(h, contexts)

    @staticmethod
    def unique_id():
        buf = C.create_string_buffer(128)
        _check(load_library().hnb_comm_unique_id(buf))
        return buf.raw

    @classmethod
    def rank(cls, ctx, unique_id, rank, n_ranks):
        lib = load_library()
        h = C.c_void_p()
        _check(lib.hnb_comm_create_rank(ctx._h, C.c_char_p(unique_id), int(rank), int(n_ranks), C.byref(h)))
        return cls(h, [ctx])

    def allreduce_alive(self, effects_per_context):
        n = len(effects_per_context[0])
        assert len(effects_per_context) == len(self._contexts) and all(len(e) == n for e in effects_per_context)
        flat = [None if fx is None else fx._h for row in effects_per_context for fx in row]
        arr = (C.c_void_p * len(flat))(*flat)
        out = (C.c_uint64 * n)()
        _check(self._lib.hnb_comm_allreduce_alive(self._h, arr, n, out))
        return [int(v) for v in out]

# ... 229 lines not shown
```

### include/hanabi_amd.h

```cpp
#ifndef HANABI_AMD_H
#define HANABI_AMD_H

#ifndef __HIPCC_RTC__
#include <stddef.h>
#include <stdint.h>
#endif

#ifdef __cplusplus
extern "C" {
#endif

typedef enum HnbStatus {
    HNB_OK = 0,
    HNB_ERR_INVALID_ARG = -1,
    HNB_ERR_BAD_PROGRAM = -2,
    HNB_ERR_HIP = -3,
    HNB_ERR_NO_DEVICE = -4,
    HNB_ERR_OUT_OF_MEMORY = -5,
    HNB_ERR_NOT_FOUND = -6,
    HNB_ERR_DEVICE_FAULT = -7
} HnbStatus;

typedef enum HnbAttr {
    HNB_ATTR_ID = 0, HNB_ATTR_PARTICLE_COUNTER = 1,
// ... 135 lines not shown
    uint32_t capacity;
    uint32_t alive_count;
    uint32_t max_update;
    uint32_t max_spawn;
    uint32_t indirect_write_index;
    uint32_t particle_counter;
    uint32_t instance_count;
    uint32_t dispatch_x;
    uint32_t dead_count;
    uint32_t spawned;
    uint32_t fault;
    uint32_t reserved;
} HnbEffectMetadata;

typedef struct HnbContext HnbContext;
typedef struct HnbProgram HnbProgram;
typedef struct HnbEffect HnbEffect;

const char* hnb_last_error(void);
const char* hnb_version(void);

int hnb_ctx_create(int device_id, HnbContext** out_ctx);
int hnb_ctx_destroy(HnbContext* ctx);
int hnb_ctx_set_stream(HnbContext* ctx, void* hip_stream);
int hnb_ctx_synchronize(HnbContext* ctx);
#define HNB_OPT_LIST_ORDER 1u
#define HNB_LIST_ORDER_SPAWN 0u
#define HNB_LIST_ORDER_SLOT 1u
#define HNB_OPT_ALTERNATE 2u
#define HNB_OPT_SKIP_LISTS 3u
#define HNB_OPT_AGE_COHORT 4u
#define HNB_AGE_COHORT_OFF 0u
#define HNB_AGE_COHORT_LEAN 1u
#define HNB_AGE_COHORT_ALL 2u
#define HNB_AGE_COHORT_AUTO 3u
#define HNB_OPT_CULL_LIFETIME 5u
#define HNB_OPT_HORIZON 6u
#define HNB_OPT_TRANSPOSE 7u
#define HNB_OPT_SCENE_MERGE 8u
#define HNB_OPT_SUFFIX_PROOF 9u
#define HNB_OPT_RING_LISTS 16u
#define HNB_OPT_SLOT_INIT 17u
#define HNB_OPT_DIRECT_UPLOAD 18u
#define HNB_OPT_OVERLAP_UPDATES 10u
#define HNB_OPT_STREAM_HINTS 11u
#define HNB_OPT_JIT_ASYNC 13u
#define HNB_OPT_TEST_BREAK_PROOF 15u
#define HNB_OPT_SET_MODULE 12u
#define HNB_SET_MODULE_OFF 0u
#define HNB_SET_MODULE_CACHED 1u
#define HNB_SET_MODULE_COMPILE 2u
#define HNB_SET_MODULE_BACKGROUND 3u
#define HNB_OPT_FUSE_STEPS 19u
#define HNB_MAX_FUSED_STEPS 8u
int hnb_ctx_set_option(HnbContext* ctx, uint32_t option, uint32_t value);

int hnb_program_create(HnbContext* ctx, const void* blob, size_t blob_size, HnbProgram** out_prog);
int hnb_program_destroy(HnbProgram* prog);
int hnb_program_validate(const void* blob, size_t blob_size);

int hnb_effect_create(HnbProgram* prog, uint32_t slot_base, HnbEffect** out_fx);
int hnb_effect_destroy(HnbEffect* fx);
int hnb_effect_set_parent(HnbEffect* child, HnbEffect* parent, uint32_t channel, uint32_t event_capacity);

int hnb_frame_begin(HnbContext* ctx, const HnbSimParams* params);
int hnb_effect_set_frame(HnbEffect* fx, uint32_t spawn_count, uint32_t seed, const float* transform3x4);
int hnb_program_set_frames(HnbProgram* prog, uint32_t first, uint32_t count, const uint32_t* spawn_counts, const uint32_t* seeds,
                           const float* transforms3x4);
int hnb_effect_index(HnbEffect* fx, uint32_t* out_index);
int hnb_effect_set_simulated(HnbEffect* fx, int simulated);
int hnb_effect_set_property(HnbEffect* fx, const char* name, const void* value, uint32_t n_words);

int hnb_simulate(HnbContext* ctx);

int hnb_simulate_steps(HnbContext* ctx, uint32_t n_steps, const HnbSimParams* params );
int hnb_program_prepare_steps(HnbProgram* prog);
int hnb_effect_set_frames_ahead(HnbEffect* fx, uint32_t n_steps, const uint32_t* spawn_counts, const uint32_t* seeds, const float* transforms3x4);
int hnb_program_set_frames_ahead(HnbProgram* prog, uint32_t first, uint32_t count, uint32_t n_steps, const uint32_t* spawn_counts, const uint32_t* seeds,
                                 const float* transforms3x4);
typedef struct HnbStepStats {
    uint64_t frames;
    uint64_t fused_frames;
    uint64_t fused_launches;
    uint64_t update_launches;
    uint64_t list_launches;
} HnbStepStats;
int hnb_ctx_step_stats(HnbContext* ctx, HnbStepStats* out);

typedef struct HnbDeviceMeta {
    uint32_t alive_count;
    uint32_t particle_counter;
    uint32_t list_column;
    uint32_t max_update;
    uint32_t dead_count, spawned;
    uint32_t indirect_write_index;
    uint32_t instance_count;
} HnbDeviceMeta;
typedef struct HnbDeviceAttr {
    uint16_t attr;
    uint8_t ncomp, scalar_type;
    uint16_t stride_bytes;
    uint16_t reserved;
    void* plane;
} HnbDeviceAttr;
#define HNB_VIEW_MAX_ATTRS 40u
typedef struct HnbDeviceView {
// ... 173 lines not shown
```

Before: 125.0 billion.

## Fuse slot-major spawn init into the streaming update kernel

Adds a JIT-specialised spawn kernel that performs the per-slot init stores for newborn particles inside the streaming update pass. The separate init-slots pass then only marks rows, and the update skips reloading freshly written attributes. The goal is to avoid a second full sweep over the newly spawned particle planes each frame. The cost is a more complex update kernel with extra template paths and registers, plus a JIT build the first time it is needed. It is disabled on timed frames and for merged or multi-step programs.

Measured after the change: 121.7 billion. 0.973x the previous value.

```diff
diff --git a/bevy_hanabi_amd/__init__.py b/bevy_hanabi_amd/__init__.py
--- a/bevy_hanabi_amd/__init__.py
+++ b/bevy_hanabi_amd/__init__.py
@@ -10,4 +10,4 @@
         raise ImportError("bevy_hanabi_amd._hanabi_host could not be built: run `python -m bevy_hanabi_amd.build`") from _e
 from . import _hanabi_host as host
 
-from .runtime import Comm, Context, Effect, EffectMetadata, HanabiError, Program, SimParams, jit_precompile, jit_precompile_set, jit_precompile_steps, validate_program
+from .runtime import Comm, Context, Effect, EffectMetadata, HanabiError, Program, SimParams, jit_precompile, jit_precompile_set, jit_precompile_spawn, jit_precompile_steps, validate_program
diff --git a/bevy_hanabi_amd/build.py b/bevy_hanabi_amd/build.py
--- a/bevy_hanabi_amd/build.py
+++ b/bevy_hanabi_amd/build.py
@@ -150,7 +150,7 @@
 
 def build_runtime(force=False, verbose=False):
     srcs = [os.path.join(_CSRC, "hanabi_amd.hip")] + sorted(os.path.join(_CSRC, f) for f in os.listdir(_CSRC) if f.endswith(".h"))
-    srcs += [os.path.join(_DIR, "..", "include", h) for h in ("hanabi_amd.h", "hanabi_amd_binned.h")]
+    srcs += [os.path.join(_DIR, "..", "include", h) for h in ("hanabi_amd.h", "hanabi_amd_binned.h", "hanabi_amd_spawn.h")]
     for build_code in EXPORT_CODE_OBJECTS + BINNED_CODE_OBJECTS + QUERY_CODE_OBJECTS:
         srcs.append(build_code(force, verbose))
     out = runtime_lib_path()
diff --git a/bevy_hanabi_amd/csrc/hanabi_amd.hip b/bevy_hanabi_amd/csrc/hanabi_amd.hip
--- a/bevy_hanabi_amd/csrc/hanabi_amd.hip
+++ b/bevy_hanabi_amd/csrc/hanabi_amd.hip
@@ -31,6 +31,7 @@
 #include "hnb_export_bin.h"
 #include "hnb_export_bin_code.inc"
 #include "hnb_bounds.h"
+#include "../../include/hanabi_amd_spawn.h"
 #include "hnb_bounds_code.inc"
 
 using namespace hnb;
@@ -160,6 +161,7 @@
     std::vector<Ins> steps_ops;
     int steps_waves = 0;
     bool steps_cohort = false;
+    bool spawn = false;
     jit::Result res;
     bool ok = false;
 };
@@ -227,6 +229,8 @@
     uint32_t set_failed_builds = 0;
     std::string set_log;
     bool fuse_steps = true;
+    bool fuse_spawn = true;
+    HnbFusedSpawnStats spawn_stats{};
     HnbStepStats step_stats{};
     hipModule_t export_module[kExportUnitCount] = {};
     hipFunction_t export_fn[kExpKernelCount] = {};
@@ -275,6 +279,16 @@
     std::vector<Ins> steps_ops;
     int steps_waves = 0;
     bool steps_cohort = false;
+    std::vector<uint8_t> spawn_blob;
+    bool spawn_aot_static = false;
+    ProgramOptions spawn_opt;
+    enum class SpawnState { NotRequested, Built, Pending, Failed };
+    hipModule_t spawn_module = nullptr;
+    hipFunction_t spawn_update = nullptr;
+    SpawnState spawn_state = SpawnState::NotRequested;
+    bool spawn_from_cache = false;
+    std::string spawn_why, spawn_kernel_name;
+    uint32_t fused_spawn_frames = 0;
     std::vector<Ins> h_init, h_update;
     std::string set_sig;
     uint64_t set_sig_hash = 0;
@@ -910,6 +924,55 @@
     p->steps_from_cache = res.from_cache;
     p->steps_state = HnbProgram::StepsState::Built;
 }
+void spawn_build_failed(HnbProgram* p, const std::string& log) {
+    p->spawn_state = HnbProgram::SpawnState::Failed;
+    p->spawn_why = log.substr(0, log.find('\n'));
+    if (p->spawn_why.empty()) p->spawn_why = "no log";
+    p->jit_log += (p->jit_log.empty() ? "" : "\n") + std::string("spawn kernel: ") + log;
+}
+void install_program_spawn(HnbProgram* p, const jit::Result& res) {
+    hipModule_t mod = nullptr;
+    hipFunction_t fu = nullptr;
+    hipError_t je = hipModuleLoadData(&mod, res.code.data());
+    if (je == hipSuccess) je = hipModuleGetFunction(&fu, mod, res.update_name.c_str());
+    if (je != hipSuccess) {
+        if (mod) hipModuleUnload(mod);
+        (void)hipGetLastError();
+        spawn_build_failed(p, std::string("loading the code object failed: ") + hipGetErrorString(je));
+        return;
+    }
+    p->spawn_module = mod; p->spawn_update = fu;
+    p->spawn_kernel_name = res.update_name;
+    p->spawn_from_cache = res.from_cache;
+    p->spawn_state = HnbProgram::SpawnState::Built;
+}
+bool spawn_module_wanted(const HnbProgram* p, const jit::Request& rq) {
+    return p->update_streams && rq.want_init && rq.want_init_slots && rq.update_len != 0u;
+}
+void queue_jit_job(HnbContext* ctx, std::unique_ptr<JitJob> job);
+void request_spawn_kernel(HnbContext* ctx, HnbProgram* p) {
+    if (p->spawn_state != HnbProgram::SpawnState::NotRequested || p->spawn_blob.empty()) return;
+    const uint8_t* b = p->spawn_blob.data();
+    const HnbProgramHeader& h = p->hdr;
+    const bool aot_static = p->spawn_aot_static;
+    const ProgramOptions& opt = p->spawn_opt;
+    const jit::Request rq = make_jit_request(b, h, p->attrs.data(), p->update_streams, aot_static, opt);
+    const bool async = ctx->jit_async;
+    jit::Result res;
+    if (jit::build_spawn(rq, res, async)) {
+        install_program_spawn(p, res);
+    } else if (async && res.log.empty()) {
+        std::unique_ptr<JitJob> job(new JitJob());
+        job->program_serial = p->serial;
+        job->spawn = true;
+        job->blob = p->spawn_blob;
+        job->hdr = h; job->attrs = p->attrs; job->streams = p->update_streams; job->aot_static = aot_static; job->opt = opt;
+        queue_jit_job(ctx, std::move(job));
+        p->spawn_state = HnbProgram::SpawnState::Pending;
+    } else {
+        spawn_build_failed(p, res.log);
+    }
+}
 const char* steps_never_reason(const HnbProgram* p) {
     if (!p->update_streams) return "never fuses: not a macro-op update";
     if (!p->skip_facts.eligible) return "never fuses: particles can die by more than their lifetime, or the program is linked to others";
@@ -961,6 +1024,8 @@
         }
         if (job->steps) {
             job->ok = jit::build_steps(make_steps_request(job->steps_ops, job->steps_waves, job->steps_cohort), job->res);
+        } else if (job->spawn) {
+            job->ok = jit::build_spawn(make_jit_request(job->blob.data(), job->hdr, job->attrs.data(), job->streams, job->aot_static, job->opt), job->res);
         } else {
             const jit::Request rq = make_jit_request(job->blob.data(), job->hdr, job->attrs.data(), job->streams, job->aot_static, job->opt);
             job->ok = jit::build(rq, job->res);
@@ -988,6 +1053,11 @@
         if (j->steps) {
             if (j->ok) install_program_steps(p, j->res);
             else steps_build_failed(p, j->res.log);
+            continue;
+        }
+        if (j->spawn) {
+            if (j->ok) install_program_spawn(p, j->res);
+            else spawn_build_failed(p, j->res.log);
             continue;
         }
         p->jit_pending = false;
@@ -1120,6 +1190,7 @@
         case HNB_OPT_DIRECT_UPLOAD: ctx->direct_upload = value != 0u; return HNB_OK;
         case HNB_OPT_JIT_ASYNC: ctx->jit_async = value != 0u; return HNB_OK;
         case HNB_OPT_FUSE_STEPS: ctx->fuse_steps = value != 0u; return HNB_OK;
+        case HNB_OPT_FUSE_SPAWN: ctx->fuse_spawn = value != 0u; return HNB_OK;
         case HNB_OPT_SET_MODULE:
             if (value > HNB_SET_MODULE_BACKGROUND) return fail(HNB_ERR_INVALID_ARG, "unknown set-module mode %u", value);
             ctx->set_mode = value;
@@ -1211,6 +1282,11 @@
             p->jit_log = res.log;
         }
     }
+    if (jit::enabled() && spawn_module_wanted(p, make_jit_request(b, h, p->attrs.data(), p->update_streams, aot_static, ctx->popt))) {
+        p->spawn_blob.assign(b, b + blob_size);
+        p->spawn_aot_static = aot_static;
+        p->spawn_opt = ctx->popt;
+    }
     if (p->has_ribbons && p->update_streams) {
         bool ok = true;
         uint32_t ticks = 0;
@@ -1315,6 +1391,7 @@
     free_tables(p);
     if (p->jit_module) hipModuleUnload(p->jit_module);
     if (p->steps_module) hipModuleUnload(p->steps_module);
+    if (p->spawn_module) hipModuleUnload(p->spawn_module);
     for (auto& blk : p->slab_blocks) hipFree(blk.base);
     hipFree(p->d_plane_by_attr);
     hipFree(p->d_code);
@@ -2164,12 +2241,16 @@
                 const uint32_t grid = n * p->dev.chunks_per_inst * (kChunk / kSlotInitWg);
                 const DevMeta* mi = p->d_meta[par];
                 if (p->plan.slot_init.marks) k_spawn_mark<<<grid, kBlock, 0, st>>>(p->dev, p->d_inst_base, mi, dfi);
-                if (p->jit_init_slots) {
+                if (p->plan.fused_spawn) {
+                    k_init_slots<InterpCode, true><<<grid, kBlock, 0, st>>>(p->dev, p->d_inst_base, mi, dfi, dub);
+                    ctx->spawn_stats.rows_launches += 1;
+                } else if (p->jit_init_slots) {
                     void* ka[] = {&p->dev, &p->d_inst_base, &mi, &dfi, &dub};
                     HIP_TRY(hipModuleLaunchKernel(p->jit_init_slots, grid, 1, 1, kBlock, 1, 1, 0, st, ka, nullptr));
                 } else if (p->wide_file) k_init_slots<InterpCodeWide><<<grid, kBlock, 0, st>>>(p->dev, p->d_inst_base, mi, dfi, dub);
                 else k_init_slots<InterpCode><<<grid, kBlock, 0, st>>>(p->dev, p->d_inst_base, mi, dfi, dub);
                 p->slot_init_frames += 1;
+                if (!p->plan.fused_spawn) ctx->spawn_stats.unfused_frames += 1;
             } else if (p->jit_init) {
                 const DevMeta* mi = p->d_meta[par];
                 void* ka[] = {&p->dev, &p->d_inst_base, &mi, &dfi, &dub};
@@ -2219,6 +2300,12 @@
             ctx->step_stats.fused_launches += 1;
             ctx->step_stats.fused_frames += p->fuse_span;
             p->fused_frames += p->fuse_span;
+        } else if (p->plan.fused_spawn) {
+            void* ka[] = {&sa, &p->dev, &p->d_inst_base, &dfi, &dub, &cb};
+            HIP_TRY(hipModuleLaunchKernel(p->spawn_update, total_chunks, 1, 1, kBlock, 1, 1, 0, st, ka, nullptr));
+            ctx->spawn_stats.fused_frames += 1;
+            ctx->spawn_stats.fused_launches += 1;
+            p->fused_spawn_frames += 1;
         } else if (p->jit_update) {
             void* ka[] = {&sa, &p->d_inst_base, &dfi, &dub, &cb};
             HIP_TRY(hipModuleLaunchKernel(p->jit_update, total_chunks, 1, 1, kBlock, 1, 1, 0, st, ka, nullptr));
@@ -2330,6 +2417,21 @@
     fj.heavy = pick_heavy_program(ctx, order, timed);
     fill_lists_jobs(ctx, order, slot, stage_off, timed, fj);
     fill_merge_jobs(ctx, order, slot, stage_off, timed, fj);
+    for (HnbProgram* p : order) {
+        plan::FusedSpawnFacts sf;
+        sf.option = ctx->fuse_spawn; sf.module_installed = p->spawn_update != nullptr; sf.update_streams = p->update_streams;
+        sf.update_merged = p->plan.merge.update_family >= 0; sf.init_merged = p->plan.merge.init_family >= 0;
+        sf.independent = p->plan.independent; sf.fuse_span = p->fuse_span; sf.timed_frame = timed;
+        if (!sf.module_installed && p->spawn_state == HnbProgram::SpawnState::NotRequested && !p->spawn_blob.empty()) {
+            plan::FusedSpawnFacts probe = sf;
+            probe.module_installed = true; probe.timed_frame = false;
+            if (plan::plan_fused_spawn(probe, p->plan.slot_init)) {
+                request_spawn_kernel(ctx, p);
+                sf.module_installed = p->spawn_update != nullptr;
+            }
+        }
+        p->plan.fused_spawn = plan::plan_fused_spawn(sf, p->plan.slot_init);
+    }
     if (stage_off) {
         if (ctx->stage_direct) {
             direct_write(ctx->d_stage[slot], ctx->h_stage[slot], stage_off);
@@ -2489,6 +2591,12 @@
 int hnb_ctx_step_stats(HnbContext* ctx, HnbStepStats* out) {
     if (!ctx || !out) return fail(HNB_ERR_INVALID_ARG, "NULL argument");
     *out = ctx->step_stats;
+    return HNB_OK;
+}
+
+int hnb_ctx_fused_spawn_stats(HnbContext* ctx, HnbFusedSpawnStats* out) {
+    if (!ctx || !out) return fail(HNB_ERR_INVALID_ARG, "NULL argument");
+    *out = ctx->spawn_stats;
     return HNB_OK;
 }
 
@@ -3403,6 +3511,14 @@
         if (prog->auto_materialise) s += " (HNB_AGE_COHORT_AUTO: the asset's render modifiers read AGE, the update keeps the plane current)";
     }
     if (prog->slot_init_frames) s += "\nslot-major init (large spawns): " + std::to_string(prog->slot_init_frames) + " frames";
+    switch (prog->spawn_state) {
+    case HnbProgram::SpawnState::NotRequested: break;
+    case HnbProgram::SpawnState::Built:
+        s += "\nspawn kernel: " + prog->spawn_kernel_name + (prog->spawn_from_cache ? " (jit cache hit)" : "") + ", " + std::to_string(prog->fused_spawn_frames) + " frames";
+        break;
+    case HnbProgram::SpawnState::Pending: s += "\nspawn kernel: pending (HNB_OPT_JIT_ASYNC)"; break;
+    case HnbProgram::SpawnState::Failed: s += "\nspawn kernel: failed: " + prog->spawn_why; break;
+    }
     if (prog->has_ribbons && prog->suffix_frames) s += "\ncasualties proven to be the list's last rows (no k_count_rows): " + std::to_string(prog->suffix_frames) + " frames";
     if (prog->has_ribbons && prog->ring_frames) s += "\nlist kept as a ring (no row rewritten): " + std::to_string(prog->ring_frames) + " frames";
     if (prog->has_ribbons && prog->sort_skipped_frames) s += "\nribbon sorts skipped in list-free frames: " + std::to_string(prog->sort_skipped_frames) + " frames";
@@ -3462,6 +3578,24 @@
     if (!rq.want_update_stream) return HNB_OK;
     jit::Result res;
     if (!jit::build_steps(rq, res)) return fail(HNB_ERR_BAD_PROGRAM, "steps kernel: specialisation failed: %s", res.log.c_str());
+    return HNB_OK;
+}
+
+int hnb_jit_precompile_spawn(const void* blob, size_t blob_size) {
+    HnbProgramHeader h;
+    int rc = validate_blob(blob, blob_size, &h);
+    if (rc != HNB_OK) return rc;
+    const uint8_t* b = static_cast<const uint8_t*>(blob);
+    std::vector<HnbAttrEntry> attrs(h.n_attrs);
+    memcpy(attrs.data(), b + h.attrs_off, h.n_attrs * sizeof(HnbAttrEntry));
+    if (!update_is_streamable(b, h, attrs.data())) return HNB_OK;
+    StreamLaunchFn fn = nullptr, fused = nullptr;
+    const char* name = "";
+    select_stream_kernel(reinterpret_cast<const Ins*>(b + h.update_off), h.update_len, &fn, &name, &fused);
+    const jit::Request rq = make_jit_request(b, h, attrs.data(), true, strcmp(name, "ProgInterp") != 0, ProgramOptions());
+    if (!rq.want_init || !rq.want_init_slots || rq.update_len == 0u) return HNB_OK;
+    jit::Result res;
+    if (!jit::build_spawn(rq, res)) return fail(HNB_ERR_BAD_PROGRAM, "spawn kernel: specialisation failed: %s", res.log.c_str());
     return HNB_OK;
 }
 
diff --git a/bevy_hanabi_amd/csrc/hnb_jit.h b/bevy_hanabi_amd/csrc/hnb_jit.h
--- a/bevy_hanabi_amd/csrc/hnb_jit.h
+++ b/bevy_hanabi_amd/csrc/hnb_jit.h
@@ -71,7 +71,7 @@
     }
 }
 
-inline void emit_code_struct(std::ostringstream& o, const Request& rq, const std::string& name) {
+inline void emit_code_struct(std::ostringstream& o, const Request& rq, const std::string& name, bool spawn_members = false) {
     o << "struct " << name << " {\n";
     o << "    using file_t = " << (rq.wide_file ? "vreg_file_wide_t" : "vreg_file_t") << ";\n";
     o << "    template <class ST> static __device__ __forceinline__ void run_init(const DevProgram& p, ST& S, const VmUniforms& U, const VmAttrIO& io) {\n";
@@ -109,7 +109,23 @@
         if ((at.update_flags & HNB_ATTR_UPD_STORE) && at.reg != HNB_REG_NONE)
             o << "        vfile_store_attr(S.r, " << (unsigned)at.ncomp << "u, " << (unsigned)at.reg << "u, base + p.attrs[" << a << "].plane_off, slot);\n";
     }
-    o << "    }\n};\n";
+    o << "    }\n";
+    if (spawn_members) {
+        bool lifetime = false;
+        o << "    template <class ST> static __device__ __forceinline__ void store_init_rest(const DevProgram& p, const ST& S, char* base, uint32_t slot, uint32_t upd) {\n";
+        for (uint32_t a = 0; a < rq.n_attrs; ++a) {
+            const HnbAttrEntry& at = rq.attrs[a];
+            if (at.reg == HNB_REG_NONE) continue;
+            if (at.reg == HNB_REG_LIFETIME) { lifetime = true; continue; }
+            const int pin = at.reg == HNB_REG_POSITION ? 0 : at.reg == HNB_REG_VELOCITY ? 1 : at.reg == HNB_REG_AGE ? 2 : -1;
+            o << "        ";
+            if (pin >= 0) o << "if (!(upd & " << (16u << pin) << "u)) ";
+            o << "vfile_store_attr(S.r, " << (unsigned)at.ncomp << "u, " << (unsigned)at.reg << "u, base + p.attrs[" << a << "].plane_off, slot);\n";
+        }
+        o << "    }\n";
+        o << "    static constexpr bool kStoresLifetime = " << (lifetime ? "true" : "false") << ";\n";
+    }
+    o << "};\n";
 }
 inline std::string stream_prog_type(const Request& rq) {
     std::ostringstream e;
@@ -143,6 +159,20 @@
     e << "hnb::k_update_slots_stream<" << stream_prog_type(rq) << ", " << rq.stream_waves << ", 0, " << (rq.stream_cohort ? "true" : "false") << ", true>";
     name_exprs.push_back(e.str());
     return "#define HNB_JIT_TU 1\n#include \"hnb_kernels.hip.h\"\n// steps module\n";
+}
+
+inline std::string make_spawn_source(const Request& rq, std::vector<std::string>& name_exprs) {
+    name_exprs.clear();
+    if (!rq.want_init || !rq.want_init_slots || rq.update_len == 0u) return std::string();
+    std::ostringstream o;
+    o << "#define HNB_JIT_TU 1\n#include \"hnb_kernels.hip.h\"\n// spawn module\nnamespace hnb {\n";
+    emit_code_struct(o, rq, "SpawnCode", true);
+    o << "}  // namespace hnb\n";
+    std::ostringstream e;
+    e << "hnb::k_update_slots_stream_spawn<hnb::SpawnCode, " << stream_prog_type(rq) << ", " << (rq.stream_waves < 4 ? rq.stream_waves : 4) << ", "
+      << (rq.stream_cohort ? "true" : "false") << ">";
+    name_exprs.push_back(e.str());
+    return o.str();
 }
 
 inline std::string set_signature(const Request& rq) {
@@ -335,6 +365,15 @@
     return true;
 }
 
+inline bool build_spawn(const Request& rq, Result& out, bool cache_only = false) {
+    std::vector<std::string> exprs, lowered;
+    const std::string src = make_spawn_source(rq, exprs);
+    if (exprs.empty()) return false;
+    if (!compile_cached(src, exprs, out.code, lowered, out.log, out.from_cache, cache_only)) return false;
+    out.update_name = lowered[0];
+    return true;
+}
+
 struct SetResult {
     std::vector<char> code;
     SetPlan plan;
diff --git a/bevy_hanabi_amd/csrc/hnb_kernels.hip.h b/bevy_hanabi_amd/csrc/hnb_kernels.hip.h
--- a/bevy_hanabi_amd/csrc/hnb_kernels.hip.h
+++ b/bevy_hanabi_amd/csrc/hnb_kernels.hip.h
@@ -337,7 +337,7 @@
         if (slot[q] != 0xffffffffu) flags[slot[q]] = 2u;
 }
 #endif
-template <class CODE>
+template <class CODE, bool ROWS_ONLY = false>
 __device__ __forceinline__ void init_slots_workgroup(const DevProgram& prog, const uint64_t* __restrict__ inst_base, const DevMeta* __restrict__ meta_in,
                                                      const DevFrameInst* __restrict__ fi, const uint32_t* __restrict__ ublocks, const uint32_t wg) {
     SlotInitCtx c;
@@ -356,6 +356,7 @@
         const uint32_t r = c.w * kSlotInitWg + q * kBlock + tid;
         row_slot[q] = r < c.n_spawn ? ld_hint(dead + (c.alive0 + r), nt) : 0xffffffffu;
     }
+    if constexpr (!ROWS_ONLY) {
     uint8_t* flags = reinterpret_cast<uint8_t*>(base + prog.alive_flag_off);
     const uint32_t slot0 = c.w * kSlotInitWg, j = slot0 / kChunk;
     uint32_t byte[kSubs];
@@ -403,6 +404,7 @@
         if (prog.cull_lifetime) reinterpret_cast<float*>(base + prog.lmin_off)[j] = 0.0f;
         if (alive_byte == 3u && st != 2u) astate[j] = 2u;
     }
+    }
 #pragma unroll
     for (uint32_t q = 0; q < kSubs; ++q) {
         const uint32_t r = c.w * kSlotInitWg + q * kBlock + tid;
@@ -419,11 +421,11 @@
         }
     }
 }
-template <class CODE>
+template <class CODE, bool ROWS_ONLY = false>
 __global__ void __launch_bounds__(kBlock)
 k_init_slots(const DevProgram prog, const uint64_t* __restrict__ inst_base, const DevMeta* __restrict__ meta_in,
              const DevFrameInst* __restrict__ fi, const uint32_t* __restrict__ ublocks) {
-    init_slots_workgroup<CODE>(prog, inst_base, meta_in, fi, ublocks, blockIdx.x);
+    init_slots_workgroup<CODE, ROWS_ONLY>(prog, inst_base, meta_in, fi, ublocks, blockIdx.x);
 }
 
 template <int P>
@@ -1055,10 +1057,12 @@
     return s;
 }
 
-template <class PROG, int PROBE, bool COHORT, bool FUSED = false>
+template <class PROG, int PROBE, bool COHORT, bool FUSED = false, bool SPAWN = false, class CODE = InterpCode>
 __device__ __forceinline__ void update_stream_chunk(const SlotArgs& args, const uint64_t* __restrict__ inst_base, const DevFrameInst* __restrict__ fi,
                                                     const uint32_t* __restrict__ ublocks, const CompactBufs& cb,
-                                                    const uint32_t wg, const uint32_t wg_total) {
+                                                    const uint32_t wg, const uint32_t wg_total,
+                                                    const DevProgram* sprog = nullptr) {
+    static_assert(!SPAWN || (!FUSED && PROBE == 0), "the spawning form is a single-frame product kernel");
     StreamLds& lds = stream_lds();
     uint32_t (&s_died)[kBlock / 64] = lds.died;
     float (&s_lmin)[kBlock / 64] = lds.lmin;
@@ -1068,7 +1072,7 @@
     uint32_t (&s_amax)[kBlock / 64] = lds.amax;
     u4v (&s_xp)[2][kBlock / 64][kStepRows * 3u / 4u] = lds.xp;
     const uint32_t tid = threadIdx.x, lane = tid & 63u, wave = tid >> 6;
-    const bool split = !FUSED && !COHORT && args.quarters == 4u;
+    const bool split = !FUSED && !COHORT && !SPAWN && args.quarters == 4u;
     const uint32_t S = FUSED ? args.fuse_steps : 1u;
     const uint32_t chunk = split ? chunk_of_workgroup(cb.xcd_remap, wg >> 2, wg_total >> 2) : chunk_of_workgroup(cb.xcd_remap, wg, wg_total);
     const uint32_t quarter = split ? (wg & 3u) : 0u;
@@ -1078,7 +1082,7 @@
     const uint32_t n_words = split ? wg_total >> 2 : wg_total;
     const uint32_t frozen = fi[k].skip;
     const uint64_t slab = inst_base[k];
-    const bool store_nt = args.store_hint != 0u;
+    const bool store_nt = args.store_hint != 0u && !SPAWN;
 #ifndef HNB_PUBLISH_FIRST_WG
 #define HNB_PUBLISH_FIRST_WG 1
 #endif
@@ -1136,7 +1140,38 @@
     const bool chunk_full = cfull[j] == 1u;
     uint32_t* astate = cfull + args.chunks_per_inst;
     uint32_t* aval = astate + args.chunks_per_inst;
-    const uint32_t ast_raw = COHORT ? astate[j] : 0u;
+    uint32_t sp_want = 0xffffffffu;
+    bool sp_chunk = false;
+    uint32_t sp_f4[kWaveRows / kStepRows] = {0u, 0u, 0u, 0u};
+    auto spawn_mask = [&](const uint32_t f4m, const uint32_t s0) {
+        uint32_t m = 0u;
+#pragma unroll
+        for (uint32_t p = 0; p < 4u; ++p) m |= (((f4m >> (8u * p)) & 0xffu) == sp_want && s0 + p < args.capacity) ? 1u << p : 0u;
+        return m;
+    };
+    if constexpr (SPAWN) {
+        const uint32_t alive0 = args.meta_in[k].alive_count;
+        const uint32_t max_spawn = args.capacity - alive0;
+        const uint32_t spawn = requested_spawn(fi[k]);
+        const uint32_t n_spawn = spawn < max_spawn ? spawn : max_spawn;
+        if (n_spawn != 0u) sp_want = n_spawn == max_spawn ? 0u : 2u;
+        bool mine = false;
+#pragma unroll
+        for (uint32_t step = 0; step < kWaveRows / kStepRows; ++step) {
+            const uint32_t s0 = wave0 + step * kStepRows + lane * 4u;
+            sp_f4[step] = chunk_full ? 0x01010101u : (s0 < args.capacity ? ld_hint(flags4 + (s0 >> 2), args.stream_hint != 0u) : 0u);
+            mine = mine || spawn_mask(sp_f4[step], s0) != 0u;
+        }
+        const bool wave_spawns = __any(mine);
+        if (lane == 0) s_amax[wave] = wave_spawns ? 1u : 0u;
+        lds_barrier();
+        sp_chunk = (s_amax[0] | s_amax[1] | s_amax[2] | s_amax[3]) != 0u;
+        lds_barrier();
+        static_assert(kBlock / 64 == 4, "the vote above reads four words");
+    }
+    const uint32_t ast_mem = COHORT ? astate[j] : 0u;
+    const bool sp_fresh = SPAWN && COHORT && args.age_cohort != 0u && sp_chunk && (ast_mem == 1u || ast_mem == 2u);
+    const uint32_t ast_raw = sp_fresh ? 2u : ast_mem;
     bool check_due = ((args.frame_phase + j) & 15u) == 0u;
     if constexpr (FUSED) {
         for (uint32_t s = 1; s < S; ++s) check_due = check_due || ((args.frame_phase + s + j) & 15u) == 0u;
@@ -1148,7 +1183,7 @@
     uint32_t lane_alive = 0;
     const bool cull = args.cull_lifetime != 0u;
     float* lmin = reinterpret_cast<float*>(base + args.lmin_off);
-    const float Lm = cull ? lmin[j] : 0.0f;
+    const float Lm = (cull && !(SPAWN && sp_chunk)) ? lmin[j] : 0.0f;
     const float dt_tick = cull ? uf(U, args.dt_operand) : 0.0f;
     auto age_after = [&](float a) {
         if constexpr (FUSED) {
@@ -1209,9 +1244,17 @@
             if (args.safe_words) rem_min = (f2u(A2) >> 31) ? 0.0f : (Lm - A2) - 1.0e-5f * Lm;
         }
     }
-    auto step_body = [&](auto coh_tag, const uint32_t step, const uint32_t f4, const u4v* pre_age = nullptr) {
+    auto step_body = [&](auto coh_tag, const uint32_t step, const uint32_t f4_mem, const u4v* pre_age = nullptr) {
         constexpr bool COH = decltype(coh_tag)::value;
         const uint32_t s0 = wave0 + step * kStepRows + lane * 4u;
+        const uint32_t spm = SPAWN ? spawn_mask(f4_mem, s0) : 0u;
+        uint32_t f4 = f4_mem;
+        if constexpr (SPAWN) {
+            const uint32_t born = sp_fresh ? 3u : 1u;
+#pragma unroll
+            for (uint32_t p = 0; p < 4u; ++p)
+                if ((spm >> p) & 1u) f4 = (f4 & ~(0xffu << (8u * p))) | (born << (8u * p));
+        }
         bool was[4], fresh[4];
 #pragma unroll
         for (int p = 0; p < 4; ++p) {
@@ -1236,18 +1279,25 @@
         bool need_life = true;
         float age_was[4] = {0.0f, 0.0f, 0.0f, 0.0f};
         const uint32_t step_first = s0 - lane * 4u;
-        const bool xp = args.transpose != 0u && PROBE == 0 && step_first + kStepRows <= args.capacity && __popcll(__ballot(any)) >= 32;
-        if (xp) {
+        bool sp_old = false;
+        if constexpr (SPAWN) {
+#pragma unroll
+            for (int p = 0; p < 4; ++p) sp_old = sp_old || (was[p] && !((spm >> p) & 1u));
+        }
+        const bool sp_skip = SPAWN ? !__any(sp_old) : false;
+        const bool xp_step = args.transpose != 0u && PROBE == 0 && step_first + kStepRows <= args.capacity && __popcll(__ballot(any)) >= 32;
+        const bool xp = SPAWN ? (xp_step && (!sp_skip || __all(full))) : xp_step;
+        if (xp && !sp_skip) {
             if (fl & 1u) xpose_load3(X.pos, p_pos, step_first, s_xp[0][wave], lane);
             if (fl & 2u) xpose_load3(X.vel, p_vel, step_first, s_xp[1][wave], lane);
         }
         if (any) {
-            if (!xp) {
+            if (!xp && !sp_skip) {
                 if (fl & 1u) pin_load3<4>(X.pos, p_pos, slot, lanes_on, true);
                 if (fl & 2u) pin_load3<4>(X.vel, p_vel, slot, lanes_on, true);
             }
             if (fl & 4u) {
-                if (!COH || ast != 1u) {
+                if ((!COH || ast != 1u) && !sp_skip) {
                     if (pre_age) { X.age[0] = u2f(pre_age->x); X.age[1] = u2f(pre_age->y); X.age[2] = u2f(pre_age->z); X.age[3] = u2f(pre_age->w); }
                     else pin_load1<4>(X.age, p_age, slot, lanes_on, true);
                     for (int p = 0; p < 4; ++p) age_was[p] = X.age[p];
@@ -1264,7 +1314,7 @@
             for (int p = 0; p < 4; ++p) may_die = may_die || (was[p] && !(age_after(X.age[p]) < Lm));
             need_life = __any(may_die);
         }
-        if (any && (fl & 8u)) {
+        if (any && (fl & 8u) && !sp_skip) {
             if (need_life) {
                 if (args.stream_hint) {
                     const u4v ql = __builtin_nontemporal_load(reinterpret_cast<const u4v*>(p_life) + (slot[0] >> 2));
@@ -1277,6 +1327,37 @@
             }
         }
         if (!need_life) loaded_all = false;
+        if constexpr (SPAWN) {
+            if (__any(spm != 0u)) {
+                float born_life[4] = {0.0f, 0.0f, 0.0f, 0.0f};
+                bool sp[4];
+#pragma unroll
+                for (int p = 0; p < 4; ++p) {
+                    sp[p] = ((spm >> p) & 1u) != 0u;
+                    if (sp[p]) {
+                        VmState<typename CODE::file_t> S;
+                        S.r = typename CODE::file_t{};
+                        S.pindex = slot[p] + fi[k].slot_base;
+                        S.seed = pcg_hash(S.pindex ^ fi[k].seed);
+                        S.pcounter = 0u;
+                        S.alive = true;
+                        VmAttrIO io;
+                        io.slab = base; io.attrs = sprog->attrs; io.slot = slot[p];
+                        CODE::zero_unassigned(*sprog, io);
+                        CODE::run_init(*sprog, S, U, io);
+                        CODE::store_init_rest(*sprog, S, base, slot[p], fl);
+                        if (fl & 1u) X.pos[p] = V3{u2f(S.r[HNB_REG_POSITION]), u2f(S.r[HNB_REG_POSITION + 1]), u2f(S.r[HNB_REG_POSITION + 2])};
+                        if (fl & 2u) X.vel[p] = V3{u2f(S.r[HNB_REG_VELOCITY]), u2f(S.r[HNB_REG_VELOCITY + 1]), u2f(S.r[HNB_REG_VELOCITY + 2])};
+                        if (fl & 4u) X.age[p] = u2f(S.r[HNB_REG_AGE]);
+                        if (fl & 8u) X.lifetime[p] = u2f(S.r[HNB_REG_LIFETIME]);
+                        born_life[p] = u2f(S.r[HNB_REG_LIFETIME]);
+                    }
+                }
+                if constexpr (CODE::kStoresLifetime) {
+                    if (!(fl & 128u) && spm != 0u) pin_store1<4>(born_life, p_life, slot, sp, spm == 0xfu);
+                }
+            }
+        }
         if constexpr (FUSED) {
             bool gone[4] = {false, false, false, false};
             for (uint32_t s = 0; s < S; ++s) {
@@ -1298,7 +1379,7 @@
                 if (fl & 64u) {
                     const bool plane_loaded = !COH || ast != 1u;
                     if (plane_loaded || args.age_current) {
-                        if (plane_loaded && (fl & 4u) && !full) {
+                        if (plane_loaded && (fl & 4u) && !full && !sp_skip) {
                             float q[4];
 #pragma unroll
                             for (int p = 0; p < 4; ++p) q[p] = was[p] ? X.age[p] : age_was[p];
@@ -1350,7 +1431,7 @@
             else if (COH && fresh[p]) nf = (nf & ~(0xffu << (8 * p))) | (1u << (8 * p));
             died_here += (uint32_t)__popcll(__ballot(died));
         }
-        if (nf != f4) flags4[s0 >> 2] = nf;
+        if (nf != f4_mem) flags4[s0 >> 2] = nf;
         if (args.write_died) store_died_bits(reinterpret_cast<uint32_t*>(base + args.died_bits_off), step_first, nib, lane);
         died_total += died_here;
     };
@@ -1359,7 +1440,15 @@
             const uint32_t s0 = wave0 + step * kStepRows + lane * 4u;
             return chunk_full ? 0x01010101u : (s0 < args.capacity ? ld_hint(flags4 + (s0 >> 2), args.stream_hint != 0u) : 0u);
         };
-        if constexpr (COHORT || PROG::kFlat) {
+        if constexpr (SPAWN) {
+            if (mixed) {
+#pragma unroll
+                for (uint32_t step = 0; step < kWaveRows / kStepRows; ++step) if (step < n_steps) step_body(BoolTag<false>{}, step, sp_f4[step]);
+            } else {
+#pragma unroll
+                for (uint32_t step = 0; step < kWaveRows / kStepRows; ++step) if (step < n_steps) step_body(BoolTag<COHORT>{}, step, sp_f4[step]);
+            }
+        } else if constexpr (COHORT || PROG::kFlat) {
             uint32_t f4s[kWaveRows / kStepRows];
 #pragma unroll
             for (uint32_t step = 0; step < kWaveRows / kStepRows; ++step) f4s[step] = step < n_steps ? f4_of(step) : 0u;
@@ -1409,7 +1498,7 @@
             for (uint32_t w = 0; w < kBlock / 64; ++w) { lo = s_amin[w] < lo ? s_amin[w] : lo; hi = s_amax[w] > hi ? s_amax[w] : hi; }
             const uint32_t next = (lo == hi) ? 1u : (lo > hi ? 0u : 4u);
             if (next == 1u) aval[j] = lo;
-            if (next != ast_raw) astate[j] = next;
+            if (next != ast_mem) astate[j] = next;
         }
         uint32_t d = 0;
 #pragma unroll
@@ -1440,6 +1529,15 @@
 k_update_slots_stream(const SlotArgs args, const uint64_t* __restrict__ inst_base, const DevFrameInst* __restrict__ fi,
                       const uint32_t* __restrict__ ublocks, const CompactBufs cb) {
     update_stream_chunk<PROG, PROBE, COHORT, FUSED>(args, inst_base, fi, ublocks, cb, blockIdx.x, gridDim.x);
+}
+#ifndef HNB_SPAWN_WAVES
+#define HNB_SPAWN_WAVES 0
+#endif
+template <class CODE, class PROG, int WAVES, bool COHORT>
+__global__ void __launch_bounds__(kBlock, (HNB_SPAWN_WAVES ? HNB_SPAWN_WAVES : WAVES))
+k_update_slots_stream_spawn(const SlotArgs args, const DevProgram prog, const uint64_t* __restrict__ inst_base, const DevFrameInst* __restrict__ fi,
+                            const uint32_t* __restrict__ ublocks, const CompactBufs cb) {
+    update_stream_chunk<PROG, 0, COHORT, false, true, CODE>(args, inst_base, fi, ublocks, cb, blockIdx.x, gridDim.x, &prog);
 }
 #ifndef HNB_JIT_TU
 #ifndef HNB_AGEK_CUT
diff --git a/bevy_hanabi_amd/csrc/hnb_plan.h b/bevy_hanabi_amd/csrc/hnb_plan.h
--- a/bevy_hanabi_amd/csrc/hnb_plan.h
+++ b/bevy_hanabi_amd/csrc/hnb_plan.h
@@ -200,6 +200,23 @@
     return d;
 }
 
+struct FusedSpawnFacts {
+    bool option = true;
+    bool module_installed = false;
+    bool update_streams = false;
+    bool update_merged = false;
+    bool init_merged = false;
+    bool independent = false;
+    uint32_t fuse_span = 1;
+    bool timed_frame = false;
+};
+inline bool plan_fused_spawn(const FusedSpawnFacts& f, const SlotInitDecision& slot_init) {
+    if (!slot_init.use) return false;
+    if (!f.option || !f.module_installed || f.timed_frame) return false;
+    if (!f.update_streams || f.update_merged || f.init_merged || f.fuse_span >= 2u) return false;
+    return f.independent;
+}
+
 struct MergeFacts {
     bool independent = false;
     uint32_t total_chunks = 0;
@@ -321,7 +338,8 @@
     MergeDecision merge;
     uint32_t init_blocks = 0;
     SlotInitDecision slot_init;
-};
-
-}
-}
+    bool fused_spawn = false;
+};
+
+}
+}
diff --git a/bevy_hanabi_amd/runtime.py b/bevy_hanabi_amd/runtime.py
--- a/bevy_hanabi_amd/runtime.py
+++ b/bevy_hanabi_amd/runtime.py
@@ -29,9 +29,11 @@
     "hnb_effect_bounds", "hnb_program_bounds",
 ]
 ABI_BINNED_SYMBOLS = ["hnb_effect_export_binned"]
+ABI_SPAWN_SYMBOLS = ["hnb_ctx_fused_spawn_stats", "hnb_jit_precompile_spawn"]
 
 OPTIONS = {"list_order": 1, "alternate": 2, "skip_lists": 3, "age_cohort": 4, "cull_lifetime": 5, "horizon": 6, "transpose": 7, "scene_merge": 8,
-           "suffix_proof": 9, "overlap_updates": 10, "stream_hints": 11, "set_module": 12, "jit_async": 13, "test_break_proof": 15, "ring_lists": 16, "slot_init": 17, "direct_upload": 18, "fuse_steps": 19}
+           "suffix_proof": 9, "overlap_updates": 10, "stream_hints": 11, "set_module": 12, "jit_async": 13, "test_break_proof": 15, "ring_lists": 16, "slot_init": 17, "direct_upload": 18, "fuse_steps": 19,
+           "fuse_spawn": 20}
 MAX_FUSED_STEPS = 8
 SET_MODULE_OFF, SET_MODULE_CACHED, SET_MODULE_COMPILE, SET_MODULE_BACKGROUND = 0, 1, 2, 3
 
@@ -58,6 +60,13 @@
 
 class StepStats(C.Structure):
     _fields_ = [(n, C.c_uint64) for n in ("frames", "fused_frames", "fused_launches", "update_launches", "list_launches")]
+
+    def as_dict(self):
+        return {n: int(getattr(self, n)) for n, _ in self._fields_}
+
+
+class FusedSpawnStats(C.Structure):
+    _fields_ = [(n, C.c_uint64) for n in ("fused_frames", "fused_launches", "rows_launches", "unfused_frames")]
 
     def as_dict(self):
         return {n: int(getattr(self, n)) for n, _ in self._fields_}
@@ -302,6 +311,8 @@
         lib.hnb_effect_set_frames_ahead.argtypes = [C.c_void_p, C.c_uint32, C.c_void_p, C.c_void_p, C.c_void_p]
         lib.hnb_program_set_frames_ahead.argtypes = [C.c_void_p, C.c_uint32, C.c_uint32, C.c_uint32, C.c_void_p, C.c_void_p, C.c_void_p]
         lib.hnb_ctx_step_stats.argtypes = [C.c_void_p, C.POINTER(StepStats)]
+        lib.hnb_ctx_fused_spawn_stats.argtypes = [C.c_void_p, C.POINTER(FusedSpawnStats)]
+        lib.hnb_jit_precompile_spawn.argtypes = [C.c_char_p, C.c_size_t]
         lib.hnb_program_prepare_steps.argtypes = [C.c_void_p]
         lib.hnb_jit_precompile_steps.argtypes = [C.c_char_p, C.c_size_t]
         lib.hnb_effect_export.argtypes = [C.c_void_p, C.POINTER(ExportDesc)]
@@ -335,6 +346,10 @@
     _check(load_library().hnb_jit_precompile_steps(blob, len(blob)))
 
 
+def jit_precompile_spawn(blob: bytes):
+    _check(load_library().hnb_jit_precompile_spawn(blob, len(blob)))
+
+
 def jit_precompile_set(blobs):
     blobs = list(blobs)
     arr = (C.c_char_p * len(blobs))(*blobs)
@@ -410,6 +425,11 @@
         _check(self._lib.hnb_ctx_step_stats(self._h, C.byref(s)))
         return s.as_dict()
 
+    def fused_spawn_stats(self):
+        s = FusedSpawnStats()
+        _check(self._lib.hnb_ctx_fused_spawn_stats(self._h, C.byref(s)))
+        return s.as_dict()
+
     def enable_kernel_timing(self, every_n_frames=1):
         _check(self._lib.hnb_ctx_enable_kernel_timing(self._h, int(every_n_frames)))
 
diff --git a/include/hanabi_amd.h b/include/hanabi_amd.h
--- a/include/hanabi_amd.h
+++ b/include/hanabi_amd.h
@@ -211,6 +211,7 @@
 #define HNB_SET_MODULE_COMPILE 2u
 #define HNB_SET_MODULE_BACKGROUND 3u
 #define HNB_OPT_FUSE_STEPS 19u
+#define HNB_OPT_FUSE_SPAWN 20u
 #define HNB_MAX_FUSED_STEPS 8u
 int hnb_ctx_set_option(HnbContext* ctx, uint32_t option, uint32_t value);
 
diff --git a/include/hanabi_amd_spawn.h b/include/hanabi_amd_spawn.h
--- /dev/null
+++ b/include/hanabi_amd_spawn.h
@@ -0,0 +1,25 @@
+#ifndef HANABI_AMD_SPAWN_H
+#define HANABI_AMD_SPAWN_H
+
+#include "hanabi_amd.h"
+
+#ifdef __cplusplus
+extern "C" {
+#endif
+
+typedef struct HnbFusedSpawnStats {
+    uint64_t fused_frames;
+    uint64_t fused_launches;
+    uint64_t rows_launches;
+    uint64_t unfused_frames;
+} HnbFusedSpawnStats;
+
+int hnb_ctx_fused_spawn_stats(HnbContext* ctx, HnbFusedSpawnStats* out);
+
+int hnb_jit_precompile_spawn(const void* blob, size_t blob_size);
+
+#ifdef __cplusplus
+}
+#endif
+
+#endif
```
